# NJU-3DV/Relightable3DGaussian

Hardware: AMD Instinct MI355X
Metric: train iters/s, synthetic lego-like 800x800, 300000 Gaussians (stage-2 hot path) (higher is better)
Workload: dtype f32; 1 GPU; stage-2 train iteration (fused glue kernels + one-launch Adam): shading fwd/bwd (K=64) + rasterize fwd (S=16) + loss + rasterize bwd + Adam; 1 view/rank/step, 300000 Gaussians, 800x800, num_rendered~1755006; parallelism=dp1

## Files before the change

include/r3dg_hip.h:

```cpp
#ifndef R3DG_HIP_H
#define R3DG_HIP_H

#include <stddef.h>
#include <stdint.h>

#ifdef __cplusplus
extern "C" {
#endif

#define R3DG_OK 0
#define R3DG_EINVAL (-1)
#define R3DG_EHIP (-2)
#define R3DG_EALLOC (-3)

typedef void* (*r3dg_alloc_fn)(void* user, size_t bytes);

const char* r3dg_last_error(void);
int r3dg_release_scratch(void);
int r3dg_version(void);

int r3dg_max_features_forward(void);
int r3dg_max_features_backward(void);

size_t r3dg_geometry_state_bytes(int P);
// ... 103 lines not shown
                                 float* d_out);
int r3dg_shade_build_transport_rayset(void* stream, int P, int K, int M, const float* d_normals, const float* d_incidents,
                                      const float* d_visibility, const float* d_zsamples, float uniform_area,
                                      const float* d_env, int He, int We, const float* d_env_transform,
                                      float* d_transport, float* d_consts);
int r3dg_shade_build_transport_baked(void* stream, int P, int K, int M, const float* d_normals, const float* d_incidents,
                                     const float* d_visibility_sh, const float* d_zsamples, float uniform_area,
                                     const float* d_env, int He, int We, const float* d_env_transform,
                                     float* d_transport, float* d_consts);
int r3dg_visibility_sh_expand(void* stream, int P, int K, const float* d_normals, const float* d_zsamples,
                              const float* d_visibility_sh, float* d_visibility_out);
int r3dg_shade_build_split(void* stream, int P, int K, const int32_t* d_perm, const float* d_normals, const float* d_incidents,
                           const float* d_visibility, const float* d_incident_dirs, const float* d_zsamples,
                           float uniform_area, float* d_lt, float* d_vis_t, float* d_consts);
size_t r3dg_shade_env_footprints_bytes(int He, int We);
int r3dg_shade_env_footprints(void* stream, int He, int We, const float* d_env, float* d_env_footprints);
int r3dg_shade_forward_split(void* stream, int P, int K, const int32_t* d_perm, const float* d_base_color,
                             const float* d_roughness, const float* d_normals, const float* d_viewdirs, const float* d_lt,
                             const float* d_vis_t, const float* d_consts, const float* d_zsamples,
                             const float* d_env_transform, const float* d_env_footprints, int He, int We, float* d_out);
int r3dg_shade_frs_supported(int K, int M, int He, int We);
size_t r3dg_shade_frs_tables_bytes(int K);
int r3dg_shade_frs_build_tables(void* stream, int K, const float* d_zsamples, float* d_tables);
int r3dg_shade_frs_classify(void* stream, int P, const float* d_ray_normals, uint8_t* d_valid);
int r3dg_shade_frs_build_taps(void* stream, int P, int K, const float* d_ray_normals, const float* d_zsamples, int He, int We,
                              uint32_t* d_taps);
int r3dg_stream_wait_stream(void* waiter, void* signaller);
int r3dg_spin(void* stream, float microseconds);
int r3dg_store_u64_to_host(void* stream, const void* d_src, void* h_pinned_dst);
int r3dg_clock_probe(void* stream, int iters, unsigned long long* d_out3, float* d_sink, int* wall_clock_khz);

int r3dg_shade_frs_rotate(void* stream, int P, const float* d_incidents, const float* d_ray_normals, float* d_cprime);
int r3dg_shade_frs_forward(void* stream, int P, int K, const float* d_base_color, const float* d_roughness,
                           const float* d_normals, const float* d_viewdirs, const float* d_incidents, const float* d_env,
                           int He, int We, const float* d_visibility, float uniform_area, const uint32_t* d_taps,
                           const float* d_ray_normals, const float* d_zsamples, const float* d_tables,
                           const uint8_t* d_valid, const int32_t* d_invalid_list, int n_invalid, float* d_cprime, int flags,
                           float* d_out, void* listed_stream, float* d_feature_rows);
int r3dg_shade_frs_backward(void* stream, int P, int K, const float* d_base_color, const float* d_roughness,
                            const float* d_normals, const float* d_viewdirs, const float* d_incidents, const float* d_env,
                            int He, int We, const float* d_visibility, float uniform_area, const uint32_t* d_taps,
                            const float* d_ray_normals, const float* d_zsamples, const float* d_tables,
                            const uint8_t* d_valid, const int32_t* d_invalid_list, int n_invalid, const float* d_cprime,
                            float* d_dcprime, const float* d_dL_dpbr, const float* d_dL_ddiffuse_light,
                            float* d_dL_dbase_color, float* d_dL_droughness, float* d_dL_dviewdirs, float* d_dL_dincidents,
                            float* d_dL_denv, const float* d_block_absmax, int n_block_absmax, void* rotate_stream);
#define R3DG_SHADE_NO_ROTATION_BACK ((void*)(intptr_t)-1)
#define R3DG_CHAIN_LISTED_ROWS_IN_DCPRIME 1
#define R3DG_CHAIN_NO_GRADIENT_OUT 2
int r3dg_shade_frs_incident_chain(void* stream, int P, const float* d_ray_normals, const uint8_t* d_valid,
                                  const float* d_dcprime, float* d_dL_dincidents, float* d_incidents, float* d_exp_avg,
                                  float* d_exp_avg_sq, float* d_cprime, float lr, float lr_tail, float beta1, float beta2,
                                  float eps, int step, float grad_scale, const float* d_skip_flag, int chain_flags);

int r3dg_shade_backward(void* stream, int P, int K, int M, const float* d_base_color, const float* d_roughness,
                        const float* d_normals, const float* d_viewdirs, const float* d_incidents, const float* d_env,
                        int He, int We, const float* d_env_transform, const float* d_visibility,
                        const float* d_incident_dirs, const float* d_incident_areas, const float* d_dL_dpbr,
                        const float* d_dL_ddiffuse_light, float* d_dL_dbase_color, float* d_dL_droughness,
                        float* d_dL_dviewdirs, float* d_dL_dincidents, float* d_dL_denv);

int r3dg_shade_backward_cached(void* stream, int P, int K, int M, const float* d_base_color, const float* d_roughness,
                               const float* d_normals, const float* d_viewdirs, const float* d_incidents,
                               const float* d_env, int He, int We, const float* d_env_transform,
                               const float* d_visibility, const float* d_incident_dirs, const float* d_incident_areas,
                               const uint32_t* d_taps, const float* d_dL_dpbr, const float* d_dL_ddiffuse_light,
                               float* d_dL_dbase_color, float* d_dL_droughness, float* d_dL_dviewdirs,
                               float* d_dL_dincidents, float* d_dL_denv, const float* d_block_absmax,
                               int n_block_absmax);

int r3dg_render_equation_forward(void* stream, int P, int Si, int Sd, int Sv, const float* d_base_color,
                                 const float* d_roughness, const float* d_metallic, const float* d_normals,
                                 const float* d_viewdirs, const float* d_incidents_shs, const float* d_direct_shs,
                                 const float* d_visibility_shs, int sample_num, const float* d_rand_float,
                                 float* d_incident_dirs, float* d_pbr, float* d_diffuse_light);
int r3dg_render_equation_forward_complex(void* stream, int P, int Si, int Sd, int Sv, const float* d_base_color,
                                         const float* d_roughness, const float* d_metallic, const float* d_normals,
                                         const float* d_viewdirs, const float* d_incidents_shs,
                                         const float* d_direct_shs, const float* d_visibility_shs, int sample_num,
                                         float* d_incident_dirs, float* d_pbr, float* d_incident_lights,
                                         float* d_local_incident_lights, float* d_global_incident_lights,
                                         float* d_incident_visibility, float* d_diffuse_light,
                                         float* d_local_diffuse_light, float* d_accum, float* d_rgb_d, float* d_rgb_s);
int r3dg_render_equation_backward(void* stream, int P, int Si, int Sd, int Sv, const float* d_base_color,
                                  const float* d_roughness, const float* d_metallic, const float* d_normals,
                                  const float* d_viewdirs, const float* d_incidents_shs, const float* d_direct_shs,
                                  const float* d_visibility_shs, int sample_num, const float* d_incident_dirs,
                                  const float* d_dL_dpbr, const float* d_dL_ddiffuse_light, float* d_dL_dbase_color,
                                  float* d_dL_droughness, float* d_dL_dmetallic, float* d_dL_dnormals,
                                  float* d_dL_dviewdirs, float* d_dL_dincidents_shs, float* d_dL_ddirect_shs,
                                  float* d_dL_dvisibility_shs);

#define R3DG_SUM_SLOTS 32

int r3dg_stage2_activate(void* stream, int P, const float* d_xyz, const float* d_scaling_raw,
                         const float* d_rotation_raw, const float* d_opacity_raw, const float* d_normal_raw,
                         const float* d_base_raw, const float* d_rough_raw, const float* d_campos, float* d_scales,
                         float* d_rotations, float* d_opacity, float* d_normal, float* d_base_color,
                         float* d_roughness, float* d_viewdirs, const float* d_viewmatrix, float* d_features);
int r3dg_stage2_pack_features(void* stream, int P, const float* d_xyz, const float* d_viewmatrix, const float* d_normal,
                              const float* d_base_color, const float* d_roughness, const float* d_shade_out,
                              float* d_features, float* d_light_l1_sum);
int r3dg_stage2_unpack_gradients(void* stream, int P, const float* d_dL_dfeatures, const float* d_shade_out,
                                 float light_weight, float* d_dL_dpbr, float* d_dL_ddiffuse_light,
                                 float* d_block_absmax, float* d_light_l1_sum);
int r3dg_stage2_activate_backward(void* stream, int P, const float* d_xyz, const float* d_scaling_raw,
                                  const float* d_rotation_raw, const float* d_opacity_raw, const float* d_normal_raw,
                                  const float* d_base_raw, const float* d_rough_raw, const float* d_viewmatrix,
                                  const float* d_campos, const float* d_dL_dfeatures, const float* d_dL_dbase_color,
                                  const float* d_dL_droughness, const float* d_dL_dviewdirs, const float* d_dL_dscales,
                                  const float* d_dL_drotations, const float* d_dL_dopacity, const float* d_dL_dmeans3D,
                                  float* d_g_xyz, float* d_g_scaling, float* d_g_rotation, float* d_g_opacity,
                                  float* d_g_normal, float* d_g_base, float* d_g_rough);
int r3dg_stage2_loss(void* stream, int width, int height, const float* d_image, const float* d_opacity,
                     const float* d_feature, const float* d_pseudo_normal, const int32_t* d_n_contrib,
                     const float* d_gt, const float* d_background, const float* d_image_mask, float w_l1, float w_pbr,
                     float w_normal, const float* d_extra_dL_dimage, const float* d_extra_dL_dsrgb, float* d_dL_dimage,
                     float* d_dL_dopacity, float* d_dL_dfeature, float* d_sums,
                     int sparse_feature_gradients);
int r3dg_stage2_smooth_forward(void* stream, int width, int height, const float* d_opacity, const float* d_feature,
                               const int32_t* d_n_contrib, const float* d_gt, const float* d_image_mask,
                               float w_base_color, float w_roughness, float w_light, float* d_scratch, float* d_sums3);
int r3dg_stage2_smooth_backward(void* stream, int width, int height, const float* d_opacity, const float* d_feature,
                                const int32_t* d_n_contrib, const float* d_image_mask, const float* d_scratch,
                                float w_base_color, float w_roughness, float w_light, int accumulate_normal,
                                float* d_dL_dopacity, float* d_dL_dfeature);
int r3dg_stage2_smooth_fused(void* stream, int width, int height, const float* d_opacity, const float* d_feature,
                             const int32_t* d_n_contrib, const float* d_gt, const float* d_image_mask, float w_base_color,
                             float w_roughness, float w_light, int accumulate_normal, float* d_dL_dopacity,
                             float* d_dL_dfeature, float* d_sums3);
int r3dg_stage2_pbr_srgb(void* stream, int width, int height, const float* d_opacity, const float* d_feature,
                         const int32_t* d_n_contrib, const float* d_background, float* d_srgb);

int r3dg_stage2_activate_with(void* stream, int P, const float* d_xyz, const float* d_scaling_raw,
                              const float* d_rotation_raw, const float* d_opacity_raw, const float* d_normal_raw,
                              const float* d_base_raw, const float* d_rough_raw, const float* d_campos, float* d_scales,
                              float* d_rotations, float* d_opacity, float* d_normal, float* d_base_color,
                              float* d_roughness, float* d_viewdirs, const float* d_viewmatrix, float* d_features,
                              int n_env, const float* d_env_raw, float* d_env, float* d_zero, int n_zero);
int r3dg_stage2_activate_backward_with(void* stream, int P, const float* d_xyz, const float* d_scaling_raw,
                                       const float* d_rotation_raw, const float* d_opacity_raw, const float* d_normal_raw,
                                       const float* d_base_raw, const float* d_rough_raw, const float* d_viewmatrix,
                                       const float* d_campos, const float* d_dL_dfeatures, const float* d_dL_dbase_color,
                                       const float* d_dL_droughness, const float* d_dL_dviewdirs, const float* d_dL_dscales,
                                       const float* d_dL_drot, const float* d_dL_dopacity, const float* d_dL_dmeans3D,
                                       float* d_g_xyz, float* d_g_scaling, float* d_g_rotation, float* d_g_opacity,
                                       float* d_g_normal, float* d_g_base, float* d_g_rough, int He, int We,
                                       const float* d_env_raw, const float* d_env, float* d_dL_denv, float w_tv,
                                       float* d_g_env_raw, float* d_tv_sum, int consume);
int r3dg_stage2_normals_srgb(void* stream, int width, int height, const float* d_viewmatrix, float tan_fovx, float tan_fovy,
                             float cx, float cy, const float* d_opacity, const float* d_depth, float* d_pseudo_normal,
                             float* d_surface_xyz, const float* d_feature, const int32_t* d_n_contrib,
                             const float* d_background, float* d_srgb);

int r3dg_ssim_forward(void* stream, int width, int height, int channels, const float* d_x, const float* d_y,
                      float* d_partials, float* d_sum);
int r3dg_ssim_backward(void* stream, int width, int height, int channels, const float* d_x, const float* d_y,
                       const float* d_partials, float scale, float* d_grad_x);
int r3dg_ssim_forward_pair(void* stream, int width, int height, int channels, const float* d_x0, const float* d_x1,
                           const float* d_y, float* d_partials0, float* d_partials1, float* d_sum0, float* d_sum1);
int r3dg_ssim_backward_pair(void* stream, int width, int height, int channels, const float* d_x0, const float* d_x1,
                            const float* d_y, const float* d_partials0, const float* d_partials1, float scale0,
                            float scale1, float* d_grad_x0, float* d_grad_x1);

int r3dg_stage1_pack_features(void* stream, int P, const float* d_xyz, const float* d_viewmatrix, const float* d_normal,
                              float* d_features);
int r3dg_stage1_loss(void* stream, int width, int height, const float* d_image, const float* d_opacity,
                     const float* d_feature, const float* d_pseudo_normal, const int32_t* d_n_contrib, const float* d_gt,
                     const float* d_image_mask, float w_l1, float w_mask_entropy, float w_normal, float w_normal_smooth,
                     float w_depth_var, const float* d_extra_dL_dimage, float* d_edge_scratch, float* d_dL_dimage,
                     float* d_dL_dopacity, float* d_dL_dfeature, float* d_sums);
int r3dg_stage1_activate_backward(void* stream, int P, const float* d_xyz, const float* d_scaling_raw,
                                  const float* d_rotation_raw, const float* d_opacity_raw, const float* d_normal_raw,
                                  const float* d_viewmatrix, const float* d_dL_dfeatures, const float* d_dL_dscales,
                                  const float* d_dL_drotations, const float* d_dL_dopacity, const float* d_dL_dmeans3D,
                                  float* d_g_xyz, float* d_g_scaling, float* d_g_rotation, float* d_g_opacity,
                                  float* d_g_normal);

int r3dg_supervision_count(void* stream, int width, int height, const float* d_gt_depth, const float* d_image_mask,
                           uint32_t* d_count);
int r3dg_stage2_supervision(void* stream, int width, int height, const float* d_opacity, const float* d_feature,
                            const int32_t* d_n_contrib, const float* d_gt_depth, const float* d_mvs_normal,
                            const float* d_image_mask, const uint32_t* d_count, float w_depth, float w_normal_mvs,
                            int accumulate_normal, float* d_dL_dopacity, float* d_dL_dfeature, float* d_sums2);
int r3dg_stage1_depth_smooth(void* stream, int width, int height, const float* d_opacity, const float* d_feature,
                             const int32_t* d_n_contrib, const float* d_gt, float w_depth_smooth, float* d_edge_scratch,
                             float* d_dL_dopacity, float* d_dL_dfeature, float* d_sum);
int r3dg_stage1_gaussian_terms(void* stream, int P, const float* d_weights, const float* d_opacity, const float* d_normal,
                               const float* d_scales, const float* d_xyz, const float* d_campos, float w_point_entropy,
                               float w_orientation, float w_scaling, float* d_dL_dopacity, float* d_dL_dfeatures,
                               float* d_dL_dscales, float* d_dL_dmeans3D, float* d_sums3);

int r3dg_stage2_env_backward(void* stream, int He, int We, const float* d_raw, const float* d_env, float* d_dL_denv,
                             float w_tv, float* d_g_raw, float* d_tv_sum, int consume);

#define R3DG_ADAM_MAX_GROUPS 16
typedef struct r3dg_adam_group {
    float* param;
    const float* grad;
    float* exp_avg;
    float* exp_avg_sq;
    uint64_t n;
    float lr, lr_tail;
    uint32_t period, split;
} r3dg_adam_group;
int r3dg_adam_step(void* stream, int n_groups, const r3dg_adam_group* groups, float beta1, float beta2, float eps,
                   int step, float grad_scale, const float* d_skip_flag);

int r3dg_rasterize_backward_sh_adam_supported(int M);
int r3dg_rasterize_backward_split_sh_adam(void* stream, void* geometry_stream, int P, int S, int D, int M, int R,
                                          const float* d_background, int width, int height, const float* d_means3D,
                                          const float* d_shs, const float* d_features, const float* d_colors_precomp,
                                          const float* d_scales, float scale_modifier, const float* d_rotations,
                                          const float* d_cov3D_precomp, const float* d_viewmatrix,
                                          const float* d_projmatrix, const float* d_campos, float tan_fovx, float tan_fovy,
                                          const int32_t* d_radii, const void* d_geom_buffer, const void* d_binning_buffer,
                                          const void* d_img_buffer, const float* d_dL_dpix, const float* d_dL_dpix_o,
                                          const float* d_dL_dpix_d, const float* d_dL_dpix_f, float* d_dL_dmean2D,
                                          float* d_dL_dconic, float* d_dL_dopacity, float* d_dL_dcolor,
                                          float* d_dL_dfeature, float* d_dL_dmean3D, float* d_dL_dcov3D, float* d_dL_dsh,
                                          float* d_dL_dscale, float* d_dL_drot, int backward_geometry, int debug,
                                          int n_active_features, const int* active_features,
                                          const r3dg_adam_group* sh_adam, float beta1, float beta2, float eps, int step,
                                          float grad_scale, const float* d_skip_flag);

int r3dg_relight_pack_features(void* stream, int P, const float* d_xyz, const float* d_viewmatrix, const float* d_normal,
                               const float* d_base_color, const float* d_roughness, const float* d_shade_out,
                               float* d_features);
int r3dg_relight_compose(void* stream, int width, int height, float focal_x, float focal_y, float cx, float cy,
                         const float* d_viewmatrix, const float* d_light_transform, const float* d_envmap, int He, int We,
                         const float* d_image, const float* d_opacity, const float* d_feature,
                         const int32_t* d_n_contrib, float* d_pbr_env, float* d_render_env, float* d_env_only);

#define R3DG_EVAL_ROW 8
#define R3DG_EVAL_MEDIAN_STATE_WORDS 1024
int r3dg_relight_capture(void* stream, int width, int height, const float* d_feature, const float* d_opacity,
                         const int32_t* d_n_contrib, const float* d_background, const float* d_mask, float* d_pbr,
                         float* d_base_color, float* d_roughness, float* d_normal, float* d_visibility, float* d_diffuse,
                         float* d_specular, float* d_lights, float* d_local_lights, float* d_global_lights,
                         float* d_depth_var);
int r3dg_eval_image_metrics(void* stream, int width, int height, int channels, const float* d_pred, const float* d_gt,
                            const float* d_mask, const float* d_fill, int fill_is_image, double* d_tile_sums,
                            double* d_row);
int r3dg_eval_median_ratio(void* stream, int width, int height, const float* d_pred, const float* d_gt,
                           const float* d_mask, uint32_t* d_state, double* d_row);

#define R3DG_SCENE_COLUMNS 130
#define R3DG_SCENE_STAGE1_COLUMNS 62
#define R3DG_SCENE_GROUPS 13
#define R3DG_SCENE_MAX_COLUMNS 250
#define R3DG_SCENE_PLACEMENT_FLOATS 111
#define R3DG_SCENE_ZERO_INCIDENTS 1
#define R3DG_SCENE_ROTATE_SH 2
int r3dg_scene_place_records(void* stream, int P, int A, const float* d_records, const int32_t* d_column_map,
                             const float* d_placement, int flags, long long row_offset, void** dst_groups);
int r3dg_scene_place_groups(void* stream, int P, void** src_groups, const float* d_placement, int flags,
                            long long row_offset, void** dst_groups);
int r3dg_scene_pack_records(void* stream, int P, int columns, void** src_groups, float* d_records);

int r3dg_relight_quantize(void* stream, int width, int height, int channels, const float* d_image, uint8_t* d_bytes);

int r3dg_view_unpack(void* stream, int width, int height, int channels, const uint8_t* d_pixels, const float* d_background,
                     float* d_image, float* d_mask);

int r3dg_view_unpack_masked(void* stream, int width, int height, const uint8_t* d_pixels, const uint8_t* d_mask_bytes,
                            float* d_image, float* d_mask);

#define R3DG_VIEW_RESIZE_MAX_SCALE 16
int r3dg_view_resize(void* stream, int width, int height, int channels, const uint8_t* d_pixels, const uint8_t* d_mask_bytes,
                     const float* d_background, int out_width, int out_height, float* d_image, float* d_mask);

#define R3DG_EXR_TILE 4096
#define R3DG_EXR_MAX_KEPT 8
#define R3DG_EXR_MAX_TILES 32768
int r3dg_exr_unpack_chunks(void* stream, int width, int height, int file_channels, int bytes_per_sample, int chunks,
                           int max_chunk_rows, const uint8_t* d_inflated, long long inflated_bytes, const int32_t* d_chunk_table,
                           int kept, const int32_t* d_kept_channels, uint32_t* d_tile_sums, long long tile_sums_count,
                           void* d_planes);

int r3dg_view_unpack_hdr(void* stream, int width, int height, int is_half, const void* d_view, const uint8_t* d_mask_bytes,
                         const float* d_background, float* d_image, float* d_mask);

int r3dg_densify_accumulate(void* stream, int P, const float* d_viewspace_grad, const float* d_normal_grad,
                            const int32_t* d_radii, const float* d_weights, float* d_xyz_gradient_accum,
                            float* d_normal_gradient_accum, float* d_denom, float* d_weights_accum,
                            float* d_max_radii2D,
                            const float* d_skip_flag);

typedef struct r3dg_densify_config {
    int32_t mode;
    int32_t n_split;
    float grad_threshold, grad_normal_threshold, min_opacity, weights_threshold;
    float dense_size, world_size_limit, split_divisor, max_screen_size;
} r3dg_densify_config;

size_t r3dg_densify_temp_bytes(int P);
int r3dg_densify_plan(void* stream, int P, const r3dg_densify_config* config, const float* d_scaling_raw,
                      const float* d_opacity_raw, const float* d_xyz_gradient_accum,
                      const float* d_normal_gradient_accum, const float* d_denom, const float* d_weights_accum,
                      const float* d_max_radii2D, int32_t* d_src_row, int32_t* d_kind, int32_t* d_counts, void* d_temp);

#define R3DG_DENSIFY_MAX_GROUPS 24
#define R3DG_DENSIFY_ROLE_COPY 0
#define R3DG_DENSIFY_ROLE_XYZ 1
#define R3DG_DENSIFY_ROLE_SCALING 2
typedef struct r3dg_densify_group {
// ... 95 lines not shown
```

relightable3dgaussian_amd/csrc/capi_stage.hip:

```cpp
#include "capi_internal.hpp"

using namespace r3dg;

extern "C" {

int r3dg_stage2_activate(void* stream_, int P, const float* xyz, const float* scaling_raw, const float* rotation_raw,
                         const float* opacity_raw, const float* normal_raw, const float* base_raw,
                         const float* rough_raw, const float* campos, float* scales, float* rot, float* opacity,
                         float* normal, float* base_color, float* roughness, float* viewdirs, const float* viewmatrix,
                         float* features)
{
    return r3dg_stage2_activate_with(stream_, P, xyz, scaling_raw, rotation_raw, opacity_raw, normal_raw, base_raw, rough_raw,
                                     campos, scales, rot, opacity, normal, base_color, roughness, viewdirs, viewmatrix, features,
                                     0, nullptr, nullptr, nullptr, 0);
}

int r3dg_stage2_activate_with(void* stream_, int P, const float* xyz, const float* scaling_raw, const float* rotation_raw,
                              const float* opacity_raw, const float* normal_raw, const float* base_raw,
                              const float* rough_raw, const float* campos, float* scales, float* rot, float* opacity,
                              float* normal, float* base_color, float* roughness, float* viewdirs, const float* viewmatrix,
                              float* features, int n_env, const float* env_raw, float* env, float* zero, int n_zero)
{
    if (P < 0) return invalid("stage2_activate: bad P");
    if (n_env < 0 || n_zero < 0) return invalid("stage2_activate: bad side-job size");
// ... 109 lines not shown
                     float* dL_dfeature, float* sums, int sparse_feature_gradients)
{
    if (width < 0 || height < 0) return invalid("stage2_loss: bad image size");
    if ((long long)width * height == 0) return R3DG_OK;
    if (!image || !opacity || !feature || !pseudo_normal || !n_contrib || !gt || !bg || !dL_dimage || !dL_dopacity ||
        !dL_dfeature || !sums)
        return invalid("stage2_loss: null buffer");
    return guarded([&]() -> int {
        StageTimer t((hipStream_t)stream_, ST_S2_LOSS);
        launch_s2_loss((hipStream_t)stream_, width * height, image, opacity, feature, pseudo_normal, n_contrib, gt, bg,
                       image_mask, w_l1, w_pbr, w_normal, extra_dimage, extra_dsrgb, dL_dimage, dL_dopacity, dL_dfeature, sums,
                       sparse_feature_gradients);
        return R3DG_OK;
    });
}

int r3dg_stage2_smooth_forward(void* stream_, int width, int height, const float* opacity, const float* feature,
                               const int32_t* n_contrib, const float* gt, const float* image_mask, float w_base_color,
                               float w_roughness, float w_light, float* scratch, float* sums3)
{
    if (width < 0 || height < 0) return invalid("stage2_smooth_forward: bad image size");
    if ((long long)width * height == 0) return R3DG_OK;
    if (!opacity || !feature || !n_contrib || !gt || !scratch || !sums3) return invalid("stage2_smooth_forward: null buffer");
    return guarded([&]() -> int {
        StageTimer t((hipStream_t)stream_, ST_S2_LOSS);
        launch_s2_smooth_forward((hipStream_t)stream_, width, height, opacity, feature, n_contrib, gt, image_mask,
                                 w_base_color, w_roughness, w_light, scratch, sums3);
        return R3DG_OK;
    });
}

int r3dg_stage2_smooth_backward(void* stream_, int width, int height, const float* opacity, const float* feature,
                                const int32_t* n_contrib, const float* image_mask, const float* scratch, float w_base_color,
                                float w_roughness, float w_light, int accumulate_normal, float* dL_dopacity,
                                float* dL_dfeature)
{
    if (width < 0 || height < 0) return invalid("stage2_smooth_backward: bad image size");
    if ((long long)width * height == 0) return R3DG_OK;
    if (!opacity || !feature || !n_contrib || !scratch || !dL_dopacity || !dL_dfeature)
        return invalid("stage2_smooth_backward: null buffer");
    return guarded([&]() -> int {
        StageTimer t((hipStream_t)stream_, ST_S2_LOSS);
        launch_s2_smooth_backward((hipStream_t)stream_, width, height, opacity, feature, n_contrib, image_mask, scratch,
                                  w_base_color != 0.f, w_roughness != 0.f, w_light != 0.f, accumulate_normal, dL_dopacity,
                                  dL_dfeature);
        return R3DG_OK;
    });
}

int r3dg_stage2_smooth_fused(void* stream_, int width, int height, const float* opacity, const float* feature,
                             const int32_t* n_contrib, const float* gt, const float* image_mask, float w_base_color,
                             float w_roughness, float w_light, int accumulate_normal, float* dL_dopacity, float* dL_dfeature,
                             float* sums3)
{
    if (width < 0 || height < 0) return invalid("stage2_smooth_fused: bad image size");
    if ((long long)width * height == 0) return R3DG_OK;
    if (!opacity || !feature || !n_contrib || !gt || !dL_dopacity || !dL_dfeature || !sums3)
        return invalid("stage2_smooth_fused: null buffer");
    return guarded([&]() -> int {
        StageTimer t((hipStream_t)stream_, ST_S2_LOSS);
        launch_s2_smooth_fused((hipStream_t)stream_, width, height, opacity, feature, n_contrib, gt, image_mask, w_base_color,
                               w_roughness, w_light, accumulate_normal, dL_dopacity, dL_dfeature, sums3);
        return R3DG_OK;
    });
}

int r3dg_stage1_pack_features(void* stream_, int P, const float* xyz, const float* viewmatrix, const float* normal,
                              float* features)
{
    if (P < 0) return invalid("stage1_pack_features: bad P");
    if (P == 0) return R3DG_OK;
    if (!xyz || !viewmatrix || !normal || !features) return invalid("stage1_pack_features: null buffer");
    return guarded([&]() -> int {
        StageTimer t((hipStream_t)stream_, ST_S2_PACK);
        launch_s1_pack((hipStream_t)stream_, P, xyz, viewmatrix, normal, features);
        return R3DG_OK;
    });
}

int r3dg_stage1_loss(void* stream_, int width, int height, const float* image, const float* opacity,
                     const float* feature, const float* pseudo_normal, const int32_t* n_contrib, const float* gt,
                     const float* image_mask, float w_l1, float w_mask_entropy, float w_normal, float w_normal_smooth,
                     float w_depth_var, const float* extra_dimage, float* edge_scratch, float* dL_dimage,
                     float* dL_dopacity, float* dL_dfeature, float* sums)
{
    if (width < 0 || height < 0) return invalid("stage1_loss: bad image size");
    if ((long long)width * height == 0) return R3DG_OK;
    if (!image || !opacity || !feature || !pseudo_normal || !n_contrib || !gt || !dL_dimage || !dL_dopacity ||
        !dL_dfeature || !sums)
        return invalid("stage1_loss: null buffer");
    if (w_normal_smooth != 0.f && !edge_scratch) return invalid("stage1_loss: the normal-smoothness term needs edge_scratch");
    return guarded([&]() -> int {
        StageTimer t((hipStream_t)stream_, ST_S2_LOSS);
        if (w_normal_smooth != 0.f)
            launch_s1_edge((hipStream_t)stream_, width, height, feature, opacity, n_contrib, gt, edge_scratch, sums + 4 * R3DG_SUM_SLOTS);
        launch_s1_loss((hipStream_t)stream_, width, height, image, opacity, feature, pseudo_normal, n_contrib, gt, image_mask,
                       w_l1, w_mask_entropy, w_normal, w_normal_smooth, w_depth_var, extra_dimage,
                       w_normal_smooth != 0.f ? edge_scratch : nullptr, dL_dimage, dL_dopacity, dL_dfeature, sums);
        return R3DG_OK;
    });
}

int r3dg_stage1_activate_backward(void* stream_, int P, const float* xyz, const float* scaling_raw,
                                  const float* rotation_raw, const float* opacity_raw, const float* normal_raw,
                                  const float* viewmatrix, const float* dL_dfeatures, const float* dL_dscales,
                                  const float* dL_drot, const float* dL_dopacity, const float* dL_dmeans3D, float* g_xyz,
                                  float* g_scaling, float* g_rotation, float* g_opacity, float* g_normal)
{
    if (P < 0) return invalid("stage1_activate_backward: bad P");
    if (P == 0) return R3DG_OK;
    if (!xyz || !scaling_raw || !rotation_raw || !opacity_raw || !normal_raw || !viewmatrix || !dL_dfeatures ||
        !dL_dscales || !dL_drot || !dL_dopacity || !dL_dmeans3D || !g_xyz || !g_scaling || !g_rotation || !g_opacity ||
        !g_normal)
        return invalid("stage1_activate_backward: null buffer");
    return guarded([&]() -> int {
        StageTimer t((hipStream_t)stream_, ST_S2_ACTIVATE_BWD);
        launch_s1_activate_backward((hipStream_t)stream_, P, xyz, scaling_raw, rotation_raw, opacity_raw, normal_raw,
                                    viewmatrix, dL_dfeatures, dL_dscales, dL_drot, dL_dopacity, dL_dmeans3D, g_xyz,
                                    g_scaling, g_rotation, g_opacity, g_normal);
        return R3DG_OK;
    });
}

int r3dg_stage2_pbr_srgb(void* stream_, int width, int height, const float* opacity, const float* feature,
                         const int32_t* n_contrib, const float* bg, float* srgb)
{
    if (width < 0 || height < 0) return invalid("stage2_pbr_srgb: bad image size");
    if ((long long)width * height == 0) return R3DG_OK;
    if (!opacity || !feature || !n_contrib || !bg || !srgb) return invalid("stage2_pbr_srgb: null buffer");
    return guarded([&]() -> int {
        launch_s2_pbr_srgb((hipStream_t)stream_, width * height, opacity, feature, n_contrib, bg, srgb);
        return R3DG_OK;
    });
}

int r3dg_stage2_normals_srgb(void* stream_, int width, int height, const float* viewmatrix, float tan_fovx, float tan_fovy,
                             float cx, float cy, const float* opacity, const float* depth, float* pseudo_normal,
                             float* surface_xyz, const float* feature, const int32_t* n_contrib, const float* bg, float* srgb)
{
    if (width < 0 || height < 0) return invalid("stage2_normals_srgb: bad image size");
    if ((long long)width * height == 0) return R3DG_OK;
    if ((long long)width * height > 0x7fffffffLL) return invalid("stage2_normals_srgb: image too large");
    if (!viewmatrix || !opacity || !depth || !pseudo_normal || !surface_xyz || !feature || !n_contrib || !bg || !srgb)
        return invalid("stage2_normals_srgb: null buffer");
    return guarded([&]() -> int {
        StageTimer t((hipStream_t)stream_, ST_NORMAL);
        const float focal_y = height / (2.0f * tan_fovy), focal_x = width / (2.0f * tan_fovx);
        launch_s2_normals_srgb((hipStream_t)stream_, width, height, viewmatrix, focal_x, focal_y, cx, cy, opacity, depth,
                               pseudo_normal, surface_xyz, feature, n_contrib, bg, srgb);
        return R3DG_OK;
    });
}

int r3dg_ssim_forward_pair(void* stream_, int width, int height, int channels, const float* x0, const float* x1,
                           const float* y, float* partials0, float* partials1, float* sum0, float* sum1)
{
    if (width < 0 || height < 0 || channels < 0) return invalid("ssim_forward: bad shape");
    if ((long long)width * height * channels == 0) return R3DG_OK;
    if (!x0 || !y || !partials0 || (x1 && !partials1)) return invalid("ssim_forward: null buffer");
    if ((long long)channels * 2 > 65535) return invalid("ssim_forward: too many channels");
    return guarded([&]() -> int {
        StageTimer t((hipStream_t)stream_, ST_SSIM);
        const float* x[2] = {x0, x1};
        float* partials[2] = {partials0, partials1};
        float* sum[2] = {sum0, sum1};
        launch_ssim_forward((hipStream_t)stream_, width, height, channels, x1 ? 2 : 1, x, y, partials, sum);
        return R3DG_OK;
    });
}

int r3dg_ssim_backward_pair(void* stream_, int width, int height, int channels, const float* x0, const float* x1,
                            const float* y, const float* partials0, const float* partials1, float scale0, float scale1,
                            float* grad_x0, float* grad_x1)
{
    if (width < 0 || height < 0 || channels < 0) return invalid("ssim_backward: bad shape");
    if ((long long)width * height * channels == 0) return R3DG_OK;
    if (!x0 || !y || !partials0 || !grad_x0 || (x1 && (!partials1 || !grad_x1))) return invalid("ssim_backward: null buffer");
    if ((long long)channels * 2 > 65535) return invalid("ssim_backward: too many channels");
    return guarded([&]() -> int {
        StageTimer t((hipStream_t)stream_, ST_SSIM);
        const float* x[2] = {x0, x1};
        float* partials[2] = {const_cast<float*>(partials0), const_cast<float*>(partials1)};
        const float scale[2] = {scale0, scale1};
        float* grad[2] = {grad_x0, grad_x1};
        launch_ssim_backward((hipStream_t)stream_, width, height, channels, x1 ? 2 : 1, x, y, partials, scale, grad);
        return R3DG_OK;
    });
}

int r3dg_ssim_forward(void* stream_, int width, int height, int channels, const float* x, const float* y,
                      float* partials, float* sum)
{
    return r3dg_ssim_forward_pair(stream_, width, height, channels, x, nullptr, y, partials, nullptr, sum, nullptr);
}

int r3dg_ssim_backward(void* stream_, int width, int height, int channels, const float* x, const float* y,
                       const float* partials, float scale, float* grad_x)
{
    return r3dg_ssim_backward_pair(stream_, width, height, channels, x, nullptr, y, partials, nullptr, scale, 0.f, grad_x,
                                   nullptr);
}

int r3dg_stage2_env_backward(void* stream_, int He, int We, const float* raw, const float* env, float* dL_denv,
                             float w_tv, float* g_raw, float* tv_sum, int consume)
{
    if (He < 0 || We < 0) return invalid("stage2_env_backward: bad texture size");
    if (He * We == 0) return R3DG_OK;
    if (!raw || !env || !dL_denv || !g_raw) return invalid("stage2_env_backward: null buffer");
    return guarded([&]() -> int {
        launch_s2_env_backward((hipStream_t)stream_, He, We, raw, env, dL_denv, w_tv, g_raw, tv_sum, consume);
        return R3DG_OK;
    });
}

int r3dg_adam_step(void* stream_, int n_groups, const r3dg_adam_group* groups, float beta1, float beta2, float eps,
                   int step, float grad_scale, const float* skip_flag)
{
    if (n_groups < 0 || n_groups > R3DG_ADAM_MAX_GROUPS) return invalid("adam_step: bad group count");
    if (step < 1) return invalid("adam_step: step counts from 1");
    if (n_groups == 0) return R3DG_OK;
    if (!groups) return invalid("adam_step: null group table");
    for (int i = 0; i < n_groups; i++) {
        if (groups[i].n >= (1ull << 32)) return invalid("adam_step: group larger than 2^32 elements");
        if (groups[i].n && (!groups[i].param || !groups[i].grad || !groups[i].exp_avg || !groups[i].exp_avg_sq))
            return invalid("adam_step: null buffer in group");
    }
    return guarded([&]() -> int {
        StageTimer t((hipStream_t)stream_, ST_ADAM);
        launch_adam((hipStream_t)stream_, n_groups, groups, beta1, beta2, eps, step, grad_scale, skip_flag);
        return R3DG_OK;
    });
}

int r3dg_relight_pack_features(void* stream_, int P, const float* xyz, const float* viewmatrix, const float* normal,
                               const float* base_color, const float* roughness, const float* shade_out, float* features)
{
    if (P < 0) return invalid("relight_pack_features: bad P");
    if (P == 0) return R3DG_OK;
    if (!xyz || !viewmatrix || !normal || !base_color || !roughness || !shade_out || !features)
        return invalid("relight_pack_features: null buffer");
    if ((size_t)features & 15) return invalid("relight_pack_features: features must be 16-byte aligned");
    return guarded([&]() -> int {
        StageTimer t((hipStream_t)stream_, ST_RELIGHT_PACK);
        launch_relight_pack((hipStream_t)stream_, P, xyz, viewmatrix, normal, base_color, roughness, shade_out, features);
        return R3DG_OK;
    });
}

int r3dg_relight_compose(void* stream_, int width, int height, float focal_x, float focal_y, float cx, float cy,
                         const float* viewmatrix, const float* light_transform, const float* envmap, int He, int We,
                         const float* image, const float* opacity, const float* feature, const int32_t* n_contrib,
                         float* pbr_env, float* render_env, float* env_only)
{
    if (width < 0 || height < 0 || He < 1 || We < 1) return invalid("relight_compose: bad shape");
    if ((long long)width * height == 0) return R3DG_OK;
    if ((long long)width * height >= (1ll << 31)) return invalid("relight_compose: image too large");
    if (!viewmatrix || !envmap || !opacity || !feature || !n_contrib) return invalid("relight_compose: null buffer");
    if (render_env && !image) return invalid("relight_compose: render_env needs the rendered image");
    if (!(focal_x > 0.f) || !(focal_y > 0.f)) return invalid("relight_compose: focal lengths must be positive");
    return guarded([&]() -> int {
        StageTimer t((hipStream_t)stream_, ST_RELIGHT_COMPOSE);
        launch_relight_compose((hipStream_t)stream_, width, height, focal_x, focal_y, cx, cy, viewmatrix, light_transform,
                               envmap, He, We, image, opacity, feature, n_contrib, pbr_env, render_env, env_only);
        return R3DG_OK;
    });
}

int r3dg_relight_capture(void* stream_, int width, int height, const float* feature, const float* opacity,
                         const int32_t* n_contrib, const float* background, const float* mask, float* pbr,
                         float* base_color, float* roughness, float* normal, float* visibility, float* diffuse,
                         float* specular, float* lights, float* local_lights, float* global_lights, float* depth_var)
{
    if (width < 0 || height < 0) return invalid("relight_capture: bad shape");
    if ((long long)width * height == 0) return R3DG_OK;
    if ((long long)width * height >= (1ll << 31)) return invalid("relight_capture: image too large");
    if (!feature || !opacity || !n_contrib) return invalid("relight_capture: null buffer");
    if ((pbr || mask) && !background) return invalid("relight_capture: the pbr map and the mask need a background");
    const CaptureMaps maps = {pbr, base_color, roughness, normal, visibility, diffuse, specular, lights, local_lights,
                              global_lights, depth_var};
    return guarded([&]() -> int {
        launch_relight_capture((hipStream_t)stream_, width, height, feature, opacity, n_contrib, background, mask, maps);
        return R3DG_OK;
    });
}

int r3dg_eval_image_metrics(void* stream_, int width, int height, int channels, const float* pred, const float* gt,
                            const float* mask, const float* fill, int fill_is_image, double* tile_sums, double* row)
{
    if (width < 1 || height < 1 || channels < 1 || channels > 3) return invalid("eval_image_metrics: bad shape");
    if ((long long)width * height >= (1ll << 31)) return invalid("eval_image_metrics: image too large");
    if (!pred || !gt || !tile_sums || !row) return invalid("eval_image_metrics: null buffer");
    if (fill && !mask) return invalid("eval_image_metrics: a fill needs a mask");
    return guarded([&]() -> int {
        launch_eval_image_metrics((hipStream_t)stream_, width, height, channels, pred, gt, mask, fill, fill_is_image, tile_sums,
                                  row);
        return R3DG_OK;
    });
}

int r3dg_eval_median_ratio(void* stream_, int width, int height, const float* pred, const float* gt, const float* mask,
                           uint32_t* state, double* row)
{
    if (width < 0 || height < 0) return invalid("eval_median_ratio: bad shape");
    if ((long long)width * height >= (1ll << 31)) return invalid("eval_median_ratio: image too large");
    if (!state || !row) return invalid("eval_median_ratio: null buffer");
    if ((long long)width * height != 0 && (!pred || !gt)) return invalid("eval_median_ratio: null image");
// ... 94 lines not shown
```

relightable3dgaussian_amd/csrc/launchers.hpp:

```cpp
#pragma once
#include "common.hpp"

namespace r3dg {

__attribute__((visibility("hidden"))) int persistent_cus();

void release_gradient_records();
void launch_mark_visible(hipStream_t s, int P, const float* means3D, const float* vm, uint8_t* present);
void launch_preprocess(hipStream_t s, int P, int D, int M, const float* means3D, const float* scales, float scale_modifier,
                       const float* rotations, const float* opacities, const float* shs, uint8_t* clamped,
                       const float* cov3D_precomp, const float* colors_precomp, const float* vm, const float* pm,
                       const float* cam_pos, int W, int H, float tan_fovx, float tan_fovy, float focal_x, float focal_y,
                       int* radii, float* means2D, float* depths, float* cov3Ds, float* rgb, float* conic_opacity,
                       float* splat, int gx, int gy, uint32_t* tiles_touched, uint32_t* block_sums,
                       unsigned long long* total, bool scan_now, uint32_t* zero_words, int zero_n);
void launch_duplicate_with_keys(hipStream_t s, int P, const float* means2D, const float* depths,
                                const uint32_t* tiles_touched, const uint32_t* block_offsets, uint32_t* point_offsets,
                                uint64_t* keys, uint32_t* values, const int* radii, int gx, int gy);
void launch_identify_tile_ranges(hipStream_t s, int L, const uint64_t* keys, uint32_t* ranges);
void launch_tile_order(hipStream_t s, int T, const uint32_t* ranges, uint32_t* order, uint32_t small_cap, uint32_t* big_list,
                       uint32_t* big_count);
void launch_render_forward(hipStream_t s, int W, int H, int S, const uint32_t* tile_order, const uint32_t* ranges,
                           const uint32_t* point_list, const float* splat, const float* features, float* final_T,
                           uint32_t* n_contrib, const float* bg, float* out_color, float* out_opacity, float* out_depth,
                           float* out_feature, float* out_weights);
void launch_pseudo_normal(hipStream_t s, int W, int H, const float* vm, float focal_x, float focal_y, float cx, float cy,
                          const float* opacities, const float* depths, float* normals, float* surface_xyz, bool debug);
void launch_render_backward(hipStream_t s, int P, int W, int H, int S, int n_active, const int* active,
                            const uint32_t* tile_order, const uint32_t* ranges, const uint32_t* point_list, const float* bg,
                            const float* splat, const float* features, const float* final_Ts, const uint32_t* n_contrib,
                            const float* dL_dpix, const float* dL_dpix_o, const float* dL_dpix_d, const float* dL_dpix_f,
                            float* dL_dmean2D, float* dL_dconic, float* dL_dopacity, float* dL_dcolor, float* dL_dfeature,
                            int bg_geom);
void launch_render_backward_features(hipStream_t s, int W, int H, int S, int n_active, const int* active,
                                     const uint32_t* tile_order, const uint32_t* ranges, const uint32_t* point_list,
                                     const float* splat, const float* final_Ts, const uint32_t* n_contrib,
                                     const float* dL_dpix_f, float* dL_dfeature);
struct ShAdamArgs {
    r3dg_adam_group g;
    float beta1, beta2, eps, bias1, inv_sqrt_bias2, grad_scale;
    const float* skip_flag;
};
bool preprocess_backward_applies_adam(int M);
void launch_preprocess_backward(hipStream_t s, int P, int D, int M, const float* means, const int* radii, const float* shs,
                                const uint8_t* clamped, const float* scales, const float* rotations, float scale_modifier,
                                const float* cov3Ds, const float* vm, const float* proj, float h_x, float h_y,
                                float tan_fovx, float tan_fovy, const float* campos, float* dL_dmean2D,
                                const float* dL_dconic, const float* conic_opacity, int W, int H, float* dL_dmeans,
                                const float* dL_dcolor, float* dL_dcov3D, float* dL_dsh, float* dL_dscale, float* dL_drot,
                                const ShAdamArgs* adam);
void launch_shade_forward(hipStream_t s, int P, int K, int M, const float* base_color, const float* roughness,
                          const float* normals, const float* viewdirs, const float* incidents, const float* env, int He,
                          int We, const float* tr, const float* visibility, const float* dirs, const float* areas,
                          float* out, const uint32_t* taps, bool train_outputs, float uniform_area, bool taps_are_radiance,
                          bool leave_room);
size_t shade_frs_table_floats(int K);
bool shade_frs_supported(int K, int M, int He, int We);
void launch_shade_frs_build_tables(hipStream_t s, int K, const float* zsamples, float* tables);
void launch_shade_frs_classify(hipStream_t s, int P, const float* ray_normals, uint8_t* valid);
void launch_shade_frs_build_taps(hipStream_t s, int P, int K, const float* ray_normals, const float* zsamples, int He,
                                 int We, uint32_t* taps);
void launch_shade_frs_forward_aux(hipStream_t s, int P, const float* incidents, const float* ray_normals, float* cprime);
void launch_shade_frs_forward_main(hipStream_t s, int P, int K, const float* base_color, const float* roughness,
                                   const float* normals, const float* viewdirs, const float* env, int He, int We,
                                   const float* visibility, float uniform_area, const uint32_t* taps,
                                   const float* ray_normals, const float* tables, const uint8_t* valid, const float* cprime,
                                   bool leave_room, float* out, float* feat);
void launch_shade_frs_forward_listed(hipStream_t s, int K, const float* base_color, const float* roughness,
                                     const float* normals, const float* viewdirs, const float* incidents, const float* env,
                                     int He, int We, const float* visibility, const float* ray_normals,
                                     const float* zsamples, float uniform_area, const int* invalid_list, int n_invalid,
                                     float* out, float* feat);
void launch_shade_frs_incident_chain(hipStream_t s, int P, const float* ray_normals, const uint8_t* valid, const float* dcp,
                                     float* d_inc, float* incidents, float* exp_avg, float* exp_avg_sq, float* cprime,
                                     float lr, float lr_tail, float beta1, float beta2, float eps, int step,
                                     float grad_scale, const float* skip_flag, int listed_in_dcprime, bool write_gradient);
const unsigned int* launch_shade_frs_backward_aux(hipStream_t s, int P, const float* g_pbr, const float* g_diff,
                                                  const float* block_absmax, int n_block_absmax, int* gmax_n);
void launch_shade_frs_backward_main(hipStream_t s, int P, int K, const float* base_color, const float* roughness,
                                    const float* normals, const float* viewdirs, const float* env, int He, int We,
                                    const float* visibility, float uniform_area, const uint32_t* taps,
                                    const float* ray_normals, const float* tables, const uint8_t* valid, const float* cprime,
                                    float* dcp, const float* g_pbr, const float* g_diff, float* d_base, float* d_rough,
                                    float* d_view, float* d_env, const unsigned int* gmax, int gmax_n);
void launch_shade_frs_backward_rotate(hipStream_t s, int P, const float* ray_normals, const float* dcp, float* d_inc,
                                      const uint8_t* valid);
void launch_shade_frs_backward_listed(hipStream_t s, int K, const float* base_color, const float* roughness,
                                      const float* normals, const float* viewdirs, const float* incidents, const float* env,
                                      int He, int We, const float* visibility, const float* ray_normals,
                                      const float* zsamples, float uniform_area, const int* invalid_list, int n_invalid,
                                      const float* g_pbr, const float* g_diff, float* d_base, float* d_rough, float* d_view,
                                      float* d_inc, float* d_env, const unsigned int* gmax, int gmax_n);
void launch_shade_build_taps(hipStream_t s, size_t n, const float* dirs, const float* tr, int He, int We, const float* env,
                             uint32_t* taps);
void launch_shade_build_split(hipStream_t s, int P, int K, const int* perm, const float* normals, const float* incidents,
                              const float* visibility, const float* dirs, const float* zsamples, float uniform_area,
                              float* lt, float* vis_t, float* consts);
void launch_shade_forward_split(hipStream_t s, int P, int K, const int* perm, const float* base_color,
                                const float* roughness, const float* normals, const float* viewdirs, const float* lt,
                                const float* vis_t, const float* consts, const float* zsamples, const float* tr,
                                const float* env4, int He, int We, float* out);
void launch_shade_env_footprints(hipStream_t s, int He, int We, const float* env, float* fp);
void launch_shade_build_transport(hipStream_t s, int P, int K, int M, const float* normals, const float* incidents,
                                  const float* visibility, const float* dirs, const float* areas, float uniform_area,
                                  float* radiance_to_transport, float* consts);
void launch_shade_build_transport_rayset(hipStream_t s, int P, int K, int M, const float* normals, const float* incidents,
                                         const float* visibility, const float* zsamples, float uniform_area, const float* env,
                                         int He, int We, const float* tr, float* transport, float* consts);
void launch_shade_build_transport_baked(hipStream_t s, int P, int K, int M, const float* normals, const float* incidents,
                                        const float* visibility_sh, const float* zsamples, float uniform_area, const float* env,
                                        int He, int We, const float* tr, float* transport, float* consts);
void launch_visibility_sh_expand(hipStream_t s, int P, int K, const float* normals, const float* zsamples,
                                 const float* visibility_sh, float* out);
void launch_shade_forward_transport(hipStream_t s, int P, int K, const float* base_color, const float* roughness,
                                    const float* normals, const float* viewdirs, const float* transport, const float* consts,
                                    const float* zsamples, const float* dirs, float* out);
void launch_shade_backward(hipStream_t s, int P, int K, int M, const float* base_color, const float* roughness,
                           const float* normals, const float* viewdirs, const float* incidents, const float* env, int He,
                           int We, const float* tr, const float* visibility, const float* dirs, const float* areas,
                           const float* g_pbr, const float* g_diff, float* d_base, float* d_rough, float* d_view,
                           float* d_inc, float* d_env, const uint32_t* taps, const float* block_absmax, int n_block_absmax);
void launch_re_forward(hipStream_t s, bool complex_, int P, int Si, int Sd, int Sv, const float* base_color,
                       const float* roughness, const float* metallic, const float* normals, const float* viewdirs,
                       const float* inc, const float* direct, const float* vis, int K, const float* rand_float,
                       float* incident_dirs, float* out_pbr, float* out_lights, float* out_local, float* out_global,
                       float* out_vis, float* out_diffuse, float* out_local_diffuse, float* out_accum, float* out_rgb_d,
                       float* out_rgb_s);
void launch_re_backward(hipStream_t s, int P, int Si, int Sd, int Sv, const float* base_color, const float* roughness,
                        const float* metallic, const float* normals, const float* viewdirs, const float* inc,
                        const float* direct, const float* vis, int K, const float* incident_dirs, const float* dL_dpbr,
                        const float* dL_ddl, float* dL_dbase, float* dL_drough, float* dL_dmetal, float* dL_dnormals,
                        float* dL_dviewdirs, float* dL_dinc, float* dL_ddirect, float* dL_dvis);
void launch_s2_activate(hipStream_t s, int P, const float* xyz, const float* scaling_raw, const float* rotation_raw,
                        const float* opacity_raw, const float* normal_raw, const float* base_raw, const float* rough_raw,
                        const float* campos, float* scales, float* rot, float* opacity, float* normal, float* base_color,
                        float* roughness, float* viewdirs, const float* viewmatrix, float* features, int n_env,
                        const float* env_raw, float* env, float* zero, int n_zero);
void launch_s2_pack(hipStream_t s, int P, const float* xyz, const float* viewmatrix, const float* normal,
                    const float* base_color, const float* roughness, const float* shade_out, float* features,
                    float* light_l1_sum);
void launch_s2_unpack(hipStream_t s, int P, const float* dL_dfeatures, const float* shade_out, float light_weight,
                      float* dL_dpbr, float* dL_ddiffuse, float* block_absmax, float* light_l1_sum);
void launch_s2_activate_backward(hipStream_t s, int P, const float* xyz, const float* scaling_raw, const float* rotation_raw,
                                 const float* opacity_raw, const float* normal_raw, const float* base_raw,
                                 const float* rough_raw, const float* viewmatrix, const float* campos,
                                 const float* dL_dfeatures, const float* dL_dbase_shade, const float* dL_drough_shade,
                                 const float* dL_dviewdirs, const float* dL_dscales, const float* dL_drot,
                                 const float* dL_dopacity, const float* dL_dmeans3D, float* g_xyz, float* g_scaling,
                                 float* g_rotation, float* g_opacity, float* g_normal, float* g_base, float* g_rough, int He,
                                 int We, const float* env_raw, const float* env, float* dL_denv, float w_tv,
                                 float* g_env_raw, float* tv_sum, int consume);
void launch_s2_loss(hipStream_t s, int HW, const float* image, const float* opacity, const float* feature,
                    const float* pseudo_normal, const int* n_contrib, const float* gt, const float* bg,
                    const float* image_mask, float w_l1, float w_pbr, float w_normal, const float* extra_dimage,
                    const float* extra_dsrgb, float* dL_dimage, float* dL_dopacity, float* dL_dfeature, float* sums,
                    int sparse);
void launch_s2_smooth_forward(hipStream_t s, int W, int H, const float* opacity, const float* feature, const int* n_contrib,
                              const float* gt, const float* image_mask, float w_base, float w_rough, float w_light,
                              float* scratch, float* sums3);
void launch_s2_smooth_fused(hipStream_t s, int W, int H, const float* opacity, const float* feature, const int* n_contrib,
                            const float* gt, const float* image_mask, float w_base, float w_rough, float w_light,
                            int accumulate_normal, float* dL_dopacity, float* dL_dfeature, float* sums3);
void launch_s2_smooth_backward(hipStream_t s, int W, int H, const float* opacity, const float* feature, const int* n_contrib,
                               const float* image_mask, const float* scratch, int has_base, int has_rough, int has_light,
                               int accumulate_normal, float* dL_dopacity, float* dL_dfeature);
void launch_s2_pbr_srgb(hipStream_t s, int HW, const float* opacity, const float* feature, const int* n_contrib,
                        const float* bg, float* srgb);
void launch_s2_normals_srgb(hipStream_t s, int W, int H, const float* vm, float focal_x, float focal_y, float cx, float cy,
                            const float* opacity, const float* depths, float* normals, float* surface_xyz,
                            const float* feature, const int* n_contrib, const float* bg, float* srgb);
void launch_ssim_forward(hipStream_t s, int W, int H, int C, int n_images, const float* const* x, const float* y,
                         float* const* partials, float* const* sum);
void launch_ssim_backward(hipStream_t s, int W, int H, int C, int n_images, const float* const* x, const float* y,
                          float* const* partials, const float* scale, float* const* grad_x);
void launch_adam(hipStream_t s, int n_groups, const r3dg_adam_group* groups, float beta1, float beta2, float eps, int step,
                 float grad_scale, const float* skip_flag);
void launch_s1_pack(hipStream_t s, int P, const float* xyz, const float* viewmatrix, const float* normal, float* features);
void launch_s1_edge(hipStream_t s, int W, int H, const float* feature, const float* opacity, const int* n_contrib,
                    const float* gt, float* edge_g, float* sum_out);
void launch_s1_loss(hipStream_t s, int W, int H, const float* image, const float* opacity, const float* feature,
                    const float* pseudo_normal, const int* n_contrib, const float* gt, const float* image_mask, float w_l1,
                    float w_entropy, float w_normal, float w_smooth, float w_var, const float* extra_dimage,
                    const float* edge_g, float* dL_dimage, float* dL_dopacity, float* dL_dfeature, float* sums);
void launch_s1_activate_backward(hipStream_t s, int P, const float* xyz, const float* scaling_raw, const float* rotation_raw,
                                 const float* opacity_raw, const float* normal_raw, const float* viewmatrix,
                                 const float* dL_dfeatures, const float* dL_dscales, const float* dL_drot,
                                 const float* dL_dopacity, const float* dL_dmeans3D, float* g_xyz, float* g_scaling,
                                 float* g_rotation, float* g_opacity, float* g_normal);
void launch_s2_env_backward(hipStream_t s, int He, int We, const float* raw, const float* env, float* dL_denv, float w_tv,
                            float* g_raw, float* tv_sum, int consume);
uint32_t tile_sort_small_cap();
void launch_tile_sort(hipStream_t s, int T, const uint32_t* tile_order, const uint32_t* ranges, const uint32_t* big_list,
                      uint32_t* big_count, uint64_t* keys, uint32_t* vals, uint64_t* scratch, bool entries);
void launch_tile_binning(hipStream_t s, int P, int T, const float* means2D, const float* depths, const int* radii,
                         const uint32_t* tiles_touched, uint32_t* block_offsets, int gx, int gy, uint32_t* tile_counts,
                         uint32_t* cursor, uint32_t* ranges, uint32_t* point_offsets, uint64_t* entries,
                         unsigned long long* total, long long capacity, float* overflow_flag, unsigned int* overflow_count,
                         bool fused, uint32_t* order, uint32_t small_cap, uint32_t* big_list, uint32_t* big_count);
int tile_binning_max_tiles();
void launch_densify_accumulate(hipStream_t s, int P, const float* viewspace_grad, const float* normal_grad, const int* radii,
                               const float* weights, float* xyz_accum, float* normal_accum, float* denom,
                               float* weights_accum, float* max_radii2D, const float* skip_flag);
size_t densify_temp_bytes(size_t P);
void launch_densify_plan(hipStream_t s, int P, const r3dg_densify_config& cfg, const float* scaling_raw,
                         const float* opacity_raw, const float* xyz_accum, const float* normal_accum, const float* denom,
                         const float* weights_accum, const float* max_radii2D, int32_t* src_row, int32_t* kind,
                         int32_t* counts, void* temp);
void launch_densify_gather(hipStream_t s, int P_out, const int32_t* src_row, const int32_t* kind, int n_groups,
                           const r3dg_densify_group* groups, const float* xyz, const float* scaling_raw,
                           const float* rotation_raw, const float* normal_table, float split_divisor);
void launch_reset_opacity(hipStream_t s, int P, float cap, float* opacity_raw, float* exp_avg, float* exp_avg_sq);
void launch_relight_pack(hipStream_t s, int P, const float* xyz, const float* viewmatrix, const float* normal,
                         const float* base_color, const float* roughness, const float* shade_out, float* features);
void launch_relight_compose(hipStream_t s, int W, int H, float fx, float fy, float cx, float cy, const float* viewmatrix,
                            const float* tr, const float* env, int He, int We, const float* image, const float* opacity,
                            const float* feature, const int* n_contrib, float* pbr_env, float* render_env, float* env_only);
struct CaptureMaps {
    float *pbr, *base_color, *roughness, *normal, *visibility, *diffuse, *specular, *lights, *local_lights, *global_lights,
        *depth_var;
};
void launch_relight_capture(hipStream_t s, int W, int H, const float* feature, const float* opacity, const int* n_contrib,
                            const float* background, const float* mask, const CaptureMaps& maps);
struct SceneGroups {
    float* p[R3DG_SCENE_GROUPS];
};
void launch_scene_place_records(hipStream_t s, int P, int A, const float* records, const int* column_map, const float* placement,
                                int flags, long long row_offset, const SceneGroups& dst);
void launch_scene_place_groups(hipStream_t s, int P, const SceneGroups& src, const float* placement, int flags,
                               long long row_offset, const SceneGroups& dst);
void launch_scene_pack_records(hipStream_t s, int P, int columns, const SceneGroups& src, float* records);
void launch_relight_quantize(hipStream_t s, int W, int H, int C, const float* image, uint8_t* bytes);
void launch_view_unpack(hipStream_t s, int W, int H, int C, const uint8_t* pixels, const float* background, float* image,
                        float* mask);
void launch_view_unpack_masked(hipStream_t s, int W, int H, const uint8_t* pixels, const uint8_t* mask_bytes, float* image,
                               float* mask);
void launch_view_resize(hipStream_t s, int W, int H, int C, const uint8_t* pixels, const uint8_t* mask_bytes, const float* background,
                        int OW, int OH, float* image, float* mask);
size_t exr_tiles_per_chunk(int W, int C, int B, int max_rows);
void launch_exr_unpack_chunks(hipStream_t s, int W, int H, int C, int B, int chunks, int max_rows, const uint8_t* inflated,
                              long long inflated_bytes, const int32_t* table, int kept, const int32_t* kept_channels,
                              uint32_t* tile_sums, void* planes);
void launch_view_unpack_hdr(hipStream_t s, int W, int H, int is_half, const void* view, const uint8_t* mask_bytes,
                            const float* background, float* image, float* mask);
void launch_eval_metric_tiles(hipStream_t s, int W, int H, int C, const float* pred, const float* gt, const float* mask,
                              const float* fill, int fill_is_image, double* tile_sums);
void launch_eval_image_metrics(hipStream_t s, int W, int H, int C, const float* pred, const float* gt, const float* mask,
                               const float* fill, int fill_is_image, double* tile_sums, double* row);
void launch_eval_median_ratio(hipStream_t s, int W, int H, const float* pred, const float* gt, const float* mask,
                              uint32_t* state, double* row);
size_t knn_temp_bytes(size_t P);
void knn_dist2(hipStream_t s, int P, const float* pts, float* dists, void* temp);
size_t bvh_build_temp_bytes(size_t P);
void bvh_build(hipStream_t s, int P, int32_t* nodes, float* aabbs, uint64_t* morton, void* temp);
void bvh_prepare_leaves(hipStream_t s, int P, const float* means, const float* scales, const float* rotations, int32_t* nodes,
                        float* aabbs, float* covs_inv);
void bvh_trace_count(hipStream_t s, int num_rays, const int32_t* nodes, const float* aabbs, const float* rays_o,
                     const float* rays_d, int32_t* counts, int* overflow);
void bvh_trace_fill(hipStream_t s, int num_rays, const int32_t* nodes, const float* aabbs, const float* rays_o,
                    const float* rays_d, const float* means, const int32_t* counts, const int64_t* offsets_inclusive,
                    uint64_t* keys, int32_t* points, float* positions, int32_t* ray_ids);
void bvh_trace_opacity(hipStream_t s, int num_rays, int P, const int32_t* nodes, const float* aabbs, const float* rays_o,
                       const float* rays_d, const float* means, const float* covs, const float* opac, const float* normals,
                       int32_t* contributes, float* out, int* overflow);
size_t bvh_trace_records_bytes(size_t P);
void bvh_pack_traversal(hipStream_t s, int P, const int32_t* nodes, const float* aabbs, const float* means,
                        const float* covs, const float* opac, const float* normals, void* records);
void bvh_trace_visits(hipStream_t s, int P, const void* records, unsigned long long out[2]);
void bvh_trace_opacity_packed(hipStream_t s, int num_rays, int P, void* records, const float* rays_o, const float* rays_d,
                              int32_t* contributes, float* out, int* overflow);
void bvh_trace_bundles(hipStream_t s, int P, int K, void* records, const int32_t* nodes, const float* zsamples, int leaf_lo,
                       int leaf_hi, float origin_offset, float* out, int32_t* contributes, float* dirs_out, int* overflow);
void bvh_trace_hemisphere(hipStream_t s, int P, int T, void* records, const int32_t* nodes, const float* raw_dirs, int leaf_lo,
                          int leaf_hi, float origin_offset, float* out, float* dirs_out, int32_t* contributes, int* overflow);
int visibility_sh_fit_loss_rows(int P);
void visibility_sh_fit(hipStream_t s, int P, int T, long long steps_done, const float* dirs, const float* visibility, float lr,
                       float beta1, float beta2, float eps, float* coeffs, float* exp_avg, float* exp_avg_sq,
                       float* loss_partials);
void launch_transpose_selftest(hipStream_t s, int N, int dpp, const float* in, float* out, int* chan, int* owner);

}
```

relightable3dgaussian_amd/csrc/ssim.hip:

```cpp
#include "launchers.hpp"

namespace r3dg {

constexpr int SSIM_R = 5;
constexpr int SSIM_T = 32;
constexpr int SSIM_E = SSIM_T + 2 * SSIM_R;
constexpr int SSIM_B = 4;
constexpr int SSIM_NLOAD = (SSIM_E * SSIM_E + 255) / 256;

__constant__ float kSsimWin[11] = {1.028380124e-03f, 7.598758209e-03f, 3.600077331e-02f, 1.093606874e-01f,
                                   2.130055279e-01f, 2.660117149e-01f, 2.130055279e-01f, 1.093606874e-01f,
                                   3.600077331e-02f, 7.598758209e-03f, 1.028380124e-03f};

struct SsimImage {
    const float* x;
    const float* y;
    float* partials;
    float* sum;
    float* grad_x;
    float scale;
};
struct SsimBatch {
    SsimImage im[2];
};

struct SsimEval {
    const float* mask;
    const float* fill;
    int fill_is_image;
    double* tile_sums;
};

template <bool EVAL>
__device__ __forceinline__ void ssim_forward_tile(int W, int H, int C, const SsimImage I, const SsimEval E)
{
    const float* __restrict__ x = I.x;
    const float* __restrict__ y = I.y;
    float* __restrict__ partials = I.partials;
    float* __restrict__ sum = I.sum;
    constexpr int IN_FLOATS = 2 * SSIM_E * (SSIM_E + 1), H_FLOATS = 5 * SSIM_E * (SSIM_T + 1);
    __shared__ float s_raw[IN_FLOATS > H_FLOATS ? IN_FLOATS : H_FLOATS];
    float (*s_x)[SSIM_E + 1] = reinterpret_cast<float (*)[SSIM_E + 1]>(s_raw);
    float (*s_y)[SSIM_E + 1] = reinterpret_cast<float (*)[SSIM_E + 1]>(s_raw + SSIM_E * (SSIM_E + 1));
    float (*s_h)[SSIM_E][SSIM_T + 1] = reinterpret_cast<float (*)[SSIM_E][SSIM_T + 1]>(s_raw);
    __shared__ float s_part[4];
    const size_t HW = (size_t)H * W;
    const int c = blockIdx.z % C;
    const float* xc = x + c * HW;
    const float* yc = y + c * HW;
    const int bx = blockIdx.x * SSIM_T, by = blockIdx.y * SSIM_T;
    {
        float xv[SSIM_NLOAD], yv[SSIM_NLOAD];
#pragma unroll
        for (int j = 0; j < SSIM_NLOAD; j++) {
            const int i = threadIdx.x + j * 256;
            const int r = i / SSIM_E, q = i % SSIM_E;
            const int gy = by + r - SSIM_R, gx = bx + q - SSIM_R;
            const bool in = i < SSIM_E * SSIM_E && gx >= 0 && gx < W && gy >= 0 && gy < H;
            const size_t o = (size_t)(in ? gy : 0) * W + (in ? gx : 0);
            float vx = xc[o], vy = yc[o];
            if constexpr (EVAL) {
                if (E.mask != nullptr) {
#pragma clang fp contract(off)
                    const float m = E.mask[o];
                    const float f = E.fill == nullptr ? 0.f : (E.fill_is_image ? E.fill[c * HW + o] : E.fill[c]);
                    const float fm = f * (1.f - m);
                    const float xm = vx * m, ym = vy * m;
                    vx = xm + fm;
                    vy = ym + fm;
                }
            }
            xv[j] = in ? vx : 0.f;
            yv[j] = in ? vy : 0.f;
        }
#pragma unroll
        for (int j = 0; j < SSIM_NLOAD; j++) {
            const int i = threadIdx.x + j * 256;
            if (i < SSIM_E * SSIM_E) {
                s_x[i / SSIM_E][i % SSIM_E] = xv[j];
                s_y[i / SSIM_E][i % SSIM_E] = yv[j];
            }
        }
    }
    __syncthreads();
    double sq_err = 0.0;
    if constexpr (EVAL) {
        const int ex = threadIdx.x % SSIM_T, ey0 = (threadIdx.x / SSIM_T) * SSIM_B;
#pragma unroll
        for (int o = 0; o < SSIM_B; o++) {
            if (bx + ex < W && by + ey0 + o < H) {
                const float d = s_x[ey0 + o + SSIM_R][ex + SSIM_R] - s_y[ey0 + o + SSIM_R][ex + SSIM_R];
                sq_err += (double)(d * d);
            }
        }
    }
    float w[11];
#pragma unroll
    for (int k = 0; k < 11; k++) w[k] = kSsimWin[k];
    constexpr int ITEMS = SSIM_E * (SSIM_T / SSIM_B), ROUNDS = (ITEMS + 255) / 256;
    float hres[ROUNDS][5][SSIM_B];
#pragma unroll
    for (int rd = 0; rd < ROUNDS; rd++) {
        const int i = threadIdx.x + rd * 256;
        if (i < ITEMS) {
            const int r = i / (SSIM_T / SSIM_B), q0 = (i % (SSIM_T / SSIM_B)) * SSIM_B;
            float xv[SSIM_B + 10], yv[SSIM_B + 10];
#pragma unroll
            for (int k = 0; k < SSIM_B + 10; k++) { xv[k] = s_x[r][q0 + k]; yv[k] = s_y[r][q0 + k]; }
#pragma unroll
            for (int o = 0; o < SSIM_B; o++) {
                float a0 = 0.f, a1 = 0.f, a2 = 0.f, a3 = 0.f, a4 = 0.f;
#pragma unroll
                for (int k = 0; k < 11; k++) {
                    const float wx = w[k] * xv[o + k], wy = w[k] * yv[o + k];
                    a0 += wx; a1 += wy; a2 += wx * xv[o + k]; a3 += wy * yv[o + k]; a4 += wx * yv[o + k];
                }
                hres[rd][0][o] = a0; hres[rd][1][o] = a1; hres[rd][2][o] = a2; hres[rd][3][o] = a3; hres[rd][4][o] = a4;
            }
        }
    }
    __syncthreads();
#pragma unroll
    for (int rd = 0; rd < ROUNDS; rd++) {
        const int i = threadIdx.x + rd * 256;
        if (i < ITEMS) {
            const int r = i / (SSIM_T / SSIM_B), q0 = (i % (SSIM_T / SSIM_B)) * SSIM_B;
#pragma unroll
            for (int m = 0; m < 5; m++)
#pragma unroll
                for (int o = 0; o < SSIM_B; o++) s_h[m][r][q0 + o] = hres[rd][m][o];
        }
    }
    __syncthreads();
    const int tx = threadIdx.x % SSIM_T, ty0 = (threadIdx.x / SSIM_T) * SSIM_B;
    const int px = bx + tx;
    float acc[5][SSIM_B];
#pragma unroll
    for (int m = 0; m < 5; m++) {
        float col[SSIM_B + 10];
#pragma unroll
        for (int k = 0; k < SSIM_B + 10; k++) col[k] = s_h[m][ty0 + k][tx];
#pragma unroll
        for (int o = 0; o < SSIM_B; o++) {
            float a = 0.f;
#pragma unroll
            for (int k = 0; k < 11; k++) a += w[k] * col[o + k];
            acc[m][o] = a;
        }
    }
    float ssim_sum = 0.f;
    float* pc = EVAL ? nullptr : partials + (size_t)c * 3 * HW;
#pragma unroll
    for (int o = 0; o < SSIM_B; o++) {
        const int py = by + ty0 + o;
        if (px < W && py < H) {
            const float mu1 = acc[0][o], mu2 = acc[1][o], e11 = acc[2][o], e22 = acc[3][o], e12 = acc[4][o];
            const float C1 = 0.01f * 0.01f, C2 = 0.03f * 0.03f;
            const float A = 2.f * mu1 * mu2 + C1;
            const float B = 2.f * (e12 - mu1 * mu2) + C2;
            const float C = mu1 * mu1 + mu2 * mu2 + C1;
            const float D = (e11 - mu1 * mu1) + (e22 - mu2 * mu2) + C2;
            const float inv = 1.f / (C * D);
            const float ssim = A * B * inv;
            ssim_sum += ssim;
            if constexpr (!EVAL) {
                const size_t off = (size_t)py * W + px;
                pc[off] = 2.f * mu2 * (B - A) * inv - ssim * 2.f * mu1 * (D - C) * inv;
                pc[HW + off] = -ssim / D;
                pc[2 * HW + off] = 2.f * A * inv;
            }
        }
    }
    const float tot = block_sum_256(ssim_sum, s_part);
    if constexpr (!EVAL) {
        if (threadIdx.x == 0 && sum != nullptr) atomicAdd(sum_slot(sum), tot);
    } else {
        __shared__ double s_sq[4];
#pragma unroll
        for (int o = 32; o > 0; o >>= 1) sq_err += __shfl_xor(sq_err, o, 64);
        if ((threadIdx.x & 63) == 0) s_sq[threadIdx.x >> 6] = sq_err;
        __syncthreads();
        if (threadIdx.x == 0) {
            const size_t wg = blockIdx.x + (size_t)gridDim.x * (blockIdx.y + (size_t)gridDim.y * blockIdx.z);
            E.tile_sums[2 * wg] = ((s_sq[0] + s_sq[1]) + s_sq[2]) + s_sq[3];
            E.tile_sums[2 * wg + 1] = (double)tot;
        }
    }
}

__global__ void __launch_bounds__(256)
ssim_forward_kernel(int W, int H, int C, SsimBatch batch)
{
    const SsimImage I = batch.im[blockIdx.z / C];
    ssim_forward_tile<false>(W, H, C, I, SsimEval{});
}

__global__ void __launch_bounds__(256)
eval_image_metrics_kernel(int W, int H, int C, SsimImage I, SsimEval E)
{
    ssim_forward_tile<true>(W, H, C, I, E);
}

__global__ void __launch_bounds__(256)
ssim_backward_kernel(int W, int H, int C, SsimBatch batch)
{
    const SsimImage I = batch.im[blockIdx.z / C];
    const float* __restrict__ x = I.x;
    const float* __restrict__ y = I.y;
    const float* __restrict__ partials = I.partials;
    const float scale = I.scale;
    float* __restrict__ grad_x = I.grad_x;
    constexpr int IN_FLOATS = 3 * SSIM_E * (SSIM_E + 1);
    __shared__ float s_raw[IN_FLOATS];
    float (*s_p)[SSIM_E][SSIM_E + 1] = reinterpret_cast<float (*)[SSIM_E][SSIM_E + 1]>(s_raw);
    float (*s_h)[SSIM_E][SSIM_T + 1] = reinterpret_cast<float (*)[SSIM_E][SSIM_T + 1]>(s_raw);
    const size_t HW = (size_t)H * W;
    const int c = blockIdx.z % C;
    const float* pc = partials + (size_t)c * 3 * HW;
    const int bx = blockIdx.x * SSIM_T, by = blockIdx.y * SSIM_T;
    const int tx = threadIdx.x % SSIM_T, ty0 = (threadIdx.x / SSIM_T) * SSIM_B;
    const int px = bx + tx;
    float xo[SSIM_B], yo[SSIM_B];
#pragma unroll
    for (int o = 0; o < SSIM_B; o++) {
        const int py = by + ty0 + o;
        const bool in = px < W && py < H;
        const size_t off = in ? (size_t)py * W + px : 0;
        xo[o] = x[c * HW + off];
        yo[o] = y[c * HW + off];
    }
    {
        float pv[3][SSIM_NLOAD];
#pragma unroll
        for (int j = 0; j < SSIM_NLOAD; j++) {
            const int i = threadIdx.x + j * 256;
            const int r = i / SSIM_E, q = i % SSIM_E;
            const int gy = by + r - SSIM_R, gx = bx + q - SSIM_R;
            const bool in = i < SSIM_E * SSIM_E && gx >= 0 && gx < W && gy >= 0 && gy < H;
            const size_t o = (size_t)(in ? gy : 0) * W + (in ? gx : 0);
            const float v0 = pc[o], v1 = pc[HW + o], v2 = pc[2 * HW + o];
            pv[0][j] = in ? v0 : 0.f;
            pv[1][j] = in ? v1 : 0.f;
            pv[2][j] = in ? v2 : 0.f;
        }
#pragma unroll
        for (int j = 0; j < SSIM_NLOAD; j++) {
            const int i = threadIdx.x + j * 256;
            if (i < SSIM_E * SSIM_E) {
                s_p[0][i / SSIM_E][i % SSIM_E] = pv[0][j];
                s_p[1][i / SSIM_E][i % SSIM_E] = pv[1][j];
                s_p[2][i / SSIM_E][i % SSIM_E] = pv[2][j];
            }
        }
    }
    __syncthreads();
    float w[11];
#pragma unroll
    for (int k = 0; k < 11; k++) w[k] = kSsimWin[k];
    constexpr int ITEMS = SSIM_E * (SSIM_T / SSIM_B), ROUNDS = (ITEMS + 255) / 256;
    float hres[ROUNDS][3][SSIM_B];
#pragma unroll
    for (int rd = 0; rd < ROUNDS; rd++) {
        const int i = threadIdx.x + rd * 256;
        if (i < ITEMS) {
            const int r = i / (SSIM_T / SSIM_B), q0 = (i % (SSIM_T / SSIM_B)) * SSIM_B;
#pragma unroll
            for (int m = 0; m < 3; m++) {
                float v[SSIM_B + 10];
#pragma unroll
                for (int k = 0; k < SSIM_B + 10; k++) v[k] = s_p[m][r][q0 + k];
#pragma unroll
                for (int o = 0; o < SSIM_B; o++) {
                    float a = 0.f;
#pragma unroll
                    for (int k = 0; k < 11; k++) a += w[k] * v[o + k];
                    hres[rd][m][o] = a;
                }
            }
        }
    }
    __syncthreads();
#pragma unroll
    for (int rd = 0; rd < ROUNDS; rd++) {
        const int i = threadIdx.x + rd * 256;
        if (i < ITEMS) {
            const int r = i / (SSIM_T / SSIM_B), q0 = (i % (SSIM_T / SSIM_B)) * SSIM_B;
#pragma unroll
            for (int m = 0; m < 3; m++)
#pragma unroll
                for (int o = 0; o < SSIM_B; o++) s_h[m][r][q0 + o] = hres[rd][m][o];
        }
    }
    __syncthreads();
    float acc[3][SSIM_B];
#pragma unroll
    for (int m = 0; m < 3; m++) {
        float col[SSIM_B + 10];
#pragma unroll
        for (int k = 0; k < SSIM_B + 10; k++) col[k] = s_h[m][ty0 + k][tx];
#pragma unroll
        for (int o = 0; o < SSIM_B; o++) {
            float a = 0.f;
#pragma unroll
            for (int k = 0; k < 11; k++) a += w[k] * col[o + k];
            acc[m][o] = a;
        }
    }
#pragma unroll
    for (int o = 0; o < SSIM_B; o++) {
        const int py = by + ty0 + o;
        if (px < W && py < H) {
            const size_t off = (size_t)py * W + px;
            grad_x[c * HW + off] = scale * (acc[0][o] + 2.f * xo[o] * acc[1][o] + yo[o] * acc[2][o]);
        }
    }
}

void launch_ssim_forward(hipStream_t s, int W, int H, int C, int n_images, const float* const* x, const float* y,
                         float* const* partials, float* const* sum)
{
    SsimBatch b = {};
    for (int i = 0; i < n_images; i++) b.im[i] = SsimImage{x[i], y, partials[i], sum[i], nullptr, 0.f};
    dim3 grid((W + SSIM_T - 1) / SSIM_T, (H + SSIM_T - 1) / SSIM_T, C * n_images);
    ssim_forward_kernel<<<grid, 256, 0, s>>>(W, H, C, b);
    check_launch(s, false, "ssim_forward_kernel");
}

void launch_eval_metric_tiles(hipStream_t s, int W, int H, int C, const float* pred, const float* gt, const float* mask,
                              const float* fill, int fill_is_image, double* tile_sums)
{
    const SsimImage I = {pred, gt, nullptr, nullptr, nullptr, 0.f};
    const SsimEval E = {mask, fill, fill_is_image, tile_sums};
    dim3 grid((W + SSIM_T - 1) / SSIM_T, (H + SSIM_T - 1) / SSIM_T, C);
    eval_image_metrics_kernel<<<grid, 256, 0, s>>>(W, H, C, I, E);
    check_launch(s, false, "eval_image_metrics_kernel");
}

void launch_ssim_backward(hipStream_t s, int W, int H, int C, int n_images, const float* const* x, const float* y,
                          float* const* partials, const float* scale, float* const* grad_x)
{
    SsimBatch b = {};
    for (int i = 0; i < n_images; i++) b.im[i] = SsimImage{x[i], y, partials[i], nullptr, grad_x[i], scale[i]};
    dim3 grid((W + SSIM_T - 1) / SSIM_T, (H + SSIM_T - 1) / SSIM_T, C * n_images);
    ssim_backward_kernel<<<grid, 256, 0, s>>>(W, H, C, b);
    check_launch(s, false, "ssim_backward_kernel");
}

}
```

relightable3dgaussian_amd/csrc/stage2_glue.hip:

```cpp
#include "launchers.hpp"
#include "glue_math.hpp"
#include "pseudo_normal.hpp"
#include "r3dg_hip.h"

namespace r3dg {

struct ActivateSide {
    int nb_main;
    int n_env;
    const float* env_raw;
    float* env;
    float* zero;
    int n_zero;
};

__global__ void __launch_bounds__(256)
s2_activate_kernel(int P, const float* __restrict__ xyz, const float* __restrict__ scaling_raw,
                   const float* __restrict__ rotation_raw, const float* __restrict__ opacity_raw,
                   const float* __restrict__ normal_raw, const float* __restrict__ base_raw,
                   const float* __restrict__ rough_raw, const float* __restrict__ campos,
                   float* __restrict__ scales, float* __restrict__ rot, float* __restrict__ opacity,
                   float* __restrict__ normal, float* __restrict__ base_color, float* __restrict__ roughness,
                   float* __restrict__ viewdirs, const float* __restrict__ viewmatrix, float* __restrict__ features,
                   ActivateSide side)
{
    if ((int)blockIdx.x >= side.nb_main) {
        const int nb_side = (int)gridDim.x - side.nb_main;
        for (int k = ((int)blockIdx.x - side.nb_main) * 256 + (int)threadIdx.x; k < side.n_env; k += nb_side * 256) {
            const float r = side.env_raw[k];
            side.env[k] = r > 20.f ? r : log1pf(expf(r));
        }
        for (int k = ((int)blockIdx.x - side.nb_main) * 256 + (int)threadIdx.x; k < side.n_zero; k += nb_side * 256)
            side.zero[k] = 0.f;
        return;
    }
    const int i = blockIdx.x * 256 + threadIdx.x;
    if (i >= P) return;
    const size_t i3 = 3 * (size_t)i, i4 = 4 * (size_t)i;
#pragma unroll
    for (int c = 0; c < 3; c++) scales[i3 + c] = __expf(scaling_raw[i3 + c]);
    {
        const float q[4] = {rotation_raw[i4], rotation_raw[i4 + 1], rotation_raw[i4 + 2], rotation_raw[i4 + 3]};
        const float inv = 1.f / fmaxf(sqrtf(q[0] * q[0] + q[1] * q[1] + q[2] * q[2] + q[3] * q[3]), 1e-12f);
#pragma unroll
        for (int c = 0; c < 4; c++) rot[i4 + c] = q[c] * inv;
    }
    opacity[i] = sigmoidf_(opacity_raw[i]);
    float inv, nrm[3];
    {
        const float v[3] = {normal_raw[i3], normal_raw[i3 + 1], normal_raw[i3 + 2]};
        normalize3(v, 1e-3f, nrm, inv);
        normal[i3] = nrm[0]; normal[i3 + 1] = nrm[1]; normal[i3 + 2] = nrm[2];
    }
    if (base_raw != nullptr) {
        float bc[3];
#pragma unroll
        for (int c = 0; c < 3; c++) base_color[i3 + c] = bc[c] = 0.03f + 0.77f * sigmoidf_(base_raw[i3 + c]);
        const float rg = 0.09f + 0.9f * sigmoidf_(rough_raw[i]);
        roughness[i] = rg;
        const float p[3] = {xyz[i3], xyz[i3 + 1], xyz[i3 + 2]};
        const float d[3] = {campos[0] - p[0], campos[1] - p[1], campos[2] - p[2]};
        float o[3];
        normalize3(d, 1e-12f, o, inv);
        viewdirs[i3] = o[0]; viewdirs[i3 + 1] = o[1]; viewdirs[i3 + 2] = o[2];
        if (features != nullptr) {
            const float depth = p[0] * viewmatrix[2] + p[1] * viewmatrix[6] + p[2] * viewmatrix[10] + viewmatrix[14];
            float* f = features + 16 * (size_t)i;
            *reinterpret_cast<float2*>(f) = make_float2(depth, depth * depth);
            f[5] = nrm[0]; f[6] = nrm[1]; f[7] = nrm[2];
            *reinterpret_cast<float4*>(f + 8) = make_float4(bc[0], bc[1], bc[2], rg);
        }
    }
}

__global__ void __launch_bounds__(256)
s2_pack_features_kernel(int P, const float* __restrict__ xyz, const float* __restrict__ viewmatrix,
                        const float* __restrict__ normal, const float* __restrict__ base_color,
                        const float* __restrict__ roughness, const float* __restrict__ shade_out,
                        float* __restrict__ features, float* __restrict__ light_l1_sum)
{
    __shared__ float s_part[4];
    const int i = blockIdx.x * 256 + threadIdx.x;
    float l1 = 0.f;
    if (i < P) {
        const size_t i3 = 3 * (size_t)i;
        const float depth = xyz[i3] * viewmatrix[2] + xyz[i3 + 1] * viewmatrix[6] + xyz[i3 + 2] * viewmatrix[10] +
                            viewmatrix[14];
        const float* so = shade_out + 19 * (size_t)i;
        const float dl[3] = {so[3], so[4], so[5]};
        float4* f = reinterpret_cast<float4*>(features + 16 * (size_t)i);
        f[0] = make_float4(depth, depth * depth, so[0], so[1]);
        f[1] = make_float4(so[2], normal[i3], normal[i3 + 1], normal[i3 + 2]);
        f[2] = make_float4(base_color[i3], base_color[i3 + 1], base_color[i3 + 2], roughness[i]);
        f[3] = make_float4(dl[0], dl[1], dl[2], so[18]);
        const float m = (dl[0] + dl[1] + dl[2]) / 3.f;
        l1 = fabsf(dl[0] - m) + fabsf(dl[1] - m) + fabsf(dl[2] - m);
    }
    const float tot = block_sum_256(l1, s_part);
    if (threadIdx.x == 0 && light_l1_sum != nullptr) atomicAdd(sum_slot(light_l1_sum), tot);
}


__global__ void __launch_bounds__(256)
s2_unpack_kernel(int P, const float* __restrict__ dL_dfeatures, const float* __restrict__ shade_out, float light_weight,
                 float* __restrict__ dL_dpbr, float* __restrict__ dL_ddiffuse, float* __restrict__ block_absmax,
                 float* __restrict__ light_l1_sum)
{
    __shared__ float s_m[4];
    __shared__ float s_l1[4];
    const int i = blockIdx.x * 256 + threadIdx.x;
    float m = 0.f, l1 = 0.f;
    bool bad = false;
    if (i < P) {
        const float4* g = reinterpret_cast<const float4*>(dL_dfeatures + 16 * (size_t)i);
        const float4 g0 = g[0], g1 = g[1], g3 = g[3];
        const size_t i3 = 3 * (size_t)i;
        dL_dpbr[i3] = g0.z; dL_dpbr[i3 + 1] = g0.w; dL_dpbr[i3 + 2] = g1.x;
        const float* so = shade_out + 19 * (size_t)i;
        const float dl[3] = {so[3], so[4], so[5]};
        const float mean = (dl[0] + dl[1] + dl[2]) / 3.f;
        const float s[3] = {signf_(dl[0] - mean), signf_(dl[1] - mean), signf_(dl[2] - mean)};
        const float sm = (s[0] + s[1] + s[2]) / 3.f;
        l1 = fabsf(dl[0] - mean) + fabsf(dl[1] - mean) + fabsf(dl[2] - mean);
        const float d0 = g3.x + light_weight * (s[0] - sm), d1 = g3.y + light_weight * (s[1] - sm),
                    d2 = g3.z + light_weight * (s[2] - sm);
        dL_ddiffuse[i3] = d0; dL_ddiffuse[i3 + 1] = d1; dL_ddiffuse[i3 + 2] = d2;
        const float v[6] = {fabsf(g0.z), fabsf(g0.w), fabsf(g1.x), fabsf(d0), fabsf(d1), fabsf(d2)};
#pragma unroll
        for (int c = 0; c < 6; c++) {
            bad = bad || !(v[c] <= 3.0e38f);
            m = fmaxf(m, v[c]);
        }
    }
    if (light_l1_sum != nullptr) {
        const float tot = block_sum_256(l1, s_l1);
        if (threadIdx.x == 0) atomicAdd(sum_slot(light_l1_sum), tot);
    }
    if (block_absmax == nullptr) return;
#pragma unroll
    for (int o = 32; o > 0; o >>= 1) m = fmaxf(m, __shfl_xor(m, o, 64));
    if (__ballot(bad) != 0ull) m = __uint_as_float(0x7f800000u);
    if ((threadIdx.x & 63) == 0) s_m[threadIdx.x >> 6] = m;
    __syncthreads();
    if (threadIdx.x == 0) block_absmax[blockIdx.x] = fmaxf(fmaxf(s_m[0], s_m[1]), fmaxf(s_m[2], s_m[3]));
}

struct EnvBackward {
    int He, We;
    const float* raw;
    const float* env;
    float* dL_denv;
    float w_tv;
    float* g_raw;
    float* tv_sum;
    int consume;
};

__device__ __forceinline__ void env_backward_block(int block, const EnvBackward& a)
{
    __shared__ float s_part[4];
    const int He = a.He, We = a.We;
    const int n = He * We * 3;
    const int i = block * 256 + threadIdx.x;
    float tv = 0.f;
    if (i < n) {
        const int w = (i / 3) % We, h = i / (3 * We);
        const float inv_v = He > 1 ? 1.f / (3.f * (He - 1) * We) : 0.f, inv_h = We > 1 ? 1.f / (3.f * He * (We - 1)) : 0.f;
        const float x = a.env[i];
        float g = 0.f;
        if (h > 0) g += inv_v * 2.f * (x - a.env[i - 3 * We]);
        if (h < He - 1) { const float d = a.env[i + 3 * We] - x; g -= inv_v * 2.f * d; tv += inv_v * d * d; }
        if (w > 0) g += inv_h * 2.f * (x - a.env[i - 3]);
        if (w < We - 1) { const float d = a.env[i + 3] - x; g -= inv_h * 2.f * d; tv += inv_h * d * d; }
        const float r = a.raw[i];
        const float dsoft = r > 20.f ? 1.f : sigmoidf_(r);
        a.g_raw[i] = (a.dL_denv[i] + a.w_tv * g) * dsoft;
        if (a.consume) a.dL_denv[i] = 0.f;
    }
    const float tot = block_sum_256(tv, s_part);
    if (threadIdx.x == 0 && a.tv_sum != nullptr) atomicAdd(sum_slot(a.tv_sum), tot);
}

__global__ void __launch_bounds__(256)
s2_env_backward_kernel(EnvBackward a)
{
    env_backward_block((int)blockIdx.x, a);
}

__global__ void __launch_bounds__(256)
s2_activate_backward_kernel(int P, const float* __restrict__ xyz, const float* __restrict__ scaling_raw,
                            const float* __restrict__ rotation_raw, const float* __restrict__ opacity_raw,
                            const float* __restrict__ normal_raw, const float* __restrict__ base_raw,
                            const float* __restrict__ rough_raw, const float* __restrict__ viewmatrix,
                            const float* __restrict__ campos, const float* __restrict__ dL_dfeatures,
                            const float* __restrict__ dL_dbase_shade, const float* __restrict__ dL_drough_shade,
                            const float* __restrict__ dL_dviewdirs, const float* __restrict__ dL_dscales,
                            const float* __restrict__ dL_drot, const float* __restrict__ dL_dopacity,
                            const float* __restrict__ dL_dmeans3D, float* __restrict__ g_xyz,
                            float* __restrict__ g_scaling, float* __restrict__ g_rotation,
                            float* __restrict__ g_opacity, float* __restrict__ g_normal, float* __restrict__ g_base,
                            float* __restrict__ g_rough, int nb_main, EnvBackward env_job)
{
    if ((int)blockIdx.x >= nb_main) {
        env_backward_block((int)blockIdx.x - nb_main, env_job);
        return;
    }
    const int i = blockIdx.x * 256 + threadIdx.x;
    if (i >= P) return;
    const size_t i3 = 3 * (size_t)i, i4 = 4 * (size_t)i;
    const float4* gf = reinterpret_cast<const float4*>(dL_dfeatures + 16 * (size_t)i);
    const float4 f0 = gf[0], f1 = gf[1], f2 = gf[2];
    {
        const float gfeat[3] = {f2.x, f2.y, f2.z};
#pragma unroll
        for (int c = 0; c < 3; c++) {
            const float s = sigmoidf_(base_raw[i3 + c]);
            g_base[i3 + c] = (gfeat[c] + dL_dbase_shade[i3 + c]) * 0.77f * s * (1.f - s);
        }
        const float s = sigmoidf_(rough_raw[i]);
        g_rough[i] = (f2.w + dL_drough_shade[i]) * 0.9f * s * (1.f - s);
    }
    if (g_xyz == nullptr) return;

#pragma unroll
    for (int c = 0; c < 3; c++) g_scaling[i3 + c] = dL_dscales[i3 + c] * __expf(scaling_raw[i3 + c]);
    {
        const float q[4] = {rotation_raw[i4], rotation_raw[i4 + 1], rotation_raw[i4 + 2], rotation_raw[i4 + 3]};
        const float g[4] = {dL_drot[i4], dL_drot[i4 + 1], dL_drot[i4 + 2], dL_drot[i4 + 3]};
        const float n = sqrtf(q[0] * q[0] + q[1] * q[1] + q[2] * q[2] + q[3] * q[3]);
        if (n > 1e-12f) {
            const float inv = 1.f / n;
            const float u[4] = {q[0] / n, q[1] / n, q[2] / n, q[3] / n};
            const float d = u[0] * g[0] + u[1] * g[1] + u[2] * g[2] + u[3] * g[3];
#pragma unroll
            for (int c = 0; c < 4; c++) g_rotation[i4 + c] = (g[c] - u[c] * d) * inv;
        } else {
#pragma unroll
            for (int c = 0; c < 4; c++) g_rotation[i4 + c] = g[c] * 1e12f;
        }
    }
    {
        const float s = sigmoidf_(opacity_raw[i]);
        g_opacity[i] = dL_dopacity[i] * s * (1.f - s);
    }
    {
        const float v[3] = {normal_raw[i3], normal_raw[i3 + 1], normal_raw[i3 + 2]};
        const float g[3] = {f1.y, f1.z, f1.w};
        float o[3];
        normalize3_backward(v, 1e-3f, g, o);
        g_normal[i3] = o[0]; g_normal[i3 + 1] = o[1]; g_normal[i3 + 2] = o[2];
    }
    {
        const float p[3] = {xyz[i3], xyz[i3 + 1], xyz[i3 + 2]};
        const float depth = p[0] * viewmatrix[2] + p[1] * viewmatrix[6] + p[2] * viewmatrix[10] + viewmatrix[14];
        const float gd = f0.x + 2.f * depth * f0.y;
        const float d[3] = {campos[0] - p[0], campos[1] - p[1], campos[2] - p[2]};
        const float gv[3] = {dL_dviewdirs[i3], dL_dviewdirs[i3 + 1], dL_dviewdirs[i3 + 2]};
        float gdd[3];
        normalize3_backward(d, 1e-12f, gv, gdd);
        g_xyz[i3] = dL_dmeans3D[i3] + gd * viewmatrix[2] - gdd[0];
        g_xyz[i3 + 1] = dL_dmeans3D[i3 + 1] + gd * viewmatrix[6] - gdd[1];
        g_xyz[i3 + 2] = dL_dmeans3D[i3 + 2] + gd * viewmatrix[10] - gdd[2];
    }
}

__global__ void __launch_bounds__(256)
s2_pbr_srgb_kernel(int HW, const float* __restrict__ opacity, const float* __restrict__ feature,
                   const int* __restrict__ n_contrib, const float* __restrict__ bg, float* __restrict__ srgb)
{
    const int i = blockIdx.x * 256 + threadIdx.x;
    if (i >= HW) return;
    const float op = opacity[i];
    const float scale = n_contrib[i] > 0 ? 1.f / fmaxf(op, 1e-5f) : 0.f;
#pragma unroll
    for (int c = 0; c < 3; c++) {
        const float x = feature[(size_t)(2 + c) * HW + i] * scale * op + (1.f - op) * bg[c];
        const float v = x <= 0.0031308f ? 12.92f * x : 1.055f * srgb_pow(fmaxf(x, 0.0031308f), 1.f / 2.4f) - 0.055f;
        srgb[(size_t)c * HW + i] = fminf(fmaxf(v, 0.f), 1.f);
    }
}

__global__ void __launch_bounds__(256)
s2_normals_srgb_kernel(int W, int H, float focal_x, float focal_y, float cx, float cy, const float* __restrict__ vm,
                       const float* __restrict__ opacity, const float* __restrict__ depths, float* __restrict__ normals,
                       float* __restrict__ surface_xyz, const float* __restrict__ feature, const int* __restrict__ n_contrib,
                       const float* __restrict__ bg, float* __restrict__ srgb)
{
    const int x = blockIdx.x * 64 + (threadIdx.x & 63), y = blockIdx.y * 4 + (threadIdx.x >> 6);
    if (x >= W || y >= H) return;
    const int HW = W * H, i = y * W + x;
    {
        const float op = opacity[i];
        const float scale = n_contrib[i] > 0 ? 1.f / fmaxf(op, 1e-5f) : 0.f;
#pragma unroll
        for (int c = 0; c < 3; c++) {
            const float v0 = feature[(size_t)(2 + c) * HW + i] * scale * op + (1.f - op) * bg[c];
            const float v = v0 <= 0.0031308f ? 12.92f * v0 : 1.055f * srgb_pow(fmaxf(v0, 0.0031308f), 1.f / 2.4f) - 0.055f;
            srgb[(size_t)c * HW + i] = fminf(fmaxf(v, 0.f), 1.f);
        }
    }
    pseudo_normal_pixel(x, y, W, H, focal_x, focal_y, cx, cy, vm, opacity, depths, normals, surface_xyz);
}

template <bool SPARSE>
__global__ void __launch_bounds__(256)
s2_loss_kernel(int HW, const float* __restrict__ image, const float* __restrict__ opacity,
               const float* __restrict__ feature, const float* __restrict__ pseudo_normal,
               const int* __restrict__ n_contrib, const float* __restrict__ gt, const float* __restrict__ bg,
               const float* __restrict__ image_mask, float w_l1, float w_pbr, float w_normal,
               const float* __restrict__ extra_dimage,
               const float* __restrict__ extra_dsrgb, float* __restrict__ dL_dimage,
               float* __restrict__ dL_dopacity, float* __restrict__ dL_dfeature, float* __restrict__ sums)
{
    __shared__ float s_part[4];
    float s_l1 = 0.f, s_pbr = 0.f, s_n = 0.f;
    for (int i = blockIdx.x * 256 + threadIdx.x; i < HW; i += gridDim.x * 256) {
        const float op = opacity[i];
        const int nc = n_contrib[i];
        float v_gt[3], v_im[3], v_ei[3], v_F[3], v_es[3], v_Fn[3], v_pn[3];
        const bool normal_on = !SPARSE || w_normal != 0.f;
#pragma unroll
        for (int c = 0; c < 3; c++) {
            v_gt[c] = gt[(size_t)c * HW + i];
            v_im[c] = image[(size_t)c * HW + i];
            v_F[c] = feature[(size_t)(2 + c) * HW + i];
        }
#pragma unroll
        for (int c = 0; c < 3; c++) {
            v_ei[c] = extra_dimage ? extra_dimage[(size_t)c * HW + i] : 0.f;
            v_es[c] = extra_dsrgb ? extra_dsrgb[(size_t)c * HW + i] : 0.f;
        }
        float mk = 1.f;
        if (normal_on) {
            mk = image_mask ? image_mask[i] : 1.f;
#pragma unroll
            for (int c = 0; c < 3; c++) {
                v_Fn[c] = feature[(size_t)(5 + c) * HW + i];
                v_pn[c] = pseudo_normal[(size_t)c * HW + i];
            }
        }
        const bool mask = nc > 0;
        const float opc = fmaxf(op, 1e-5f);
        const float scale = mask ? 1.f / opc : 0.f;
        const float dscale_dop = (mask && op >= 1e-5f) ? -1.f / (opc * opc) : 0.f;
        float g_op = 0.f;
#pragma unroll
        for (int c = 0; c < 3; c++) {
            const float g = v_gt[c];
            const float d0 = v_im[c] - g;
            s_l1 += fabsf(d0);
            dL_dimage[(size_t)c * HW + i] = w_l1 * signf_(d0) + v_ei[c];
            const float F = v_F[c];
            const float r = F * scale;
            const float x = r * op + (1.f - op) * bg[c];
            const bool lin = x <= 0.0031308f;
            const float xs = fmaxf(x, 0.0031308f);
            const float curve = lin ? 12.92f * x : 1.055f * srgb_pow(xs, 1.f / 2.4f) - 0.055f;
            const bool unclipped = curve >= 0.f && curve <= 1.f;
            const float srgb = fminf(fmaxf(curve, 0.f), 1.f);
            const float d1 = srgb - g;
            s_pbr += fabsf(d1);
            const float dsrgb = !unclipped ? 0.f : (lin ? 12.92f : 1.055f / 2.4f * srgb_pow(xs, 1.f / 2.4f - 1.f));
            const float gx = (w_pbr * signf_(d1) + v_es[c]) * dsrgb;
            dL_dfeature[(size_t)(2 + c) * HW + i] = gx * op * scale;
            g_op += gx * (r - bg[c] + op * F * dscale_dop);
            if (normal_on) {
                const float Fn = v_Fn[c];
                const float dn = (Fn * scale - v_pn[c]) * mk;
                s_n += dn * dn;
                const float gn = 2.f * w_normal * dn * mk;
                dL_dfeature[(size_t)(5 + c) * HW + i] = gn * scale;
                g_op += gn * Fn * dscale_dop;
            }
        }
        dL_dopacity[i] = g_op;
        if (!SPARSE) {
            dL_dfeature[i] = 0.f;
            dL_dfeature[(size_t)HW + i] = 0.f;
#pragma unroll
            for (int c = 8; c < 16; c++) dL_dfeature[(size_t)c * HW + i] = 0.f;
        }
    }
    const float t0 = block_sum_256(s_l1, s_part);
    __syncthreads();
    const float t1 = block_sum_256(s_pbr, s_part);
    __syncthreads();
    const float t2 = block_sum_256(s_n, s_part);
    if (threadIdx.x == 0) {
        atomicAdd(sum_slot(sums + 0 * R3DG_SUM_SLOTS), t0);
        atomicAdd(sum_slot(sums + 1 * R3DG_SUM_SLOTS), t1);
        atomicAdd(sum_slot(sums + 2 * R3DG_SUM_SLOTS), t2);
    }
}

void launch_s2_activate(hipStream_t s, int P, const float* xyz, const float* scaling_raw, const float* rotation_raw,
                        const float* opacity_raw, const float* normal_raw, const float* base_raw,
                        const float* rough_raw, const float* campos, float* scales, float* rot, float* opacity,
                        float* normal, float* base_color, float* roughness, float* viewdirs, const float* viewmatrix,
                        float* features, int n_env, const float* env_raw, float* env, float* zero, int n_zero)
{
    ActivateSide side;
    side.nb_main = (P + 255) / 256;
    side.n_env = env_raw != nullptr && env != nullptr ? n_env : 0;
    side.env_raw = env_raw;
    side.env = env;
    side.zero = zero;
    side.n_zero = zero != nullptr ? n_zero : 0;
    const int work = side.n_env > side.n_zero ? side.n_env : side.n_zero;
    const int nb_side = work > 0 ? (work + 255) / 256 < 8 ? (work + 255) / 256 : 8 : 0;
    s2_activate_kernel<<<side.nb_main + nb_side, 256, 0, s>>>(P, xyz, scaling_raw, rotation_raw, opacity_raw, normal_raw,
                                                              base_raw, rough_raw, campos, scales, rot, opacity, normal,
                                                              base_color, roughness, viewdirs, viewmatrix, features, side);
    check_launch(s, false, "s2_activate_kernel");
}

void launch_s2_pack(hipStream_t s, int P, const float* xyz, const float* viewmatrix, const float* normal,
                    const float* base_color, const float* roughness, const float* shade_out, float* features,
                    float* light_l1_sum)
{
    s2_pack_features_kernel<<<(P + 255) / 256, 256, 0, s>>>(P, xyz, viewmatrix, normal, base_color, roughness,
                                                            shade_out, features, light_l1_sum);
    check_launch(s, false, "s2_pack_features_kernel");
}

void launch_s2_unpack(hipStream_t s, int P, const float* dL_dfeatures, const float* shade_out, float light_weight,
                      float* dL_dpbr, float* dL_ddiffuse, float* block_absmax, float* light_l1_sum)
{
    s2_unpack_kernel<<<(P + 255) / 256, 256, 0, s>>>(P, dL_dfeatures, shade_out, light_weight, dL_dpbr, dL_ddiffuse,
                                                    block_absmax, light_l1_sum);
    check_launch(s, false, "s2_unpack_kernel");
}

void launch_s2_activate_backward(hipStream_t s, int P, const float* xyz, const float* scaling_raw,
                                 const float* rotation_raw, const float* opacity_raw, const float* normal_raw,
                                 const float* base_raw, const float* rough_raw, const float* viewmatrix,
                                 const float* campos, const float* dL_dfeatures, const float* dL_dbase_shade,
                                 const float* dL_drough_shade, const float* dL_dviewdirs, const float* dL_dscales,
                                 const float* dL_drot, const float* dL_dopacity, const float* dL_dmeans3D, float* g_xyz,
                                 float* g_scaling, float* g_rotation, float* g_opacity, float* g_normal, float* g_base,
                                 float* g_rough, int He, int We, const float* env_raw, const float* env, float* dL_denv,
                                 float w_tv, float* g_env_raw, float* tv_sum, int consume)
{
    EnvBackward job;
    job.He = He; job.We = We; job.raw = env_raw; job.env = env; job.dL_denv = dL_denv; job.w_tv = w_tv; job.g_raw = g_env_raw;
    job.tv_sum = tv_sum; job.consume = consume;
    const int nb_main = (P + 255) / 256;
    const int nb_env = env_raw != nullptr ? (He * We * 3 + 255) / 256 : 0;
    s2_activate_backward_kernel<<<nb_main + nb_env, 256, 0, s>>>(
        P, xyz, scaling_raw, rotation_raw, opacity_raw, normal_raw, base_raw, rough_raw, viewmatrix, campos,
        dL_dfeatures, dL_dbase_shade, dL_drough_shade, dL_dviewdirs, dL_dscales, dL_drot, dL_dopacity, dL_dmeans3D, g_xyz,
        g_scaling, g_rotation, g_opacity, g_normal, g_base, g_rough, nb_main, job);
    check_launch(s, false, "s2_activate_backward_kernel");
}

void launch_s2_normals_srgb(hipStream_t s, int W, int H, const float* vm, float focal_x, float focal_y, float cx, float cy,
                            const float* opacity, const float* depths, float* normals, float* surface_xyz, const float* feature,
                            const int* n_contrib, const float* bg, float* srgb)
{
    dim3 grid((W + 63) / 64, (H + 3) / 4);
    s2_normals_srgb_kernel<<<grid, 256, 0, s>>>(W, H, focal_x, focal_y, cx, cy, vm, opacity, depths, normals, surface_xyz,
                                                feature, n_contrib, bg, srgb);
    check_launch(s, false, "s2_normals_srgb_kernel");
}

void launch_s2_pbr_srgb(hipStream_t s, int HW, const float* opacity, const float* feature, const int* n_contrib,
                        const float* bg, float* srgb)
{
    s2_pbr_srgb_kernel<<<(HW + 255) / 256, 256, 0, s>>>(HW, opacity, feature, n_contrib, bg, srgb);
    check_launch(s, false, "s2_pbr_srgb_kernel");
}

constexpr int LOSS_BLOCKS = 768;

void launch_s2_loss(hipStream_t s, int HW, const float* image, const float* opacity, const float* feature,
                    const float* pseudo_normal, const int* n_contrib, const float* gt, const float* bg,
                    const float* image_mask, float w_l1, float w_pbr, float w_normal, const float* extra_dimage,
                    const float* extra_dsrgb, float* dL_dimage, float* dL_dopacity, float* dL_dfeature, float* sums,
                    int sparse)
{
    if (sparse)
        s2_loss_kernel<true><<<min((HW + 255) / 256, LOSS_BLOCKS), 256, 0, s>>>(
            HW, image, opacity, feature, pseudo_normal, n_contrib, gt, bg, image_mask, w_l1, w_pbr, w_normal, extra_dimage,
            extra_dsrgb, dL_dimage, dL_dopacity, dL_dfeature, sums);
    else
        s2_loss_kernel<false><<<min((HW + 255) / 256, LOSS_BLOCKS), 256, 0, s>>>(
            HW, image, opacity, feature, pseudo_normal, n_contrib, gt, bg, image_mask, w_l1, w_pbr, w_normal, extra_dimage,
            extra_dsrgb, dL_dimage, dL_dopacity, dL_dfeature, sums);
    check_launch(s, false, "s2_loss_kernel");
}

void launch_s2_env_backward(hipStream_t s, int He, int We, const float* raw, const float* env, float* dL_denv,
                            float w_tv, float* g_raw, float* tv_sum, int consume)
{
    EnvBackward job;
    job.He = He; job.We = We; job.raw = raw; job.env = env; job.dL_denv = dL_denv; job.w_tv = w_tv; job.g_raw = g_raw;
    job.tv_sum = tv_sum; job.consume = consume;
    s2_env_backward_kernel<<<(He * We * 3 + 255) / 256, 256, 0, s>>>(job);
    check_launch(s, false, "s2_env_backward_kernel");
}

}
```

relightable3dgaussian_amd/fused_step.py:

```python
import collections
import contextlib
import os

import torch
import torch.nn.functional as F

from . import _lib, rasterizer_ops, shading_ops
from .fused_adam import AdamGroup, FusedAdam
from .fused_base import _STREAMS, SUM_SLOTS, FusedStepBase, _in_context, _world_of, grad_slab, learning_rates, shared_stream
from .fused_samples import SampleSet, of_samples
from .fused_stage1 import FusedStage1Step
from .grad_comm import BucketComm
from .shading_ops import LEAVE_ROOM, TRAIN_OUTPUTS
from .train_step import FROZEN_GEOMETRY_GROUPS, LAMBDA_DSSIM, STAGE2_WEIGHTS, update_visibility, update_visibility_device

PARAM_NAMES = ("xyz", "normal", "scaling", "rotation", "opacity", "shs", "base_color", "roughness", "incidents", "env")

_View = collections.namedtuple("_View", "cam bg gt mask H W N vm campos main raw order_stream gt_depth mvs_normal")


class FusedStage2Step(FusedStepBase):

    _chain_kernel = True
    _opt_order = PARAM_NAMES
# ... 103 lines not shown
                                lambda self, v: setattr(self._comm, "comm_probe_every", v))

    get_scaling = lambda self: torch.exp(self.scaling)
    get_rotation = lambda self: F.normalize(self.rotation)
    get_opacity = lambda self: torch.sigmoid(self.opacity)
    get_shs = lambda self: self.shs
    get_normal = lambda self: F.normalize(self.normal, dim=-1, eps=1e-3)

    def refresh_activations(self, cam=None, env_out=None, zero=None):
        L = _lib.lib()
        campos = cam.camera_center if cam is not None else torch.zeros(3, device=self.dev)
        with torch.cuda.device(self.dev):
            st = L.r3dg_stage2_activate_with(
                _lib.current_stream(), self.P, self.xyz.data_ptr(), self.scaling.data_ptr(), self.rotation.data_ptr(),
                self.opacity.data_ptr(), self.normal.data_ptr(), self.base_color.data_ptr(), self.roughness.data_ptr(),
                campos.contiguous().data_ptr(), self.a_scales.data_ptr(), self.a_rot.data_ptr(),
                self.a_opacity.data_ptr(), self.a_normal.data_ptr(), self.a_base.data_ptr(), self.a_rough.data_ptr(),
                self.a_viewdirs.data_ptr(),
                cam.world_view_transform.contiguous().data_ptr() if cam is not None and self._direct_rows else None,
                self.features.data_ptr() if cam is not None and self._direct_rows else None,
                0 if env_out is None else env_out.numel(), None if env_out is None else self.env.data_ptr(),
                None if env_out is None else env_out.data_ptr(), None if zero is None else zero.data_ptr(),
                0 if zero is None else zero.numel())
        _lib.check(st, "stage2_activate")

    @_in_context
    def refresh_visibility(self):
        self.flush()
        self.refresh_activations()
        self._samples.refresh(self.xyz, self.a_scales, self.a_rot, self.a_opacity, self.a_normal)
        self._pre_rotated = None

    def taps(self, He, We):
        return self._samples.select(He, We)

    def _rotation_is_current(self):
        pr = self._pre_rotated
        return pr is not None and pr[0] is self._samples.frs and pr[1] is self._incidents and pr[2] == self._incidents._version

    def _early_stream(self):
        if self._adam_stream is None:
            self._adam_stream = shared_stream(self.dev, "early")
        return self._adam_stream

    def _aux_stream(self):
        if self._samples.frs is None or self.dp or self.serial_streams:
            return None
        return self._early_stream()

    def _listed_stream(self):
        frs = self._samples.frs
        if frs is None or frs.n_invalid == 0 or self.serial_streams:
            return None
        return self._early_stream()

    @_in_context
    def forward_backward(self, cam, bg, gt, early_adam=False, image_mask=None, split_geometry=None, chain_incidents=False,
                         gt_depth=None, mvs_normal=None, sh_adam_in_backward=False):
        H, W = cam.image_height, cam.image_width
        if self._supervised and (gt_depth is None or (self.w["normal_mvs_depth"] != 0.0 and mvs_normal is None)):
            raise RuntimeError("FusedStage2Step: the depth / normal_mvs_depth terms need gt_depth%s" % (
                "" if self.w["normal_mvs_depth"] == 0.0 else " and mvs_normal"))
        main = torch.cuda.current_stream(self.dev)
        v = _View(cam, bg, gt, image_mask, H, W, H * W, cam.world_view_transform.contiguous(), cam.camera_center.contiguous(),
                  main, main.cuda_stream, None if self.serial_streams else self._order_stream, gt_depth, mvs_normal)
        with torch.cuda.device(self.dev):
            pending, env_c, flag_cur, use_bounded, rotated_for = self._front_end(v)
            taps, packed = self._shade_forward(v, env_c, rotated_for)
            fw = pending.finish(v.order_stream)
            self._skip_cur = flag_cur
            g, active = self._image_loss(v, fw)
            fused_a = sh_adam_in_backward and self._fuses_sh_adam()
            dL_dfeatures, bw, geo_stream, handle_a = self._raster_backward(
                v, fw, g, active, early_adam if split_geometry is None else split_geometry, fused_a)
            b_early = self._schedule_early(v, handle_a, geo_stream, use_bounded, early_adam, chain_incidents, fused_a)
            self._shade_backward(v, env_c, taps, packed, dL_dfeatures, bw, geo_stream, b_early, chain_incidents)
            self._remaining_buckets(handle_a)
        return self._end_forward_backward(fw, None if bw is None else bw[0], use_bounded, v.N)

    def _front_end(self, v):
        rotated_for = None
        aux = self._aux_stream()
        if self._chain_deferred is not None:
            self.flush()
        if aux is not None:
            _lib.stream_wait(aux, v.main)
            rotated_for = self._samples.frs
            if not self._rotation_is_current():
                with torch.cuda.stream(aux):
                    rotated_for.rotate(self._incidents)
        if self._env_c is None or self._env_c.shape != self.env.shape[1:]:
            self._env_c = torch.empty(tuple(self.env.shape[1:]), dtype=torch.float32, device=self.dev)
        env_c = self._env_c
        self.refresh_activations(v.cam, env_out=env_c, zero=self.sums)
        self._iter += 1
        flag_cur = self._flag_of_iteration()
        use_bounded = self._use_bounded(v.W, v.H)
        if self._early_pending and (aux is None or not (use_bounded and v.order_stream is not None)):
            _lib.stream_wait(v.main, self._adam_stream)
            self._early_pending = False
        if use_bounded:
            bounded = dict(capacity=self._capacity, overflow_flag=flag_cur, overflow_count=self._overflow_count,
                           ordering_stream=v.order_stream)
        else:
            flag_cur.zero_()
            bounded = {}
        cam, empty = v.cam, torch.Tensor([])
        pending = rasterizer_ops.rasterize_gaussians_begin(
            v.bg, self.xyz, self.features, empty, self.a_opacity, self.a_scales, self.a_rot, 1.0, empty, v.vm,
            cam.full_proj_transform, cam.tanfovx, cam.tanfovy, cam.cx, cam.cy, v.H, v.W, self.shs, 3, v.campos, False,
            True, False, want_weights=False,
            defer_pseudo_normal=True, **bounded)
        if self._pending_b is not None:
            self.flush()
        if aux is not None:
            _lib.stream_wait(v.main, aux)
            self._early_pending = False
        return pending, env_c, flag_cur, use_bounded, rotated_for

    def _shade_forward(self, v, env_c, rotated_for):
        L = _lib.lib()
        He, We = env_c.shape[0], env_c.shape[1]
        sm = self._samples
        taps = sm.select(He, We)
        frs, area = sm.frs, sm.uniform_area
        if frs is not None:
            rotated = rotated_for is frs or (self.dp and self._rotation_is_current())
            frs.forward(self.a_base, self.a_rough, self.a_normal, self.a_viewdirs, self._incidents, env_c,
                        sm.visibility, self.shade_out, uniform_area=area,
                        leave_room=v.order_stream is not None and not self.dp,
                        listed_stream=self._listed_stream(), rotated=rotated,
                        feature_rows=self.features if self._direct_rows else None)
        else:
            _lib.check(L.r3dg_shade_forward_cached(
                v.raw, self.P, self.K, self.M, self.a_base.data_ptr(), self.a_rough.data_ptr(), self.a_normal.data_ptr(),
                self.a_viewdirs.data_ptr(), self._incidents.data_ptr(), env_c.data_ptr(), He, We, None,
                sm.visibility.data_ptr(), sm.incident_dirs.data_ptr(),
                None if area is not None else sm.incident_areas.data_ptr(), area or 0.0,
                taps.data_ptr(), TRAIN_OUTPUTS | (LEAVE_ROOM if v.order_stream is not None else 0),
                self.shade_out.data_ptr()), "shade_forward")
        if frs is not None and self._listed_stream() is not None:
            _lib.stream_wait(v.main, self._listed_stream())
        packed = not (frs is not None and self._direct_rows)
        if packed:
            _lib.check(L.r3dg_stage2_pack_features(v.raw, self.P, self.xyz.data_ptr(), v.vm.data_ptr(), self.a_normal.data_ptr(),
                self.a_base.data_ptr(), self.a_rough.data_ptr(), self.shade_out.data_ptr(), self.features.data_ptr(),
                self.sums[3].data_ptr()), "stage2_pack_features")
        return taps, packed

    def _image_loss(self, v, fw):
        L = _lib.lib()
        cam, W, H, N = v.cam, v.W, v.H, v.N
        _R, n_contrib, image, opacity, depth, feature, pseudo_normal, sxyz = fw[:8]
        g = torch.empty((47, H, W), dtype=torch.float32, device=self.dev)
        gt_c, bg_c = v.gt.contiguous(), v.bg.contiguous()
        srgb, part_i, part_p, gs_i, gs_p = g[20:23], g[23:32], g[32:41], g[41:44], g[44:47]
        lam = LAMBDA_DSSIM
        _lib.check(L.r3dg_stage2_normals_srgb(v.raw, W, H, v.vm.data_ptr(), float(cam.tanfovx), float(cam.tanfovy), float(cam.cx),
            float(cam.cy), opacity.data_ptr(), depth.data_ptr(), pseudo_normal.data_ptr(), sxyz.data_ptr(), feature.data_ptr(),
            n_contrib.data_ptr(), bg_c.data_ptr(), srgb.data_ptr()), "stage2_normals_srgb")
        _lib.check(L.r3dg_ssim_forward_pair(v.raw, W, H, 3, image.data_ptr(), srgb.data_ptr(), gt_c.data_ptr(), part_i.data_ptr(),
                                            part_p.data_ptr(), self.sums[5].data_ptr(), self.sums[6].data_ptr()), "ssim_forward")
        _lib.check(L.r3dg_ssim_backward_pair(v.raw, W, H, 3, image.data_ptr(), srgb.data_ptr(), gt_c.data_ptr(),
                                             part_i.data_ptr(), part_p.data_ptr(), -self.w["l1"] * lam / (3.0 * N),
                                             -self.w["pbr"] * lam / (3.0 * N), gs_i.data_ptr(), gs_p.data_ptr()),
                   "ssim_backward")
        mask_c = None if v.mask is None else v.mask.contiguous()
        _lib.check(L.r3dg_stage2_loss(v.raw, W, H, image.data_ptr(), opacity.data_ptr(), feature.data_ptr(),
            pseudo_normal.data_ptr(), n_contrib.data_ptr(), gt_c.data_ptr(), bg_c.data_ptr(), _lib.ptr(mask_c),
            self.w["l1"] * (1.0 - lam) / (3.0 * N), self.w["pbr"] * (1.0 - lam) / (3.0 * N), self.w["normal"] / (3.0 * N),
            gs_i.data_ptr(), gs_p.data_ptr(), g[0:3].data_ptr(), g[3:4].data_ptr(), g[4:20].data_ptr(), self.sums.data_ptr(), 1),
            "stage2_loss")
        active = [2, 3, 4] + ([5, 6, 7] if self.w["normal"] != 0.0 else [])
        w_bc, w_r, w_ls = (self.w[k] / (3.0 * N) for k in ("base_color_smooth", "roughness_smooth", "light_smooth"))
        if w_bc != 0.0 or w_r != 0.0 or w_ls != 0.0:
            _lib.check(L.r3dg_stage2_smooth_fused(v.raw, W, H, opacity.data_ptr(), feature.data_ptr(), n_contrib.data_ptr(),
                gt_c.data_ptr(), _lib.ptr(mask_c), w_bc, w_r, w_ls, 1 if self.w["normal"] != 0.0 else 0, g[3:4].data_ptr(),
                g[4:20].data_ptr(), self.sums[7].data_ptr()), "stage2_smooth_fused")
            active += ([8, 9, 10] if w_bc != 0.0 else []) + ([11] if w_r != 0.0 else [])
            if w_ls != 0.0:
                active += [12, 13, 14] + ([5, 6, 7] if self.w["normal"] == 0.0 else [])
        if self._supervised:
            w_d, w_nm = self.w["depth"], self.w["normal_mvs_depth"] / (3.0 * N)
            depth_c = v.gt_depth.contiguous()
            mvs_c = None if w_nm == 0.0 else v.mvs_normal.contiguous()
            self._sup_count_cur = self._supervision_count(v, depth_c, mask_c) if w_d != 0.0 else None
            _lib.check(L.r3dg_stage2_supervision(v.raw, W, H, opacity.data_ptr(), feature.data_ptr(), n_contrib.data_ptr(),
                depth_c.data_ptr(), _lib.ptr(mvs_c), _lib.ptr(mask_c), _lib.ptr(self._sup_count_cur), w_d, w_nm,
                1 if 5 in active else 0, g[3:4].data_ptr(), g[4:20].data_ptr(), self.sums[10].data_ptr()), "stage2_supervision")
            active += ([0] if w_d != 0.0 else []) + ([5, 6, 7] if w_nm != 0.0 and 5 not in active else [])
        self.last_active_features = sorted(set(active))
        return g, active

    def _supervision_count(self, v, depth_c, mask_c):
        key = id(v.gt_depth)
        hit = self._sup_counts.get(key)
        mv = None if v.mask is None else v.mask._version
        if hit is not None and hit[0] is v.gt_depth and hit[1] is v.mask and hit[2] == (v.gt_depth._version, mv):
            return hit[3]
        count = torch.empty(1, dtype=torch.int32, device=self.dev)
        _lib.check(_lib.lib().r3dg_supervision_count(v.raw, v.W, v.H, depth_c.data_ptr(), _lib.ptr(mask_c), count.data_ptr()),
                   "supervision_count")
        self._sup_counts[key] = (v.gt_depth, v.mask, (v.gt_depth._version, mv), count)
        return count

    def _fuses_sh_adam(self):
        can = getattr(rasterizer_ops.rasterize_gaussians_backward, "sh_adam_supported", None)
        return (not self.dp and bool(self._groups_a) and not self.frozen_geometry and can is not None
                and os.environ.get("R3DG_SH_ADAM_IN_BACKWARD", "1") != "0" and can(self.M))

    def _raster_backward(self, v, fw, g, active, split_geometry, fused_a=False):
        cam, empty = v.cam, torch.Tensor([])
        R, radii, geom, binning, img = fw[0], fw[9], fw[10], fw[11], fw[12]
        geo_stream = None
        if self.frozen_geometry:
            active = [a for a in active if a not in (0, 5, 6, 7)]
            dL_dfeatures = rasterizer_ops.rasterize_gaussians_backward_features(
                self.P, 16, v.H, v.W, g[4:20], geom, R, binning, img, active_features=sorted(active))
            bw = None
        else:
            geo_stream = self._listed_stream() if split_geometry else None
            fused = dict(sh_adam=self.opt.fused_step_of(self._groups_a[0], self.opt.step_count + 1, 1.0, self._skip_cur)) \
                if fused_a else {}
            bw = rasterizer_ops.rasterize_gaussians_backward(
                v.bg, self.xyz, self.features, radii, empty, self.a_scales, self.a_rot, 1.0, empty, v.vm,
                cam.full_proj_transform, cam.tanfovx, cam.tanfovy, g[0:3], g[3:4], empty, g[4:20],
                self.shs, 3, v.campos, geom, R, binning, img, True, False, dL_dsh_out=self.grads["shs"],
                geometry_stream=geo_stream, active_features=sorted(active), zeroed_accumulators=self._acc, **fused)
            dL_dfeatures = bw[4]
            if geo_stream is not None:
                if self._geo_done is None:
                    self._geo_done = torch.cuda.Event()
                self._geo_done.record(geo_stream)
        handle_a = None
        if self._bucket_a is not None and not self._single_bucket:
            with torch.cuda.stream(geo_stream) if geo_stream is not None else contextlib.nullcontext():
                handle_a = self._comm.allreduce_async(self._bucket_a, "A", self._iter)
        return dL_dfeatures, bw, geo_stream, handle_a

    def _schedule_early(self, v, handle_a, geo_stream, use_bounded, early_adam, chain_incidents, fused_a=False):
        a_launch = early_adam and bool(self._groups_a) and (handle_a is not None or not self.dp)
        b_early = (not self.dp and self._samples.frs is not None and v.order_stream is not None and use_bounded and
                   (a_launch or (bool(self._groups_b) and (self.P * self.K <= 40_000_000 if early_adam else chain_incidents))))
        a_early = a_launch or fused_a
        self._early, self._b_early, self._a_late = a_early or b_early, b_early, b_early and not a_early
        if self._early:
            side = self._early_stream()
            self.opt.begin_step()
            self._early_pending = not self.dp
        if fused_a:
            if b_early:
                _lib.stream_wait(v.order_stream, geo_stream if geo_stream is not None else v.main)
        elif a_early:
            if geo_stream is None and not self.dp:
                side.wait_stream(v.main)
            with torch.cuda.stream(side):
                if self.dp:
                    self._comm.wait(handle_a, "A", self._iter, side)
                    self._skip_cur = self._snapshot_flag()
                self.opt.step_groups(self._groups_a, [self.grads[k] for k in self._opt_order], 1.0 / self.world,
                                     skip_flag=self._skip_cur)
            if b_early:
                _lib.stream_wait(v.order_stream, side)
        return b_early

    def _shade_backward(self, v, env_c, taps, packed, dL_dfeatures, bw, geo_stream, b_early, chain_incidents):
        L = _lib.lib()
        P, gr = self.P, self.grads
        _lib.check(L.r3dg_stage2_unpack_gradients(
            v.raw, P, dL_dfeatures.data_ptr(), self.shade_out.data_ptr(), self.w["light"] / (3.0 * P),
            self.d_pbr.data_ptr(), self.d_diffuse.data_ptr(), self._absmax.data_ptr(),
            None if packed else self.sums[3].data_ptr()), "stage2_unpack_gradients")
        if self._d_env is None or self._d_env.shape != env_c.shape:
            self._d_env = torch.zeros_like(env_c)
        sm = self._samples
        frs = sm.frs
        if frs is not None:
            chain = b_early and bool(self._groups_b)
            dp_chain = (self.dp and chain_incidents and bool(self._groups_b) and not self._single_bucket
                        and os.environ.get("R3DG_DP_CHAIN", "1") != "0")
            d_base, d_rough, d_view, _d_inc, d_env = frs.backward(
                self.a_base, self.a_rough, self.a_normal, self.a_viewdirs, self._incidents, env_c, sm.visibility,
                self.d_pbr, self.d_diffuse, uniform_area=sm.uniform_area,
                out_incidents=frs.dcprime_rows() if dp_chain else gr["incidents"], out_env=self._d_env,
                block_absmax=self._absmax,
                rotate_stream=self._adam_stream if self._early else None, rotation_back=not (chain or dp_chain))
            self._dp_chain = frs if dp_chain else None
            if b_early:
                self._chain_deferred = (frs, self._skip_cur, self.opt.step_count)
        else:
            d_base, d_rough, d_view, _d_inc, d_env = shading_ops.shade_backward(self.a_base, self.a_rough, self.a_normal,
                self.a_viewdirs, self._incidents, env_c, sm.visibility, sm.incident_dirs, sm.incident_areas, self.d_pbr,
                self.d_diffuse, out_incidents=gr["incidents"], taps=taps, out_env=self._d_env, block_absmax=self._absmax)
        if geo_stream is not None:
            v.main.wait_event(self._geo_done)
        env_job = (env_c.shape[0], env_c.shape[1], self.env.data_ptr(), env_c.data_ptr(), d_env.data_ptr(),
                   self.w["env_smooth"], gr["env"].data_ptr(), self.sums[4].data_ptr(), 1)
        geo = (lambda t: None) if self.frozen_geometry else (lambda t: t.data_ptr())
        _means2D, _dcol, dL_dopacity, dL_dmeans3D, _dfeat, _dcov, _dsh, dL_dscales, dL_drot = bw or (None,) * 9
        _lib.check(L.r3dg_stage2_activate_backward_with(v.raw, P, geo(self.xyz), geo(self.scaling), geo(self.rotation),
            geo(self.opacity), geo(self.normal), self.base_color.data_ptr(), self.roughness.data_ptr(), geo(v.vm), geo(v.campos),
            dL_dfeatures.data_ptr(), d_base.data_ptr(), d_rough.data_ptr(), geo(d_view), geo(dL_dscales), geo(dL_drot),
            geo(dL_dopacity), geo(dL_dmeans3D), geo(gr["xyz"]), geo(gr["scaling"]), geo(gr["rotation"]), geo(gr["opacity"]),
            geo(gr["normal"]), gr["base_color"].data_ptr(), gr["roughness"].data_ptr(), *env_job), "stage2_activate_backward")

    def _remaining_buckets(self, handle_a):
        comm, it = self._comm, self._iter
        self._handles = None
        if self._single_bucket:
            self._handles = (None, comm.allreduce_async(self._bucket_all, "ALL", it), None)
        elif self.dp:
            handle_c = comm.allreduce_async(self._bucket_c, "C", it)
            if self._dp_chain is not None:
                handle_b = comm.allreduce_async(self._dp_chain.dcprime.view(-1), "B", it)
            else:
                with torch.cuda.stream(self._adam_stream) if self._early else contextlib.nullcontext():
                    handle_b = comm.allreduce_async(self._bucket_b, "B", it)
            self._handles = (handle_a, handle_c, handle_b)

    def loss(self):
        self.poll_overflow()
        N, P = self._N, self.P
        lam = LAMBDA_DSSIM
        w = torch.tensor([self.w["l1"] * (1 - lam) / (3.0 * N), self.w["pbr"] * (1 - lam) / (3.0 * N),
                          self.w["normal"] / (3.0 * N), self.w["light"] / (3.0 * P), self.w["env_smooth"],
                          -self.w["l1"] * lam / (3.0 * N), -self.w["pbr"] * lam / (3.0 * N),
                          self.w["base_color_smooth"] / (3.0 * N), self.w["roughness_smooth"] / (3.0 * N),
                          self.w["light_smooth"] / (3.0 * N)], device=self.dev)
        if self._supervised:
            count = 0 if self._sup_count_cur is None else int(self._sup_count_cur.item())
            w = torch.cat([w, torch.tensor([self.w["depth"] / count if count else 0.0, self.w["normal_mvs_depth"] / (3.0 * N)],
                                           device=self.dev)])
        return (self.sums.sum(1) * w).sum() + lam * (self.w["l1"] + self.w["pbr"])

    @_in_context
    def optimizer_step(self):
        grads = [self.grads[k] for k in self._opt_order]
        if not self.dp:
            if self._b_early:
                todo = (self._groups_a if self._a_late else ()) + self._groups_c
            elif self._early:
                _lib.stream_wait(torch.cuda.current_stream(), self._adam_stream)
                self._early_pending = False
                todo = self._groups_c + self._groups_b
            else:
# ... 83 lines not shown
```

relightable3dgaussian_amd/rasterizer_ops.py:

```python
import ctypes as C

import torch

from . import _lib

NUM_CHANNELS = 3


def _f32c(t):
    if t is None or t.numel() == 0:
        return None
    if t.dtype != torch.float32:
        raise RuntimeError("expected a float32 tensor, got %s" % t.dtype)
    if not t.is_cuda:
        raise RuntimeError("expected a CUDA(HIP) tensor")
    return t.contiguous()


class _Resizer:

    def __init__(self, device):
        self.device = device
        self.buffers = [torch.empty(0, dtype=torch.uint8, device=device) for _ in range(3)]
        self.callbacks = [_lib.ALLOC_FN(self._make(i)) for i in range(3)]
# ... 56 lines not shown
def rasterize_gaussians_begin(background, means3D, features, colors, opacity, scales, rotations, scale_modifier,
                              cov3D_precomp, viewmatrix, projmatrix, tan_fovx, tan_fovy, cx, cy, image_height,
                              image_width, sh, degree, campos, prefiltered, computer_pseudo_normal, debug,
                              capacity=None, overflow_flag=None, overflow_count=None, ordering_stream=None,
                              want_weights=True, defer_pseudo_normal=False):
    L = _lib.lib()
    if means3D.ndimension() != 2 or means3D.size(1) != 3:
        raise RuntimeError("means3D must have dimensions (num_points, 3)")
    if not means3D.is_cuda:
        raise RuntimeError("means3D must be a CUDA(HIP) tensor")
    P = means3D.size(0)
    S = features.size(1)
    H, W = int(image_height), int(image_width)
    dev = means3D.device
    fopt = dict(dtype=torch.float32, device=dev)

    slab = (torch.zeros if P == 0 else torch.empty)((11 + S, H, W), **fopt)
    out_color, out_opacity, out_depth = slab[0:3], slab[3:4], slab[4:5]
    out_feature, out_normal, out_surface_xyz = slab[5:5 + S], slab[5 + S:8 + S], slab[8 + S:11 + S]
    if defer_pseudo_normal:
        computer_pseudo_normal = False
    elif not computer_pseudo_normal:
        slab[5 + S:].zero_()
    out_weights = torch.zeros((P, 1), **fopt) if want_weights else None
    radii = torch.empty((P,), dtype=torch.int32, device=dev)

    rs = _Resizer(dev)
    ticket = C.c_void_p(None)
    if P != 0:
        M = sh.size(1) if sh.size(0) != 0 else 0
        t = [_f32c(x) for x in (background, means3D, sh, colors, features, opacity, scales, rotations, cov3D_precomp,
                                viewmatrix, projmatrix, campos)]
        bg_, means_, sh_, col_, feat_, op_, sc_, rot_, cov_, vm_, pm_, cam_ = t
        if feat_ is not None and feat_.data_ptr() != features.data_ptr():
            raise RuntimeError("rasterize_gaussians_begin needs contiguous features (their contents are read later)")
        rs.keep = t
        common = (rs.callbacks[0], rs.callbacks[1], rs.callbacks[2], None, P, S, int(degree), M,
                  _lib.ptr(bg_), W, H, _lib.ptr(means_), _lib.ptr(sh_), _lib.ptr(col_), _lib.ptr(feat_), _lib.ptr(op_),
                  _lib.ptr(sc_), float(scale_modifier), _lib.ptr(rot_), _lib.ptr(cov_), _lib.ptr(vm_), _lib.ptr(pm_),
                  _lib.ptr(cam_), float(tan_fovx), float(tan_fovy), float(cx), float(cy), int(bool(prefiltered)),
                  int(bool(computer_pseudo_normal)), out_color.data_ptr(), out_opacity.data_ptr(), out_depth.data_ptr(),
                  _lib.ptr(out_feature), out_normal.data_ptr(), out_surface_xyz.data_ptr(),
                  out_weights.data_ptr() if out_weights is not None else None,
                  radii.data_ptr(), int(bool(debug)))
        with torch.cuda.device(dev):
            if capacity is None:
                st = L.r3dg_rasterize_forward_begin(_lib.current_stream(), *common, C.byref(ticket))
            else:
                if overflow_flag is not None and (overflow_flag.dtype != torch.float32 or not overflow_flag.is_cuda):
                    raise RuntimeError("overflow_flag must be a float32 device tensor")
                if overflow_count is not None and (overflow_count.dtype != torch.int32 or not overflow_count.is_cuda):
                    raise RuntimeError("overflow_count must be an int32 device tensor")
                rs.keep.append((overflow_flag, overflow_count))
                st = L.r3dg_rasterize_forward_begin_bounded(
                    _lib.current_stream(), *common,
                    C.c_void_p(ordering_stream.cuda_stream) if ordering_stream is not None else None, int(capacity),
                    overflow_flag.data_ptr() if overflow_flag is not None else None,
                    overflow_count.data_ptr() if overflow_count is not None else None, C.byref(ticket))
        _lib.check(st, "rasterize_gaussians")
    elif capacity is not None and overflow_flag is not None:
        overflow_flag[:1].zero_()
    return _PendingForward(ticket, rs, (out_color, out_opacity, out_depth, out_feature, out_normal, out_surface_xyz,
                                        out_weights, radii), dev, H, W, capacity=capacity)


def rasterize_gaussians(background, means3D, features, colors, opacity, scales, rotations, scale_modifier,
                        cov3D_precomp, viewmatrix, projmatrix, tan_fovx, tan_fovy, cx, cy, image_height, image_width,
                        sh, degree, campos, prefiltered, computer_pseudo_normal, debug):
    return rasterize_gaussians_begin(background, means3D, features, colors, opacity, scales, rotations, scale_modifier,
                                     cov3D_precomp, viewmatrix, projmatrix, tan_fovx, tan_fovy, cx, cy, image_height,
                                     image_width, sh, degree, campos, prefiltered, computer_pseudo_normal,
                                     debug).finish()


def rasterize_gaussians_backward(background, means3D, features, radii, colors, scales, rotations, scale_modifier,
                                 cov3D_precomp, viewmatrix, projmatrix, tan_fovx, tan_fovy, dL_dout_color,
                                 dL_dout_opacity, dL_dout_depth, dL_dout_feature, sh, degree, campos, geomBuffer, R,
                                 binningBuffer, imageBuffer, backward_geometry, debug, dL_dsh_out=None,
                                 geometry_stream=None, active_features=None, zeroed_accumulators=None, sh_adam=None):
    L = _lib.lib()
    P = means3D.size(0)
    S = features.size(1)
    H = dL_dout_color.size(1)
    W = dL_dout_color.size(2)
    M = sh.size(1) if sh.size(0) != 0 else 0
    dev = means3D.device
    fopt = dict(dtype=torch.float32, device=dev)

    if zeroed_accumulators is not None:
        acc = zeroed_accumulators
        if acc.numel() != (11 + S) * P or acc.dtype != torch.float32 or not acc.is_contiguous() or acc.device != dev:
            raise RuntimeError("zeroed_accumulators must be a contiguous float32 tensor of (11 + S) * P floats on the device")
    else:
        acc = torch.empty((11 + S) * P, **fopt)
    dL_dfeatures = acc[0:S * P].view(P, S)
    o = S * P
    dL_dconic = acc[o:o + 4 * P].view(P, 2, 2); o += 4 * P
    dL_dmeans2D = acc[o:o + 3 * P].view(P, 3); o += 3 * P
    dL_dopacity = acc[o:o + P].view(P, 1); o += P
    dL_dcolors = acc[o:o + 3 * P].view(P, NUM_CHANNELS)
    have_sh = sh.numel() != 0 and colors.numel() == 0
    have_scale = scales.numel() != 0 and cov3D_precomp.numel() == 0
    dL_dmeans3D = torch.empty((P, 3), **fopt)
    dL_dcov3D = torch.empty((P, 6), **fopt)
    if dL_dsh_out is not None and have_sh:
        if tuple(dL_dsh_out.shape) != (P, M, 3) or not dL_dsh_out.is_contiguous() or dL_dsh_out.dtype != torch.float32:
            raise RuntimeError("dL_dsh_out must be a contiguous float32 [P,M,3] tensor")
        dL_dsh = dL_dsh_out
    else:
        dL_dsh = (torch.empty if have_sh else torch.zeros)((P, M, 3), **fopt)
    dL_dscales = (torch.empty if have_scale else torch.zeros)((P, 3), **fopt)
    dL_drotations = (torch.empty if have_scale else torch.zeros)((P, 4), **fopt)

    if P != 0:
        t = [_f32c(x) for x in (background, means3D, sh, features, colors, scales, rotations, cov3D_precomp, viewmatrix,
                                projmatrix, campos, dL_dout_color, dL_dout_opacity, dL_dout_depth, dL_dout_feature)]
        bg_, means_, sh_, feat_, col_, sc_, rot_, cov_, vm_, pm_, cam_, gC, gO, gD, gF = t
        radii_ = radii.contiguous()
        with torch.cuda.device(dev):
            cur = _lib.current_stream()
            gs = cur if geometry_stream is None else C.c_void_p(geometry_stream.cuda_stream)
            if active_features is None:
                n_act, act = -1, None
            else:
                n_act = len(active_features)
                act = (C.c_int * max(1, n_act))(*[int(a) for a in active_features])
            if sh_adam is not None:
                if sh_ is not sh or not have_sh:
                    raise RuntimeError("sh_adam: needs the contiguous float32 SH tensor itself as `sh`")
                entry, tail = L.r3dg_rasterize_backward_split_sh_adam, sh_adam
            else:
                entry, tail = L.r3dg_rasterize_backward_split, ()
            st = entry(
                cur, gs, P, S, int(degree), M, int(R), _lib.ptr(bg_), W, H, _lib.ptr(means_),
                _lib.ptr(sh_), _lib.ptr(feat_), _lib.ptr(col_), _lib.ptr(sc_), float(scale_modifier), _lib.ptr(rot_),
                _lib.ptr(cov_), _lib.ptr(vm_), _lib.ptr(pm_), _lib.ptr(cam_), float(tan_fovx), float(tan_fovy),
                radii_.data_ptr(), _lib.ptr(geomBuffer), _lib.ptr(binningBuffer), _lib.ptr(imageBuffer), _lib.ptr(gC),
                _lib.ptr(gO), _lib.ptr(gD), _lib.ptr(gF), dL_dmeans2D.data_ptr(), dL_dconic.data_ptr(),
                dL_dopacity.data_ptr(), dL_dcolors.data_ptr(), _lib.ptr(dL_dfeatures), dL_dmeans3D.data_ptr(),
                dL_dcov3D.data_ptr(), _lib.ptr(dL_dsh), dL_dscales.data_ptr(), dL_drotations.data_ptr(),
                int(bool(backward_geometry)), int(bool(debug)), n_act, act, *tail)
        _lib.check(st, "rasterize_gaussians_backward")
    return (dL_dmeans2D, dL_dcolors, dL_dopacity, dL_dmeans3D, dL_dfeatures, dL_dcov3D, dL_dsh, dL_dscales,
            dL_drotations)


def _sh_adam_supported(M):
    return bool(_lib.lib().r3dg_rasterize_backward_sh_adam_supported(int(M)))


rasterize_gaussians_backward.sh_adam_supported = _sh_adam_supported


def rasterize_gaussians_backward_features(P, S, image_height, image_width, dL_dout_feature, geomBuffer, R, binningBuffer,
                                          imageBuffer, debug=False, active_features=None):
    L = _lib.lib()
    dev = dL_dout_feature.device
    dL_dfeatures = torch.zeros((P, S), dtype=torch.float32, device=dev)
    if P != 0 and int(R) != 0:
        gF = _f32c(dL_dout_feature)
        if active_features is None:
            n_act, act = -1, None
        else:
            n_act = len(active_features)
            act = (C.c_int * max(1, n_act))(*[int(a) for a in active_features])
        with torch.cuda.device(dev):
            st = L.r3dg_rasterize_backward_features(
                _lib.current_stream(), int(P), int(S), int(R), int(image_width), int(image_height), _lib.ptr(geomBuffer),
                _lib.ptr(binningBuffer), _lib.ptr(imageBuffer), gF.data_ptr(), dL_dfeatures.data_ptr(), n_act, act,
                int(bool(debug)))
        _lib.check(st, "rasterize_gaussians_backward_features")
    return dL_dfeatures


def mark_visible(means3D, viewmatrix, projmatrix):
    L = _lib.lib()
    P = means3D.size(0)
    present = torch.zeros((P,), dtype=torch.bool, device=means3D.device)
    if P != 0:
        m, v, p = _f32c(means3D), _f32c(viewmatrix), _f32c(projmatrix)
        with torch.cuda.device(means3D.device):
            st = L.r3dg_mark_visible(_lib.current_stream(), P, m.data_ptr(), v.data_ptr(), p.data_ptr(),
                                     present.data_ptr())
        _lib.check(st, "mark_visible")
    return present


def num_rendered_of(geomBuffer, P):
    off = int(_lib.lib().r3dg_geometry_state_total_offset(int(P)))
    return geomBuffer[off:off + 8].view(torch.int64)[0]


def decode_state(geomBuffer, binningBuffer, imgBuffer, P, R, H, W):
    L = _lib.lib()
    T = ((W + 15) // 16) * ((H + 15) // 16)
    g = _offsets(L.r3dg_geometry_state_offsets, 9, P)
    i = _offsets(L.r3dg_image_state_offsets, 3, W, H)
    b = _offsets(L.r3dg_binning_state_offsets, 4, R)

    def view(buf, off, count, dtype, shape):
        nb = count * torch.empty((), dtype=dtype).element_size()
        return buf[off:off + nb].view(dtype).view(*shape)
    out = dict(
        depths=view(geomBuffer, g[0], P, torch.float32, (P,)),
        clamped=view(geomBuffer, g[1], 3 * P, torch.uint8, (P, 3)),
        means2D=view(geomBuffer, g[3], 2 * P, torch.float32, (P, 2)),
        cov3D=view(geomBuffer, g[4], 6 * P, torch.float32, (P, 6)),
        conic_opacity=view(geomBuffer, g[5], 4 * P, torch.float32, (P, 4)),
        rgb=view(geomBuffer, g[6], 3 * P, torch.float32, (P, 3)),
        tiles_touched=view(geomBuffer, g[7], P, torch.int32, (P,)),
        point_offsets=view(geomBuffer, g[8], P, torch.int32, (P,)),
        final_T=view(imgBuffer, i[0], H * W, torch.float32, (H, W)),
        n_contrib=view(imgBuffer, i[1], H * W, torch.int32, (H, W)),
        ranges=view(imgBuffer, i[2], 2 * T, torch.int32, (T, 2)),
    )
    if R > 0:
        out.update(
            keys_unsorted=view(binningBuffer, b[0], R, torch.int64, (R,)),
            keys=view(binningBuffer, b[1], R, torch.int64, (R,)),
            vals_unsorted=view(binningBuffer, b[2], R, torch.int32, (R,)),
            point_list=view(binningBuffer, b[3], R, torch.int32, (R,)),
        )
    return out
```

Measured before the change: 837.8 iters/s.

## Fuse stage-2 image tail: normals, sRGB, SSIM fwd/bwd and loss in one kernel

Replaces four launches (normals+sRGB, paired SSIM forward, paired SSIM backward, stage-2 loss) with one tiled kernel. Each block recomputes the SSIM forward and backward over a 32x32 tile with a halo held in LDS, then writes the loss gradients directly. This removes the intermediate srgb, partials and SSIM-gradient planes (27 HxW planes) and their global round-trips, and shrinks the scratch allocation. The cost is redundant halo computation, heavy register and LDS use, and a fallback path kept for large images.

```diff
diff --git a/include/r3dg_hip.h b/include/r3dg_hip.h
--- a/include/r3dg_hip.h
+++ b/include/r3dg_hip.h
@@ -279,6 +279,14 @@
                              float cx, float cy, const float* d_opacity, const float* d_depth, float* d_pseudo_normal,
                              float* d_surface_xyz, const float* d_feature, const int32_t* d_n_contrib,
                              const float* d_background, float* d_srgb);
+int r3dg_stage2_image_tail_supported(int width, int height);
+int r3dg_stage2_image_tail(void* stream, int width, int height, const float* d_viewmatrix, float tan_fovx, float tan_fovy,
+                           float cx, float cy, const float* d_image, const float* d_opacity, const float* d_depth,
+                           const float* d_feature, const int32_t* d_n_contrib, const float* d_gt, const float* d_background,
+                           const float* d_image_mask, float w_l1, float w_pbr, float w_normal, float scale_image,
+                           float scale_pbr, float* d_pseudo_normal, float* d_surface_xyz, float* d_dL_dimage,
+                           float* d_dL_dopacity, float* d_dL_dfeature, float* d_sums, float* d_ssim_sum_image,
+                           float* d_ssim_sum_pbr);
 
 int r3dg_ssim_forward(void* stream, int width, int height, int channels, const float* d_x, const float* d_y,
                       float* d_partials, float* d_sum);
diff --git a/relightable3dgaussian_amd/csrc/capi_stage.hip b/relightable3dgaussian_amd/csrc/capi_stage.hip
--- a/relightable3dgaussian_amd/csrc/capi_stage.hip
+++ b/relightable3dgaussian_amd/csrc/capi_stage.hip
@@ -285,6 +285,31 @@
     });
 }
 
+int r3dg_stage2_image_tail_supported(int width, int height) { return image_tail_applies(width, height) ? 1 : 0; }
+
+int r3dg_stage2_image_tail(void* stream_, int width, int height, const float* viewmatrix, float tan_fovx, float tan_fovy, float cx,
+                           float cy, const float* image, const float* opacity, const float* depth, const float* feature,
+                           const int32_t* n_contrib, const float* gt, const float* bg, const float* image_mask, float w_l1,
+                           float w_pbr, float w_normal, float scale_image, float scale_pbr, float* pseudo_normal,
+                           float* surface_xyz, float* dL_dimage, float* dL_dopacity, float* dL_dfeature, float* sums,
+                           float* ssim_sum_image, float* ssim_sum_pbr)
+{
+    if (width < 0 || height < 0) return invalid("stage2_image_tail: bad image size");
+    if ((long long)width * height == 0) return R3DG_OK;
+    if (!image_tail_applies(width, height)) return invalid("stage2_image_tail: image too large");
+    if (!viewmatrix || !image || !opacity || !depth || !feature || !n_contrib || !gt || !bg || !pseudo_normal || !surface_xyz ||
+        !dL_dimage || !dL_dopacity || !dL_dfeature || !sums || !ssim_sum_image || !ssim_sum_pbr)
+        return invalid("stage2_image_tail: null buffer");
+    return guarded([&]() -> int {
+        StageTimer t((hipStream_t)stream_, ST_S2_LOSS);
+        const float focal_y = height / (2.0f * tan_fovy), focal_x = width / (2.0f * tan_fovx);
+        launch_s2_image_tail((hipStream_t)stream_, width, height, viewmatrix, focal_x, focal_y, cx, cy, image, opacity, depth,
+                             feature, n_contrib, gt, bg, image_mask, w_l1, w_pbr, w_normal, scale_image, scale_pbr, pseudo_normal,
+                             surface_xyz, dL_dimage, dL_dopacity, dL_dfeature, sums, ssim_sum_image, ssim_sum_pbr);
+        return R3DG_OK;
+    });
+}
+
 int r3dg_ssim_forward_pair(void* stream_, int width, int height, int channels, const float* x0, const float* x1,
                            const float* y, float* partials0, float* partials1, float* sum0, float* sum1)
 {
diff --git a/relightable3dgaussian_amd/csrc/image_tail.hip b/relightable3dgaussian_amd/csrc/image_tail.hip
--- /dev/null
+++ b/relightable3dgaussian_amd/csrc/image_tail.hip
@@ -0,0 +1,367 @@
+#include "launchers.hpp"
+#include "ssim_window.hpp"
+#include "stage2_loss_math.hpp"
+#include "pseudo_normal.hpp"
+#include "r3dg_hip.h"
+
+namespace r3dg {
+
+constexpr int TAIL_T = 32;
+constexpr int TAIL_P = TAIL_T + 2 * SSIM_R;
+constexpr int TAIL_E = TAIL_T + 4 * SSIM_R;
+constexpr int TAIL_NLOAD = (TAIL_E * TAIL_E + 255) / 256;
+constexpr int TAIL_FB = 3;
+constexpr int TAIL_FV = 7;
+constexpr int TAIL_BB = 4;
+constexpr int TAIL_IN_FLOATS = 2 * TAIL_E * (TAIL_E + 1);
+constexpr int TAIL_H_FLOATS = 5 * TAIL_E * (TAIL_P + 1);
+constexpr int TAIL_PART_FLOATS = 3 * TAIL_P * (TAIL_P + 1);
+constexpr int TAIL_G_FLOATS = 3 * TAIL_P * (TAIL_T + 1);
+constexpr int TAIL_G_AT = TAIL_IN_FLOATS;
+static_assert(TAIL_G_AT % 2 == 0 && TAIL_PART_FLOATS <= TAIL_G_AT && TAIL_G_AT + TAIL_G_FLOATS <= TAIL_H_FLOATS, "LDS regions of the tail overlap");
+static_assert(TAIL_P % TAIL_FB == 0 && TAIL_P % TAIL_FV == 0 && TAIL_P * (TAIL_P / TAIL_FV) <= 256, "forward items");
+static_assert(TAIL_T % TAIL_BB == 0 && TAIL_T * (TAIL_T / TAIL_BB) == 256, "backward items");
+
+struct TailPbrRaw {
+    float op;
+    int nc;
+    float F, y;
+};
+
+struct ImageTail {
+    int W, H, tiles_x, n_tiles;
+    float focal_x, focal_y, cx, cy;
+    const float* vm;
+    const float* image;
+    const float* opacity;
+    const float* depths;
+    const float* feature;
+    const int* n_contrib;
+    const float* gt;
+    const float* bg;
+    const float* image_mask;
+    float w_l1, w_pbr, w_normal, scale_image, scale_pbr;
+    float* pseudo_normal;
+    float* surface_xyz;
+    float* dL_dimage;
+    float* dL_dopacity;
+    float* dL_dfeature;
+    float* sums;
+    float* ssim_sum_image;
+    float* ssim_sum_pbr;
+};
+
+__device__ __noinline__ void tail_pseudo_normal(int x, int y, int W, int H, float focal_x, float focal_y, float cx, float cy,
+                                                const float* __restrict__ vm, const float* __restrict__ opacities,
+                                                const float* __restrict__ depths, float* __restrict__ normals,
+                                                float* __restrict__ surface_xyz)
+{
+    pseudo_normal_pixel(x, y, W, H, focal_x, focal_y, cx, cy, vm, opacities, depths, normals, surface_xyz);
+}
+
+template <class Raw, class Fetch, class Make>
+__device__ __forceinline__ void tail_ssim_channel(float* s_raw, int W, int H, int bx, int by, Fetch fetch, Make make, float (&acc)[3][TAIL_BB],
+                                                  float& ssim_sum)
+{
+    float2v (*s_xy)[TAIL_E + 1] = reinterpret_cast<float2v (*)[TAIL_E + 1]>(s_raw);
+    float2v (*s_h01)[TAIL_P + 1] = reinterpret_cast<float2v (*)[TAIL_P + 1]>(s_raw);
+    float2v (*s_h23)[TAIL_P + 1] = reinterpret_cast<float2v (*)[TAIL_P + 1]>(s_raw + 2 * TAIL_E * (TAIL_P + 1));
+    float (*s_h4)[TAIL_P + 1] = reinterpret_cast<float (*)[TAIL_P + 1]>(s_raw + 4 * TAIL_E * (TAIL_P + 1));
+    float2v (*s_p01)[TAIL_P + 1] = reinterpret_cast<float2v (*)[TAIL_P + 1]>(s_raw);
+    float (*s_p2)[TAIL_P + 1] = reinterpret_cast<float (*)[TAIL_P + 1]>(s_raw + 2 * TAIL_P * (TAIL_P + 1));
+    float2v (*s_g01)[TAIL_T + 1] = reinterpret_cast<float2v (*)[TAIL_T + 1]>(s_raw + TAIL_G_AT);
+    float (*s_g2)[TAIL_T + 1] = reinterpret_cast<float (*)[TAIL_T + 1]>(s_raw + TAIL_G_AT + 2 * TAIL_P * (TAIL_T + 1));
+    int tid = threadIdx.x;
+    asm volatile("" : "+v"(tid));
+    {
+        float2v xy[TAIL_NLOAD];
+        Raw raw[TAIL_NLOAD];
+        bool in[TAIL_NLOAD];
+#pragma unroll
+        for (int j = 0; j < TAIL_NLOAD; j++) {
+            const int i = tid + j * 256;
+            const int r = i / TAIL_E, q = i % TAIL_E;
+            const int gy = by + r - 2 * SSIM_R, gx = bx + q - 2 * SSIM_R;
+            in[j] = i < TAIL_E * TAIL_E && gx >= 0 && gx < W && gy >= 0 && gy < H;
+            raw[j] = fetch((size_t)(in[j] ? gy : 0) * W + (in[j] ? gx : 0));
+        }
+#pragma unroll
+        for (int j = 0; j < TAIL_NLOAD; j++) {
+            float vx, vy;
+            make(raw[j], vx, vy);
+            xy[j].x = in[j] ? vx : 0.f;
+            xy[j].y = in[j] ? vy : 0.f;
+        }
+#pragma unroll
+        for (int j = 0; j < TAIL_NLOAD; j++) {
+            const int i = tid + j * 256;
+            if (i < TAIL_E * TAIL_E) s_xy[i / TAIL_E][i % TAIL_E] = xy[j];
+        }
+    }
+    __syncthreads();
+    float w[11];
+    ssim_load_window(w);
+    {
+        constexpr int GROUPS = TAIL_P / TAIL_FB, ITEMS = TAIL_E * GROUPS, ROUNDS = (ITEMS + 255) / 256;
+        float2v h01[ROUNDS][TAIL_FB], h23[ROUNDS][TAIL_FB];
+        float h4[ROUNDS][TAIL_FB];
+#pragma unroll
+        for (int rd = 0; rd < ROUNDS; rd++) {
+            const int i = tid + rd * 256;
+            if (i < ITEMS) {
+                const int r = i / GROUPS, q0 = (i % GROUPS) * TAIL_FB;
+                float2v xy[TAIL_FB + 10];
+#pragma unroll
+                for (int k = 0; k < TAIL_FB + 10; k++) xy[k] = s_xy[r][q0 + k];
+#pragma unroll
+                for (int o = 0; o < TAIL_FB; o++) ssim_taps_pair_packed(w, xy + o, h01[rd][o], h23[rd][o], h4[rd][o]);
+            }
+        }
+        __syncthreads();
+#pragma unroll
+        for (int rd = 0; rd < ROUNDS; rd++) {
+            const int i = tid + rd * 256;
+            if (i < ITEMS) {
+                const int r = i / GROUPS, q0 = (i % GROUPS) * TAIL_FB;
+#pragma unroll
+                for (int o = 0; o < TAIL_FB; o++) {
+                    s_h01[r][q0 + o] = h01[rd][o];
+                    s_h23[r][q0 + o] = h23[rd][o];
+                    s_h4[r][q0 + o] = h4[rd][o];
+                }
+            }
+        }
+    }
+    __syncthreads();
+    {
+        constexpr int ITEMS = TAIL_P * (TAIL_P / TAIL_FV);
+        const int qx = tid % TAIL_P, r0 = (tid / TAIL_P) * TAIL_FV;
+        float2v p01[TAIL_FV];
+        float p2[TAIL_FV];
+        if (tid < ITEMS) {
+            float2v mu[TAIL_FV], ee[TAIL_FV];
+            float e12[TAIL_FV];
+            {
+                float2v col[TAIL_FV + 10];
+#pragma unroll
+                for (int k = 0; k < TAIL_FV + 10; k++) col[k] = s_h01[r0 + k][qx];
+#pragma unroll
+                for (int o = 0; o < TAIL_FV; o++) mu[o] = ssim_taps(w, col + o);
+#pragma unroll
+                for (int k = 0; k < TAIL_FV + 10; k++) col[k] = s_h23[r0 + k][qx];
+#pragma unroll
+                for (int o = 0; o < TAIL_FV; o++) ee[o] = ssim_taps(w, col + o);
+            }
+            {
+                float col[TAIL_FV + 10];
+#pragma unroll
+                for (int k = 0; k < TAIL_FV + 10; k++) col[k] = s_h4[r0 + k][qx];
+#pragma unroll
+                for (int o = 0; o < TAIL_FV; o++) e12[o] = ssim_taps(w, col + o);
+            }
+            const int gx = bx + qx - SSIM_R;
+#pragma unroll
+            for (int o = 0; o < TAIL_FV; o++) {
+                const int gy = by + r0 + o - SSIM_R;
+                float q0, q1, q2;
+                const float ssim = ssim_pixel<true>(mu[o].x, mu[o].y, ee[o].x, ee[o].y, e12[o], q0, q1, q2);
+                const bool in = gx >= 0 && gx < W && gy >= 0 && gy < H;
+                p01[o].x = in ? q0 : 0.f;
+                p01[o].y = in ? q1 : 0.f;
+                p2[o] = in ? q2 : 0.f;
+                const bool own = in && gx >= bx && gx < bx + TAIL_T && gy >= by && gy < by + TAIL_T;
+                ssim_sum += own ? ssim : 0.f;
+            }
+        }
+        __syncthreads();
+        if (tid < ITEMS) {
+#pragma unroll
+            for (int o = 0; o < TAIL_FV; o++) {
+                s_p01[r0 + o][qx] = p01[o];
+                s_p2[r0 + o][qx] = p2[o];
+            }
+        }
+    }
+    __syncthreads();
+    {
+        constexpr int GROUPS = TAIL_T / TAIL_BB, ITEMS = TAIL_P * GROUPS, ROUNDS = (ITEMS + 255) / 256;
+#pragma unroll
+        for (int rd = 0; rd < ROUNDS; rd++) {
+            const int i = tid + rd * 256;
+            if (i < ITEMS) {
+                const int r = i / GROUPS, q0 = (i % GROUPS) * TAIL_BB;
+                float2v v01[TAIL_BB + 10];
+                float v2[TAIL_BB + 10];
+#pragma unroll
+                for (int k = 0; k < TAIL_BB + 10; k++) { v01[k] = s_p01[r][q0 + k]; v2[k] = s_p2[r][q0 + k]; }
+#pragma unroll
+                for (int o = 0; o < TAIL_BB; o++) {
+                    s_g01[r][q0 + o] = ssim_taps(w, v01 + o);
+                    s_g2[r][q0 + o] = ssim_taps(w, v2 + o);
+                }
+            }
+        }
+    }
+    __syncthreads();
+    const int tx = tid % TAIL_T, ty0 = (tid / TAIL_T) * TAIL_BB;
+    {
+        float2v c01[TAIL_BB + 10];
+        float c2[TAIL_BB + 10];
+#pragma unroll
+        for (int k = 0; k < TAIL_BB + 10; k++) { c01[k] = s_g01[ty0 + k][tx]; c2[k] = s_g2[ty0 + k][tx]; }
+#pragma unroll
+        for (int o = 0; o < TAIL_BB; o++) {
+            const float2v a01 = ssim_taps(w, c01 + o);
+            acc[0][o] = a01.x;
+            acc[1][o] = a01.y;
+            acc[2][o] = ssim_taps(w, c2 + o);
+        }
+    }
+}
+
+__global__ void __launch_bounds__(256, 3)
+s2_image_tail_kernel(const ImageTail a)
+{
+    __shared__ __attribute__((aligned(16))) float s_raw[TAIL_H_FLOATS];
+    __shared__ float s_part[4];
+    const int W = a.W, H = a.H;
+    const size_t HW = (size_t)H * W;
+    const bool pbr_job = (int)blockIdx.x < a.n_tiles;
+    const int job = pbr_job ? (int)blockIdx.x : (int)blockIdx.x - a.n_tiles;
+    const int tile = job % a.n_tiles;
+    const int bx = (tile % a.tiles_x) * TAIL_T, by = (tile / a.tiles_x) * TAIL_T;
+    const int tx = threadIdx.x % TAIL_T, ty0 = (threadIdx.x / TAIL_T) * TAIL_BB;
+    const int px = bx + tx;
+    float acc[3][TAIL_BB];
+    float ssim_sum = 0.f;
+
+    if (!pbr_job) {
+        const int c = job / a.n_tiles;
+        const float* __restrict__ xc = a.image + c * HW;
+        const float* __restrict__ yc = a.gt + c * HW;
+        tail_ssim_channel<float2v>(s_raw, W, H, bx, by, [&](size_t o) { float2v r; r.x = xc[o]; r.y = yc[o]; return r; },
+                                   [](const float2v r, float& vx, float& vy) { vx = r.x; vy = r.y; }, acc, ssim_sum);
+        float s_l1 = 0.f;
+        float im[TAIL_BB], g[TAIL_BB];
+        size_t off[TAIL_BB];
+#pragma unroll
+        for (int o = 0; o < TAIL_BB; o++) {
+            const int py = by + ty0 + o;
+            off[o] = px < W && py < H ? (size_t)py * W + px : 0;
+            im[o] = xc[off[o]];
+            g[o] = yc[off[o]];
+        }
+#pragma unroll
+        for (int o = 0; o < TAIL_BB; o++) {
+            if (px < W && by + ty0 + o < H) {
+                const float extra = ssim_grad_pixel(a.scale_image, acc[0][o], acc[1][o], acc[2][o], im[o], g[o]);
+                a.dL_dimage[c * HW + off[o]] = s2_loss_image(im[o], g[o], a.w_l1, extra, s_l1);
+            }
+        }
+        const float t0 = block_sum_256(s_l1, s_part);
+        __syncthreads();
+        const float t1 = block_sum_256(ssim_sum, s_part);
+        if (threadIdx.x == 0) {
+            atomicAdd(sum_slot(a.sums + 0 * R3DG_SUM_SLOTS), t0);
+            atomicAdd(sum_slot(a.ssim_sum_image), t1);
+        }
+        return;
+    }
+
+    const bool normal_on = a.w_normal != 0.f;
+    float g_op[TAIL_BB] = {0.f, 0.f, 0.f, 0.f};
+#pragma unroll 1
+    for (int o = 0; o < TAIL_BB; o++) {
+        const int py = by + ty0 + o;
+        if (px < W && py < H)
+            tail_pseudo_normal(px, py, W, H, a.focal_x, a.focal_y, a.cx, a.cy, a.vm, a.opacity, a.depths, a.pseudo_normal,
+                               a.surface_xyz);
+    }
+    float s_pbr = 0.f, s_n = 0.f;
+#pragma unroll 1
+    for (int c = 0; c < 3; c++) {
+        const float* __restrict__ Fc = a.feature + (size_t)(2 + c) * HW;
+        const float* __restrict__ yc = a.gt + c * HW;
+        const float bgc = a.bg[c];
+        int txo = threadIdx.x % TAIL_T, tyo = (threadIdx.x / TAIL_T) * TAIL_BB, bxo = bx, byo = by, Wo = W, Ho = H;
+        asm volatile("" : "+v"(txo), "+v"(tyo), "+s"(bxo), "+s"(byo), "+s"(Wo), "+s"(Ho));
+        tail_ssim_channel<TailPbrRaw>(s_raw, Wo, Ho, bxo, byo,
+                                      [&](size_t o) { return TailPbrRaw{a.opacity[o], a.n_contrib[o], Fc[o], yc[o]}; },
+                                      [&](const TailPbrRaw r, float& vx, float& vy) {
+                                          vx = s2_pbr_srgb_pixel(r.F, s2_divide_scale(r.op, r.nc), r.op, bgc);
+                                          vy = r.y;
+                                      },
+                                      acc, ssim_sum);
+        const int px = bxo + txo;
+        TailPbrRaw own[TAIL_BB];
+        float mk[TAIL_BB], Fn[TAIL_BB], pn[TAIL_BB];
+        size_t off[TAIL_BB];
+#pragma unroll
+        for (int o = 0; o < TAIL_BB; o++) {
+            const int py = byo + tyo + o;
+            off[o] = px < Wo && py < Ho ? (size_t)py * Wo + px : 0;
+            own[o] = TailPbrRaw{a.opacity[off[o]], a.n_contrib[off[o]], Fc[off[o]], yc[off[o]]};
+            mk[o] = 1.f; Fn[o] = 0.f; pn[o] = 0.f;
+            if (normal_on) {
+                if (a.image_mask != nullptr) mk[o] = a.image_mask[off[o]];
+                Fn[o] = a.feature[(size_t)(5 + c) * HW + off[o]];
+                pn[o] = a.pseudo_normal[c * HW + off[o]];
+            }
+        }
+#pragma unroll
+        for (int o = 0; o < TAIL_BB; o++) {
+            const int py = byo + tyo + o;
+            if (px < Wo && py < Ho) {
+                const float F = own[o].F, g = own[o].y, op = own[o].op;
+                const S2Divide dv = s2_divide(op, own[o].nc);
+                const float srgb = s2_pbr_srgb_pixel(F, dv.scale, op, bgc);
+                const float extra = ssim_grad_pixel(a.scale_pbr, acc[0][o], acc[1][o], acc[2][o], srgb, g);
+                a.dL_dfeature[(size_t)(2 + c) * HW + off[o]] = s2_loss_pbr(F, g, op, bgc, dv, a.w_pbr, extra, s_pbr, g_op[o]);
+                if (normal_on)
+                    a.dL_dfeature[(size_t)(5 + c) * HW + off[o]] = s2_loss_normal(Fn[o], pn[o], mk[o], dv, a.w_normal, s_n, g_op[o]);
+            }
+        }
+    }
+#pragma unroll
+    for (int o = 0; o < TAIL_BB; o++) {
+        const int py = by + ty0 + o;
+        if (px < W && py < H) a.dL_dopacity[(size_t)py * W + px] = g_op[o];
+    }
+    const float t1 = block_sum_256(s_pbr, s_part);
+    __syncthreads();
+    const float t2 = block_sum_256(s_n, s_part);
+    __syncthreads();
+    const float t3 = block_sum_256(ssim_sum, s_part);
+    if (threadIdx.x == 0) {
+        atomicAdd(sum_slot(a.sums + 1 * R3DG_SUM_SLOTS), t1);
+        if (normal_on) atomicAdd(sum_slot(a.sums + 2 * R3DG_SUM_SLOTS), t2);
+        atomicAdd(sum_slot(a.ssim_sum_pbr), t3);
+    }
+}
+
+bool image_tail_applies(int W, int H)
+{
+    return W > 0 && H > 0 && (long long)W * H <= 0x7fffffffLL;
+}
+
+void launch_s2_image_tail(hipStream_t s, int W, int H, const float* vm, float focal_x, float focal_y, float cx, float cy,
+                          const float* image, const float* opacity, const float* depths, const float* feature, const int* n_contrib,
+                          const float* gt, const float* bg, const float* image_mask, float w_l1, float w_pbr, float w_normal,
+                          float scale_image, float scale_pbr, float* pseudo_normal, float* surface_xyz, float* dL_dimage,
+                          float* dL_dopacity, float* dL_dfeature, float* sums, float* ssim_sum_image, float* ssim_sum_pbr)
+{
+    ImageTail a;
+    a.W = W; a.H = H;
+    a.tiles_x = (W + TAIL_T - 1) / TAIL_T;
+    a.n_tiles = a.tiles_x * ((H + TAIL_T - 1) / TAIL_T);
+    a.focal_x = focal_x; a.focal_y = focal_y; a.cx = cx; a.cy = cy;
+    a.vm = vm; a.image = image; a.opacity = opacity; a.depths = depths; a.feature = feature; a.n_contrib = n_contrib; a.gt = gt;
+    a.bg = bg; a.image_mask = image_mask;
+    a.w_l1 = w_l1; a.w_pbr = w_pbr; a.w_normal = w_normal; a.scale_image = scale_image; a.scale_pbr = scale_pbr;
+    a.pseudo_normal = pseudo_normal; a.surface_xyz = surface_xyz; a.dL_dimage = dL_dimage; a.dL_dopacity = dL_dopacity;
+    a.dL_dfeature = dL_dfeature; a.sums = sums; a.ssim_sum_image = ssim_sum_image; a.ssim_sum_pbr = ssim_sum_pbr;
+    s2_image_tail_kernel<<<4 * a.n_tiles, 256, 0, s>>>(a);
+    check_launch(s, false, "s2_image_tail_kernel");
+}
+
+}
diff --git a/relightable3dgaussian_amd/csrc/launchers.hpp b/relightable3dgaussian_amd/csrc/launchers.hpp
--- a/relightable3dgaussian_amd/csrc/launchers.hpp
+++ b/relightable3dgaussian_amd/csrc/launchers.hpp
@@ -169,6 +169,12 @@
 void launch_s2_normals_srgb(hipStream_t s, int W, int H, const float* vm, float focal_x, float focal_y, float cx, float cy,
                             const float* opacity, const float* depths, float* normals, float* surface_xyz,
                             const float* feature, const int* n_contrib, const float* bg, float* srgb);
+bool image_tail_applies(int W, int H);
+void launch_s2_image_tail(hipStream_t s, int W, int H, const float* vm, float focal_x, float focal_y, float cx, float cy,
+                          const float* image, const float* opacity, const float* depths, const float* feature, const int* n_contrib,
+                          const float* gt, const float* bg, const float* image_mask, float w_l1, float w_pbr, float w_normal,
+                          float scale_image, float scale_pbr, float* pseudo_normal, float* surface_xyz, float* dL_dimage,
+                          float* dL_dopacity, float* dL_dfeature, float* sums, float* ssim_sum_image, float* ssim_sum_pbr);
 void launch_ssim_forward(hipStream_t s, int W, int H, int C, int n_images, const float* const* x, const float* y,
                          float* const* partials, float* const* sum);
 void launch_ssim_backward(hipStream_t s, int W, int H, int C, int n_images, const float* const* x, const float* y,
diff --git a/relightable3dgaussian_amd/csrc/ssim.hip b/relightable3dgaussian_amd/csrc/ssim.hip
--- a/relightable3dgaussian_amd/csrc/ssim.hip
+++ b/relightable3dgaussian_amd/csrc/ssim.hip
@@ -1,16 +1,12 @@
 #include "launchers.hpp"
+#include "ssim_window.hpp"
 
 namespace r3dg {
 
-constexpr int SSIM_R = 5;
 constexpr int SSIM_T = 32;
 constexpr int SSIM_E = SSIM_T + 2 * SSIM_R;
 constexpr int SSIM_B = 4;
 constexpr int SSIM_NLOAD = (SSIM_E * SSIM_E + 255) / 256;
-
-__constant__ float kSsimWin[11] = {1.028380124e-03f, 7.598758209e-03f, 3.600077331e-02f, 1.093606874e-01f,
-                                   2.130055279e-01f, 2.660117149e-01f, 2.130055279e-01f, 1.093606874e-01f,
-                                   3.600077331e-02f, 7.598758209e-03f, 1.028380124e-03f};
 
 struct SsimImage {
     const float* x;
@@ -95,8 +91,7 @@
         }
     }
     float w[11];
-#pragma unroll
-    for (int k = 0; k < 11; k++) w[k] = kSsimWin[k];
+    ssim_load_window(w);
     constexpr int ITEMS = SSIM_E * (SSIM_T / SSIM_B), ROUNDS = (ITEMS + 255) / 256;
     float hres[ROUNDS][5][SSIM_B];
 #pragma unroll
@@ -108,15 +103,8 @@
 #pragma unroll
             for (int k = 0; k < SSIM_B + 10; k++) { xv[k] = s_x[r][q0 + k]; yv[k] = s_y[r][q0 + k]; }
 #pragma unroll
-            for (int o = 0; o < SSIM_B; o++) {
-                float a0 = 0.f, a1 = 0.f, a2 = 0.f, a3 = 0.f, a4 = 0.f;
-#pragma unroll
-                for (int k = 0; k < 11; k++) {
-                    const float wx = w[k] * xv[o + k], wy = w[k] * yv[o + k];
-                    a0 += wx; a1 += wy; a2 += wx * xv[o + k]; a3 += wy * yv[o + k]; a4 += wx * yv[o + k];
-                }
-                hres[rd][0][o] = a0; hres[rd][1][o] = a1; hres[rd][2][o] = a2; hres[rd][3][o] = a3; hres[rd][4][o] = a4;
-            }
+            for (int o = 0; o < SSIM_B; o++)
+                ssim_taps_pair(w, xv + o, yv + o, hres[rd][0][o], hres[rd][1][o], hres[rd][2][o], hres[rd][3][o], hres[rd][4][o]);
         }
     }
     __syncthreads();
@@ -141,12 +129,7 @@
 #pragma unroll
         for (int k = 0; k < SSIM_B + 10; k++) col[k] = s_h[m][ty0 + k][tx];
 #pragma unroll
-        for (int o = 0; o < SSIM_B; o++) {
-            float a = 0.f;
-#pragma unroll
-            for (int k = 0; k < 11; k++) a += w[k] * col[o + k];
-            acc[m][o] = a;
-        }
+        for (int o = 0; o < SSIM_B; o++) acc[m][o] = ssim_taps(w, col + o);
     }
     float ssim_sum = 0.f;
     float* pc = EVAL ? nullptr : partials + (size_t)c * 3 * HW;
@@ -154,20 +137,13 @@
     for (int o = 0; o < SSIM_B; o++) {
         const int py = by + ty0 + o;
         if (px < W && py < H) {
-            const float mu1 = acc[0][o], mu2 = acc[1][o], e11 = acc[2][o], e22 = acc[3][o], e12 = acc[4][o];
-            const float C1 = 0.01f * 0.01f, C2 = 0.03f * 0.03f;
-            const float A = 2.f * mu1 * mu2 + C1;
-            const float B = 2.f * (e12 - mu1 * mu2) + C2;
-            const float C = mu1 * mu1 + mu2 * mu2 + C1;
-            const float D = (e11 - mu1 * mu1) + (e22 - mu2 * mu2) + C2;
-            const float inv = 1.f / (C * D);
-            const float ssim = A * B * inv;
-            ssim_sum += ssim;
+            float p0, p1, p2;
+            ssim_sum += ssim_pixel<!EVAL>(acc[0][o], acc[1][o], acc[2][o], acc[3][o], acc[4][o], p0, p1, p2);
             if constexpr (!EVAL) {
                 const size_t off = (size_t)py * W + px;
-                pc[off] = 2.f * mu2 * (B - A) * inv - ssim * 2.f * mu1 * (D - C) * inv;
-                pc[HW + off] = -ssim / D;
-                pc[2 * HW + off] = 2.f * A * inv;
+                pc[off] = p0;
+                pc[HW + off] = p1;
+                pc[2 * HW + off] = p2;
             }
         }
     }
@@ -255,8 +231,7 @@
     }
     __syncthreads();
     float w[11];
-#pragma unroll
-    for (int k = 0; k < 11; k++) w[k] = kSsimWin[k];
+    ssim_load_window(w);
     constexpr int ITEMS = SSIM_E * (SSIM_T / SSIM_B), ROUNDS = (ITEMS + 255) / 256;
     float hres[ROUNDS][3][SSIM_B];
 #pragma unroll
@@ -270,12 +245,7 @@
 #pragma unroll
                 for (int k = 0; k < SSIM_B + 10; k++) v[k] = s_p[m][r][q0 + k];
 #pragma unroll
-                for (int o = 0; o < SSIM_B; o++) {
-                    float a = 0.f;
-#pragma unroll
-                    for (int k = 0; k < 11; k++) a += w[k] * v[o + k];
-                    hres[rd][m][o] = a;
-                }
+                for (int o = 0; o < SSIM_B; o++) hres[rd][m][o] = ssim_taps(w, v + o);
             }
         }
     }
@@ -299,19 +269,14 @@
 #pragma unroll
         for (int k = 0; k < SSIM_B + 10; k++) col[k] = s_h[m][ty0 + k][tx];
 #pragma unroll
-        for (int o = 0; o < SSIM_B; o++) {
-            float a = 0.f;
-#pragma unroll
-            for (int k = 0; k < 11; k++) a += w[k] * col[o + k];
-            acc[m][o] = a;
-        }
+        for (int o = 0; o < SSIM_B; o++) acc[m][o] = ssim_taps(w, col + o);
     }
 #pragma unroll
     for (int o = 0; o < SSIM_B; o++) {
         const int py = by + ty0 + o;
         if (px < W && py < H) {
             const size_t off = (size_t)py * W + px;
-            grad_x[c * HW + off] = scale * (acc[0][o] + 2.f * xo[o] * acc[1][o] + yo[o] * acc[2][o]);
+            grad_x[c * HW + off] = ssim_grad_pixel(scale, acc[0][o], acc[1][o], acc[2][o], xo[o], yo[o]);
         }
     }
 }
diff --git a/relightable3dgaussian_amd/csrc/ssim_window.hpp b/relightable3dgaussian_amd/csrc/ssim_window.hpp
--- /dev/null
+++ b/relightable3dgaussian_amd/csrc/ssim_window.hpp
@@ -0,0 +1,72 @@
+#pragma once
+#include "common.hpp"
+
+namespace r3dg {
+
+constexpr int SSIM_R = 5;
+
+inline __constant__ float kSsimWin[11] = {1.028380124e-03f, 7.598758209e-03f, 3.600077331e-02f, 1.093606874e-01f,
+                                          2.130055279e-01f, 2.660117149e-01f, 2.130055279e-01f, 1.093606874e-01f,
+                                          3.600077331e-02f, 7.598758209e-03f, 1.028380124e-03f};
+
+__device__ __forceinline__ void ssim_load_window(float (&w)[11])
+{
+#pragma unroll
+    for (int k = 0; k < 11; k++) w[k] = kSsimWin[k];
+}
+
+__device__ __forceinline__ void ssim_taps_pair(const float (&w)[11], const float* xv, const float* yv, float& a0, float& a1,
+                                               float& a2, float& a3, float& a4)
+{
+    a0 = 0.f; a1 = 0.f; a2 = 0.f; a3 = 0.f; a4 = 0.f;
+#pragma unroll
+    for (int k = 0; k < 11; k++) {
+        const float wx = w[k] * xv[k], wy = w[k] * yv[k];
+        a0 += wx; a1 += wy; a2 += wx * xv[k]; a3 += wy * yv[k]; a4 += wx * yv[k];
+    }
+}
+
+typedef float float2v __attribute__((ext_vector_type(2)));
+template <class T>
+__device__ __forceinline__ T ssim_taps(const float (&w)[11], const T* v)
+{
+    T a = 0.f;
+#pragma unroll
+    for (int k = 0; k < 11; k++) a += w[k] * v[k];
+    return a;
+}
+
+__device__ __forceinline__ void ssim_taps_pair_packed(const float (&w)[11], const float2v* xy, float2v& a01, float2v& a23, float& a4)
+{
+    a01 = 0.f; a23 = 0.f; a4 = 0.f;
+#pragma unroll
+    for (int k = 0; k < 11; k++) {
+        const float2v wxy = w[k] * xy[k];
+        a01 += wxy; a23 += wxy * xy[k]; a4 += wxy.x * xy[k].y;
+    }
+}
+
+template <bool PARTIALS>
+__device__ __forceinline__ float ssim_pixel(float mu1, float mu2, float e11, float e22, float e12, float& p0, float& p1, float& p2)
+{
+    const float C1 = 0.01f * 0.01f, C2 = 0.03f * 0.03f;
+    const float A = 2.f * mu1 * mu2 + C1;
+    const float B = 2.f * (e12 - mu1 * mu2) + C2;
+    const float C = mu1 * mu1 + mu2 * mu2 + C1;
+    const float D = (e11 - mu1 * mu1) + (e22 - mu2 * mu2) + C2;
+    const float inv = 1.f / (C * D);
+    const float ssim = A * B * inv;
+    if constexpr (PARTIALS) {
+        p0 = 2.f * mu2 * (B - A) * inv - ssim * 2.f * mu1 * (D - C) * inv;
+        p1 = -ssim / D;
+        p2 = 2.f * A * inv;
+    }
+    return ssim;
+}
+
+__device__ __forceinline__ float ssim_grad_pixel(float scale, float a0, float a1, float a2, float x, float y)
+{
+    return scale * (a0 + 2.f * x * a1 + y * a2);
+}
+
+}
diff --git a/relightable3dgaussian_amd/csrc/stage2_glue.hip b/relightable3dgaussian_amd/csrc/stage2_glue.hip
--- a/relightable3dgaussian_amd/csrc/stage2_glue.hip
+++ b/relightable3dgaussian_amd/csrc/stage2_glue.hip
@@ -1,5 +1,6 @@
 #include "launchers.hpp"
 #include "glue_math.hpp"
+#include "stage2_loss_math.hpp"
 #include "pseudo_normal.hpp"
 #include "r3dg_hip.h"
 
@@ -271,13 +272,10 @@
     const int i = blockIdx.x * 256 + threadIdx.x;
     if (i >= HW) return;
     const float op = opacity[i];
-    const float scale = n_contrib[i] > 0 ? 1.f / fmaxf(op, 1e-5f) : 0.f;
-#pragma unroll
-    for (int c = 0; c < 3; c++) {
-        const float x = feature[(size_t)(2 + c) * HW + i] * scale * op + (1.f - op) * bg[c];
-        const float v = x <= 0.0031308f ? 12.92f * x : 1.055f * srgb_pow(fmaxf(x, 0.0031308f), 1.f / 2.4f) - 0.055f;
-        srgb[(size_t)c * HW + i] = fminf(fmaxf(v, 0.f), 1.f);
-    }
+    const float scale = s2_divide_scale(op, n_contrib[i]);
+#pragma unroll
+    for (int c = 0; c < 3; c++)
+        srgb[(size_t)c * HW + i] = s2_pbr_srgb_pixel(feature[(size_t)(2 + c) * HW + i], scale, op, bg[c]);
 }
 
 __global__ void __launch_bounds__(256)
@@ -291,13 +289,10 @@
     const int HW = W * H, i = y * W + x;
     {
         const float op = opacity[i];
-        const float scale = n_contrib[i] > 0 ? 1.f / fmaxf(op, 1e-5f) : 0.f;
-#pragma unroll
-        for (int c = 0; c < 3; c++) {
-            const float v0 = feature[(size_t)(2 + c) * HW + i] * scale * op + (1.f - op) * bg[c];
-            const float v = v0 <= 0.0031308f ? 12.92f * v0 : 1.055f * srgb_pow(fmaxf(v0, 0.0031308f), 1.f / 2.4f) - 0.055f;
-            srgb[(size_t)c * HW + i] = fminf(fmaxf(v, 0.f), 1.f);
-        }
+        const float scale = s2_divide_scale(op, n_contrib[i]);
+#pragma unroll
+        for (int c = 0; c < 3; c++)
+            srgb[(size_t)c * HW + i] = s2_pbr_srgb_pixel(feature[(size_t)(2 + c) * HW + i], scale, op, bg[c]);
     }
     pseudo_normal_pixel(x, y, W, H, focal_x, focal_y, cx, cy, vm, opacity, depths, normals, surface_xyz);
 }
@@ -339,39 +334,14 @@
                 v_pn[c] = pseudo_normal[(size_t)c * HW + i];
             }
         }
-        const bool mask = nc > 0;
-        const float opc = fmaxf(op, 1e-5f);
-        const float scale = mask ? 1.f / opc : 0.f;
-        const float dscale_dop = (mask && op >= 1e-5f) ? -1.f / (opc * opc) : 0.f;
+        const S2Divide dv = s2_divide(op, nc);
         float g_op = 0.f;
 #pragma unroll
         for (int c = 0; c < 3; c++) {
-            const float g = v_gt[c];
-            const float d0 = v_im[c] - g;
-            s_l1 += fabsf(d0);
-            dL_dimage[(size_t)c * HW + i] = w_l1 * signf_(d0) + v_ei[c];
-            const float F = v_F[c];
-            const float r = F * scale;
-            const float x = r * op + (1.f - op) * bg[c];
-            const bool lin = x <= 0.0031308f;
-            const float xs = fmaxf(x, 0.0031308f);
-            const float curve = lin ? 12.92f * x : 1.055f * srgb_pow(xs, 1.f / 2.4f) - 0.055f;
-            const bool unclipped = curve >= 0.f && curve <= 1.f;
-            const float srgb = fminf(fmaxf(curve, 0.f), 1.f);
-            const float d1 = srgb - g;
-            s_pbr += fabsf(d1);
-            const float dsrgb = !unclipped ? 0.f : (lin ? 12.92f : 1.055f / 2.4f * srgb_pow(xs, 1.f / 2.4f - 1.f));
-            const float gx = (w_pbr * signf_(d1) + v_es[c]) * dsrgb;
-            dL_dfeature[(size_t)(2 + c) * HW + i] = gx * op * scale;
-            g_op += gx * (r - bg[c] + op * F * dscale_dop);
-            if (normal_on) {
-                const float Fn = v_Fn[c];
-                const float dn = (Fn * scale - v_pn[c]) * mk;
-                s_n += dn * dn;
-                const float gn = 2.f * w_normal * dn * mk;
-                dL_dfeature[(size_t)(5 + c) * HW + i] = gn * scale;
-                g_op += gn * Fn * dscale_dop;
-            }
+            dL_dimage[(size_t)c * HW + i] = s2_loss_image(v_im[c], v_gt[c], w_l1, v_ei[c], s_l1);
+            dL_dfeature[(size_t)(2 + c) * HW + i] = s2_loss_pbr(v_F[c], v_gt[c], op, bg[c], dv, w_pbr, v_es[c], s_pbr, g_op);
+            if (normal_on)
+                dL_dfeature[(size_t)(5 + c) * HW + i] = s2_loss_normal(v_Fn[c], v_pn[c], mk, dv, w_normal, s_n, g_op);
         }
         dL_dopacity[i] = g_op;
         if (!SPARSE) {
diff --git a/relightable3dgaussian_amd/csrc/stage2_loss_math.hpp b/relightable3dgaussian_amd/csrc/stage2_loss_math.hpp
--- /dev/null
+++ b/relightable3dgaussian_amd/csrc/stage2_loss_math.hpp
@@ -0,0 +1,62 @@
+#pragma once
+#include "glue_math.hpp"
+
+namespace r3dg {
+
+struct S2Divide {
+    float scale, dscale_dop;
+};
+__device__ __forceinline__ float s2_divide_scale(float op, int nc) { return nc > 0 ? 1.f / fmaxf(op, 1e-5f) : 0.f; }
+__device__ __forceinline__ S2Divide s2_divide(float op, int nc)
+{
+    const bool mask = nc > 0;
+    const float opc = fmaxf(op, 1e-5f);
+    S2Divide d;
+    d.scale = mask ? 1.f / opc : 0.f;
+    d.dscale_dop = (mask && op >= 1e-5f) ? -1.f / (opc * opc) : 0.f;
+    return d;
+}
+
+__device__ __forceinline__ float s2_pbr_srgb_pixel(float F, float scale, float op, float bgc)
+{
+    const float v0 = F * scale * op + (1.f - op) * bgc;
+    const float v = v0 <= 0.0031308f ? 12.92f * v0 : 1.055f * srgb_pow(fmaxf(v0, 0.0031308f), 1.f / 2.4f) - 0.055f;
+    return fminf(fmaxf(v, 0.f), 1.f);
+}
+
+__device__ __forceinline__ float s2_loss_image(float im, float g, float w_l1, float extra, float& s_l1)
+{
+    const float d0 = im - g;
+    s_l1 += fabsf(d0);
+    return w_l1 * signf_(d0) + extra;
+}
+
+__device__ __forceinline__ float s2_loss_pbr(float F, float g, float op, float bgc, const S2Divide dv, float w_pbr, float extra,
+                                             float& s_pbr, float& g_op)
+{
+    const float scale = dv.scale;
+    const float r = F * scale;
+    const float x = r * op + (1.f - op) * bgc;
+    const bool lin = x <= 0.0031308f;
+    const float xs = fmaxf(x, 0.0031308f);
+    const float curve = lin ? 12.92f * x : 1.055f * srgb_pow(xs, 1.f / 2.4f) - 0.055f;
+    const bool unclipped = curve >= 0.f && curve <= 1.f;
+    const float srgb = fminf(fmaxf(curve, 0.f), 1.f);
+    const float d1 = srgb - g;
+    s_pbr += fabsf(d1);
+    const float dsrgb = !unclipped ? 0.f : (lin ? 12.92f : 1.055f / 2.4f * srgb_pow(xs, 1.f / 2.4f - 1.f));
+    const float gx = (w_pbr * signf_(d1) + extra) * dsrgb;
+    g_op += gx * (r - bgc + op * F * dv.dscale_dop);
+    return gx * op * scale;
+}
+
+__device__ __forceinline__ float s2_loss_normal(float Fn, float pn, float mk, const S2Divide dv, float w_normal, float& s_n, float& g_op)
+{
+    const float dn = (Fn * dv.scale - pn) * mk;
+    s_n += dn * dn;
+    const float gn = 2.f * w_normal * dn * mk;
+    g_op += gn * Fn * dv.dscale_dop;
+    return gn * dv.scale;
+}
+
+}
diff --git a/relightable3dgaussian_amd/fused_step.py b/relightable3dgaussian_amd/fused_step.py
--- a/relightable3dgaussian_amd/fused_step.py
+++ b/relightable3dgaussian_amd/fused_step.py
@@ -279,25 +279,33 @@
         L = _lib.lib()
         cam, W, H, N = v.cam, v.W, v.H, v.N
         _R, n_contrib, image, opacity, depth, feature, pseudo_normal, sxyz = fw[:8]
-        g = torch.empty((47, H, W), dtype=torch.float32, device=self.dev)
         gt_c, bg_c = v.gt.contiguous(), v.bg.contiguous()
-        srgb, part_i, part_p, gs_i, gs_p = g[20:23], g[23:32], g[32:41], g[41:44], g[44:47]
+        mask_c = None if v.mask is None else v.mask.contiguous()
         lam = LAMBDA_DSSIM
-        _lib.check(L.r3dg_stage2_normals_srgb(v.raw, W, H, v.vm.data_ptr(), float(cam.tanfovx), float(cam.tanfovy), float(cam.cx),
-            float(cam.cy), opacity.data_ptr(), depth.data_ptr(), pseudo_normal.data_ptr(), sxyz.data_ptr(), feature.data_ptr(),
-            n_contrib.data_ptr(), bg_c.data_ptr(), srgb.data_ptr()), "stage2_normals_srgb")
-        _lib.check(L.r3dg_ssim_forward_pair(v.raw, W, H, 3, image.data_ptr(), srgb.data_ptr(), gt_c.data_ptr(), part_i.data_ptr(),
-                                            part_p.data_ptr(), self.sums[5].data_ptr(), self.sums[6].data_ptr()), "ssim_forward")
-        _lib.check(L.r3dg_ssim_backward_pair(v.raw, W, H, 3, image.data_ptr(), srgb.data_ptr(), gt_c.data_ptr(),
-                                             part_i.data_ptr(), part_p.data_ptr(), -self.w["l1"] * lam / (3.0 * N),
-                                             -self.w["pbr"] * lam / (3.0 * N), gs_i.data_ptr(), gs_p.data_ptr()),
-                   "ssim_backward")
-        mask_c = None if v.mask is None else v.mask.contiguous()
-        _lib.check(L.r3dg_stage2_loss(v.raw, W, H, image.data_ptr(), opacity.data_ptr(), feature.data_ptr(),
-            pseudo_normal.data_ptr(), n_contrib.data_ptr(), gt_c.data_ptr(), bg_c.data_ptr(), _lib.ptr(mask_c),
-            self.w["l1"] * (1.0 - lam) / (3.0 * N), self.w["pbr"] * (1.0 - lam) / (3.0 * N), self.w["normal"] / (3.0 * N),
-            gs_i.data_ptr(), gs_p.data_ptr(), g[0:3].data_ptr(), g[3:4].data_ptr(), g[4:20].data_ptr(), self.sums.data_ptr(), 1),
-            "stage2_loss")
+        w_l1, w_pbr, w_n = (self.w["l1"] * (1.0 - lam) / (3.0 * N), self.w["pbr"] * (1.0 - lam) / (3.0 * N),
+                            self.w["normal"] / (3.0 * N))
+        ssim_i, ssim_p = -self.w["l1"] * lam / (3.0 * N), -self.w["pbr"] * lam / (3.0 * N)
+        if self._fuses_image_tail(W, H):
+            g = torch.empty((20, H, W), dtype=torch.float32, device=self.dev)
+            _lib.check(L.r3dg_stage2_image_tail(v.raw, W, H, v.vm.data_ptr(), float(cam.tanfovx), float(cam.tanfovy), float(cam.cx),
+                float(cam.cy), image.data_ptr(), opacity.data_ptr(), depth.data_ptr(), feature.data_ptr(), n_contrib.data_ptr(),
+                gt_c.data_ptr(), bg_c.data_ptr(), _lib.ptr(mask_c), w_l1, w_pbr, w_n, ssim_i, ssim_p, pseudo_normal.data_ptr(),
+                sxyz.data_ptr(), g[0:3].data_ptr(), g[3:4].data_ptr(), g[4:20].data_ptr(), self.sums.data_ptr(),
+                self.sums[5].data_ptr(), self.sums[6].data_ptr()), "stage2_image_tail")
+        else:
+            g = torch.empty((47, H, W), dtype=torch.float32, device=self.dev)
+            srgb, part_i, part_p, gs_i, gs_p = g[20:23], g[23:32], g[32:41], g[41:44], g[44:47]
+            _lib.check(L.r3dg_stage2_normals_srgb(v.raw, W, H, v.vm.data_ptr(), float(cam.tanfovx), float(cam.tanfovy),
+                float(cam.cx), float(cam.cy), opacity.data_ptr(), depth.data_ptr(), pseudo_normal.data_ptr(), sxyz.data_ptr(),
+                feature.data_ptr(), n_contrib.data_ptr(), bg_c.data_ptr(), srgb.data_ptr()), "stage2_normals_srgb")
+            _lib.check(L.r3dg_ssim_forward_pair(v.raw, W, H, 3, image.data_ptr(), srgb.data_ptr(), gt_c.data_ptr(),
+                part_i.data_ptr(), part_p.data_ptr(), self.sums[5].data_ptr(), self.sums[6].data_ptr()), "ssim_forward")
+            _lib.check(L.r3dg_ssim_backward_pair(v.raw, W, H, 3, image.data_ptr(), srgb.data_ptr(), gt_c.data_ptr(),
+                part_i.data_ptr(), part_p.data_ptr(), ssim_i, ssim_p, gs_i.data_ptr(), gs_p.data_ptr()), "ssim_backward")
+            _lib.check(L.r3dg_stage2_loss(v.raw, W, H, image.data_ptr(), opacity.data_ptr(), feature.data_ptr(),
+                pseudo_normal.data_ptr(), n_contrib.data_ptr(), gt_c.data_ptr(), bg_c.data_ptr(), _lib.ptr(mask_c), w_l1, w_pbr, w_n,
+                gs_i.data_ptr(), gs_p.data_ptr(), g[0:3].data_ptr(), g[3:4].data_ptr(), g[4:20].data_ptr(), self.sums.data_ptr(), 1),
+                "stage2_loss")
         active = [2, 3, 4] + ([5, 6, 7] if self.w["normal"] != 0.0 else [])
         w_bc, w_r, w_ls = (self.w[k] / (3.0 * N) for k in ("base_color_smooth", "roughness_smooth", "light_smooth"))
         if w_bc != 0.0 or w_r != 0.0 or w_ls != 0.0:
@@ -318,6 +326,11 @@
             active += ([0] if w_d != 0.0 else []) + ([5, 6, 7] if w_nm != 0.0 and 5 not in active else [])
         self.last_active_features = sorted(set(active))
         return g, active
+
+    @staticmethod
+    def _fuses_image_tail(W, H):
+        can = getattr(rasterizer_ops.rasterize_gaussians_begin, "image_tail_supported", None)
+        return can is not None and os.environ.get("R3DG_IMAGE_TAIL", "1") != "0" and bool(can(W, H))
 
     def _supervision_count(self, v, depth_c, mask_c):
         key = id(v.gt_depth)
diff --git a/relightable3dgaussian_amd/rasterizer_ops.py b/relightable3dgaussian_amd/rasterizer_ops.py
--- a/relightable3dgaussian_amd/rasterizer_ops.py
+++ b/relightable3dgaussian_amd/rasterizer_ops.py
@@ -232,6 +232,13 @@
 rasterize_gaussians_backward.sh_adam_supported = _sh_adam_supported
 
 
+def _image_tail_supported(W, H):
+    return _lib.lib().r3dg_stage2_image_tail_supported(int(W), int(H)) == 1
+
+
+rasterize_gaussians_begin.image_tail_supported = _image_tail_supported
+
+
 def rasterize_gaussians_backward_features(P, S, image_height, image_width, dL_dout_feature, geomBuffer, R, binningBuffer,
                                           imageBuffer, debug=False, active_features=None):
     L = _lib.lib()
```

Measured after the change: 848.8 iters/s, median of 6. +1.3%, better.
